# bifurcation/fourq

Hardware: AMD Instinct MI355X
Metric: FourQ scalar-mults/sec (batch, whole node) (higher is better)
Workload: dtype u64

## Files before the change

### fourq_amd/_lib.py

```python
import ctypes
import os
from ctypes import POINTER, c_char_p, c_int, c_size_t, c_uint8, c_uint64, c_void_p

HERE = os.path.dirname(os.path.abspath(__file__))
LIB_PATH = os.environ.get("FOURQ_AMD_LIB") or os.path.join(HERE, "libfourq_amd.so")

os.environ.setdefault("GPU_MAX_HW_QUEUES", "8")

OK, ERR_INVALID, ERR_NODEVICE, ERR_NOMEM, ERR_HIP = 0, -1, -2, -3, -4
DH_OK, DH_NOT_ON_CURVE, DH_NEUTRAL = 0, 1, 2
DECODE_OK, DECODE_RESERVED_BIT, DECODE_NOT_ON_CURVE, DECODE_REF_ATTRIBUTE_ERROR = 0, 1, 2, 3

MAX_BATCH = 0xFFFFFF00
ABI_VERSION = 600
COMB_POINTS = 1024 + 80
COMB_WORDS = COMB_POINTS * 12
BYTES_DECODE_BASE = 16
SIG_S_RANGE, SIG_MSG_CLAMPED, SIG_MAX_MSG = 32, 64, 1 << 20
H2C_RO, H2C_NU, H2C_MAX_DST = 0, 1, 255


class HostStats(ctypes.Structure):
    _fields_ = [("h2d_ms", ctypes.c_double), ("d2h_ms", ctypes.c_double), ("h2d_bytes", c_uint64), ("d2h_bytes", c_uint64),
                ("chunks", ctypes.c_uint32), ("pinned_in", c_int), ("pinned_out", c_int), ("kernels_ms", ctypes.c_double), ("kernels_span_ms", ctypes.c_double),
# ... 24 lines not shown
    "fourq_ctx_host_stats_sized": (c_int, [c_void_p, c_void_p, c_size_t]),
    "fourq_ctx_host_chunk_stamps": (c_int, [c_void_p, ctypes.c_uint32, POINTER(ctypes.c_double)]),
    "fourq_ctx_set_host_timing": (c_int, [c_void_p, c_int]),
    "fourq_diag_clock": (c_int, [c_void_p, ctypes.c_uint32, POINTER(ctypes.c_double), POINTER(ctypes.c_double), POINTER(ctypes.c_double), POINTER(c_int)]),
    "fourq_diag_clock_begin": (c_int, [c_void_p]),
    "fourq_diag_clock_stop": (c_int, [c_void_p]),
    "fourq_diag_clock_end": (c_int, [c_void_p, POINTER(ctypes.c_double), POINTER(ctypes.c_double), POINTER(ctypes.c_double), POINTER(ctypes.c_double)]),
    "fourq_dev_alloc": (c_int, [c_void_p, c_size_t, POINTER(c_void_p)]),
    "fourq_dev_free": (c_int, [c_void_p, c_void_p]),
    "fourq_dev_upload": (c_int, [c_void_p, c_void_p, c_void_p, c_size_t]),
    "fourq_dev_download": (c_int, [c_void_p, c_void_p, c_void_p, c_size_t]),
    "fourq_table_windowed": (c_int, [c_void_p, c_void_p, c_void_p]),
    "fourq_table_endo": (c_int, [c_void_p, c_void_p, c_void_p]),
    "fourq_mul_endo_batch": (c_int, [c_void_p, c_void_p, c_void_p, c_void_p, c_size_t]),
    "fourq_mul_windowed_batch": (c_int, [c_void_p, c_void_p, c_void_p, c_void_p, c_size_t]),
    "fourq_mul_endo_batch_dev": (c_int, [c_void_p, c_void_p, c_void_p, c_void_p, c_size_t]),
    "fourq_mul_windowed_batch_dev": (c_int, [c_void_p, c_void_p, c_void_p, c_void_p, c_size_t]),
    "fourq_mul_endo_affine_batch": (c_int, [c_void_p, c_void_p, c_void_p, c_void_p, c_size_t]),
    "fourq_mul_windowed_affine_batch": (c_int, [c_void_p, c_void_p, c_void_p, c_void_p, c_size_t]),
    "fourq_mul_endo_affine_batch_dev": (c_int, [c_void_p, c_void_p, c_void_p, c_void_p, c_size_t]),
    "fourq_mul_windowed_affine_batch_dev": (c_int, [c_void_p, c_void_p, c_void_p, c_void_p, c_size_t]),
    "fourq_mul_endo_bytes_batch": (c_int, [c_void_p, c_void_p, c_void_p, c_void_p, c_void_p, c_size_t]),
    "fourq_mul_windowed_bytes_batch": (c_int, [c_void_p, c_void_p, c_void_p, c_void_p, c_void_p, c_size_t]),
    "fourq_mul_endo_bytes_batch_dev": (c_int, [c_void_p, c_void_p, c_void_p, c_void_p, c_void_p, c_size_t]),
    "fourq_mul_windowed_bytes_batch_dev": (c_int, [c_void_p, c_void_p, c_void_p, c_void_p, c_void_p, c_size_t]),
    "fourq_mul_endo_fixed_batch": (c_int, [c_void_p, c_void_p, c_void_p, c_void_p, c_size_t]),
    "fourq_mul_windowed_fixed_batch": (c_int, [c_void_p, c_void_p, c_void_p, c_void_p, c_size_t]),
    "fourq_mul_endo_fixed_batch_dev": (c_int, [c_void_p, c_void_p, c_void_p, c_void_p, c_size_t]),
    "fourq_mul_windowed_fixed_batch_dev": (c_int, [c_void_p, c_void_p, c_void_p, c_void_p, c_size_t]),
    "fourq_mul_endo_mixed_batch": (c_int, [c_void_p, c_void_p, c_void_p, c_void_p, c_void_p, c_void_p, c_size_t]),
    "fourq_mul_endo_mixed_batch_dev": (c_int, [c_void_p, c_void_p, c_void_p, c_void_p, c_void_p, c_void_p, c_size_t]),
    "fourq_dh_endo_batch": (c_int, [c_void_p, c_void_p, c_void_p, c_void_p, c_void_p, c_void_p, c_size_t]),
    "fourq_dh_windowed_batch": (c_int, [c_void_p, c_void_p, c_void_p, c_void_p, c_void_p, c_void_p, c_size_t]),
    "fourq_dh_endo_batch_dev": (c_int, [c_void_p, c_void_p, c_void_p, c_void_p, c_void_p, c_void_p, c_size_t]),
    "fourq_dh_windowed_batch_dev": (c_int, [c_void_p, c_void_p, c_void_p, c_void_p, c_void_p, c_void_p, c_size_t]),
    "fourq_dh_endo_bytes_batch": (c_int, [c_void_p, c_void_p, c_void_p, c_void_p, c_void_p, c_void_p, c_size_t]),
    "fourq_dh_windowed_bytes_batch": (c_int, [c_void_p, c_void_p, c_void_p, c_void_p, c_void_p, c_void_p, c_size_t]),
    "fourq_dh_endo_bytes_batch_dev": (c_int, [c_void_p, c_void_p, c_void_p, c_void_p, c_void_p, c_void_p, c_size_t]),
    "fourq_dh_windowed_bytes_batch_dev": (c_int, [c_void_p, c_void_p, c_void_p, c_void_p, c_void_p, c_void_p, c_size_t]),
    "fourq_dh_exchange_batch": (c_int, [c_void_p, c_void_p, c_void_p, c_void_p, c_void_p, c_void_p, c_void_p, c_size_t]),
    "fourq_dh_exchange_batch_dev": (c_int, [c_void_p, c_void_p, c_void_p, c_void_p, c_void_p, c_void_p, c_void_p, c_size_t]),
    "fourq_dh_exchange_comb_batch": (c_int, [c_void_p, c_void_p, c_void_p, c_void_p, c_void_p, c_void_p, c_size_t]),
    "fourq_dh_exchange_comb_batch_dev": (c_int, [c_void_p, c_void_p, c_void_p, c_void_p, c_void_p, c_void_p, c_size_t]),
    "fourq_comb_table": (c_int, [c_void_p, c_void_p, c_void_p]),
    "fourq_comb_stage": (c_int, [c_void_p, c_void_p]),
    "fourq_comb_mul_batch": (c_int, [c_void_p, c_void_p, c_void_p, c_void_p, c_void_p, c_size_t]),
    "fourq_comb_mul_batch_dev": (c_int, [c_void_p, c_void_p, c_void_p, c_void_p, c_void_p, c_size_t]),
    "fourq_double_mul_affine_batch": (c_int, [c_void_p, c_void_p, c_void_p, c_void_p, c_void_p, c_void_p, c_size_t]),
    "fourq_double_mul_affine_batch_dev": (c_int, [c_void_p, c_void_p, c_void_p, c_void_p, c_void_p, c_void_p, c_size_t]),
    "fourq_double_mul_bytes_batch": (c_int, [c_void_p, c_void_p, c_void_p, c_void_p, c_void_p, c_void_p, c_void_p, c_size_t]),
    "fourq_double_mul_bytes_batch_dev": (c_int, [c_void_p, c_void_p, c_void_p, c_void_p, c_void_p, c_void_p, c_void_p, c_size_t]),
    "fourq_verify_bytes_batch": (c_int, [c_void_p, c_void_p, c_void_p, c_void_p, c_void_p, c_void_p, c_void_p, c_void_p, c_size_t]),
    "fourq_verify_bytes_batch_dev": (c_int, [c_void_p, c_void_p, c_void_p, c_void_p, c_void_p, c_void_p, c_void_p, c_void_p, c_size_t]),
    "fourq_sha512_batch": (c_int, [c_void_p, c_void_p, c_size_t, c_void_p, c_size_t, c_void_p, c_size_t]),
    "fourq_sha512_batch_dev": (c_int, [c_void_p, c_void_p, c_size_t, c_void_p, c_size_t, c_void_p, c_size_t]),
    "fourq_sig_keygen_batch": (c_int, [c_void_p, c_void_p, c_void_p, c_void_p, c_size_t]),
    "fourq_sig_keygen_batch_dev": (c_int, [c_void_p, c_void_p, c_void_p, c_void_p, c_size_t]),
    "fourq_sig_sign_batch": (c_int, [c_void_p, c_void_p, c_void_p, c_void_p, c_void_p, c_size_t, c_void_p, c_size_t, c_void_p, c_size_t]),
    "fourq_sig_sign_batch_dev": (c_int, [c_void_p, c_void_p, c_void_p, c_void_p, c_void_p, c_size_t, c_void_p, c_size_t, c_void_p, c_size_t]),
    "fourq_sig_verify_batch": (c_int, [c_void_p, c_void_p, c_void_p, c_void_p, c_size_t, c_void_p, c_size_t, c_void_p, c_void_p, c_void_p, c_size_t]),
    "fourq_sig_verify_batch_dev": (c_int, [c_void_p, c_void_p, c_void_p, c_void_p, c_size_t, c_void_p, c_size_t, c_void_p, c_void_p, c_void_p, c_size_t]),
    "fourq_hash_to_field_batch": (c_int, [c_void_p, c_void_p, c_size_t, c_int, c_void_p, c_size_t, c_void_p, c_size_t, c_void_p, c_size_t]),
    "fourq_hash_to_field_batch_dev": (c_int, [c_void_p, c_void_p, c_size_t, c_int, c_void_p, c_size_t, c_void_p, c_size_t, c_void_p, c_size_t]),
    "fourq_map_to_curve_batch": (c_int, [c_void_p, c_void_p, c_void_p, c_size_t]),
    "fourq_map_to_curve_batch_dev": (c_int, [c_void_p, c_void_p, c_void_p, c_size_t]),
    "fourq_hash_to_curve_batch": (c_int, [c_void_p, c_void_p, c_size_t, c_int, c_void_p, c_size_t, c_void_p, c_size_t, c_void_p, c_size_t]),
    "fourq_hash_to_curve_batch_dev": (c_int, [c_void_p, c_void_p, c_size_t, c_int, c_void_p, c_size_t, c_void_p, c_size_t, c_void_p, c_size_t]),
    "fourq_hash_to_curve_affine_batch": (c_int, [c_void_p, c_void_p, c_size_t, c_int, c_void_p, c_size_t, c_void_p, c_size_t, c_void_p, c_size_t]),
    "fourq_hash_to_curve_affine_batch_dev": (c_int, [c_void_p, c_void_p, c_size_t, c_int, c_void_p, c_size_t, c_void_p, c_size_t, c_void_p, c_size_t]),
    "fourq_encode_batch": (c_int, [c_void_p, c_void_p, c_void_p, c_size_t]),
    "fourq_decode_batch": (c_int, [c_void_p, c_void_p, c_void_p, c_void_p, c_size_t]),
    "fourq_encode_batch_dev": (c_int, [c_void_p, c_void_p, c_void_p, c_size_t]),
    "fourq_decode_batch_dev": (c_int, [c_void_p, c_void_p, c_void_p, c_void_p, c_size_t]),
    "fourq_prim_words": (c_int, [c_int, POINTER(c_size_t), POINTER(c_size_t)]),
    "fourq_prim_batch": (c_int, [c_void_p, c_int, c_void_p, c_void_p, c_size_t]),
}

PRIM = {
    "FP_ADD": 0, "FP_SUB": 1, "FP_MUL": 2, "FP_SQR": 3, "FP_NEG": 4, "FP_INV": 5, "FP_INVSQRT": 6, "FP_SELECT": 7,
    "FP2_ADD": 16, "FP2_SUB": 17, "FP2_MUL": 18, "FP2_SQR": 19, "FP2_NEG": 20, "FP2_CONJ": 21, "FP2_INV": 22, "FP2_SELECT": 23,
    "PT_DBL": 32, "PT_ADD": 33, "PT_ADD_CORE": 34, "PT_R1TOR2": 35, "PT_R1TOR3": 36, "PT_R2TOR4": 37,
    "PT_TAU": 38, "PT_TAU_DUAL": 39, "PT_UPSILON": 40, "PT_CHI": 41, "PT_PHI": 42, "PT_PSI": 43,
    "PT_ON_CURVE": 44, "PT_COFACTOR392": 45, "PT_R1TOAFFINE": 46, "PT_MAP_ELL2": 47,
    "SC_DECOMPOSE": 64, "SC_RECODE": 65, "SC_WINDOWED": 66, "SC_REDUCE512": 67, "SC_MULSUB": 68, "SC_MUL": 69,
}


class FourQError(RuntimeError):
    pass


_lib = None


def load():
    global _lib
    if _lib is not None:
        return _lib
    if os.environ.get("FOURQ_NO_TORCH") != "1":
        try:
            import torch
        except ImportError:
            pass
    if not os.path.exists(LIB_PATH):
        try:
            from .build import build_library
            build_library()
        except Exception as exc:
            raise FourQError("libfourq_amd.so is not built (%s) and building it failed: %s. "
                             "Run `python -m fourq_amd.build`; there is no CPU fallback." % (LIB_PATH, exc))
    lib = ctypes.CDLL(LIB_PATH)
    for name, (res, args) in PROTOTYPES.items():
        fn = getattr(lib, name)
        fn.restype = res
        fn.argtypes = args
    if lib.fourq_version() != ABI_VERSION:
        raise FourQError("%s is version %d, this package expects %d: rebuild it (`python -m fourq_amd.build --force`)"
                         % (LIB_PATH, lib.fourq_version(), ABI_VERSION))
    _warn_if_not_built_from_these_sources(lib)
    _lib = lib
    return lib


def build_matches_sources(lib=None):
    if os.environ.get("FOURQ_AMD_LIB"):
        return None
    try:
        from .build import source_id
        want = source_id()
    except OSError:
        return None
    return (lib or load()).fourq_build_id().decode() == want


def _warn_if_not_built_from_these_sources(lib):
    if build_matches_sources(lib) is False:
        import warnings
        warnings.warn("%s (build %s) was not compiled from the sources in %s: run `python -m fourq_amd.build` -- results and timings "
                      "below are those of the OLD code" % (LIB_PATH, lib.fourq_build_id().decode(), os.path.join(HERE, "csrc")), RuntimeWarning, stacklevel=3)


def check(rc, ctx=None):
    if rc == OK:
        return
    lib = load()
    msg = lib.fourq_strerror(rc).decode()
    if ctx is not None and rc == ERR_HIP:
        msg += ": " + lib.fourq_last_error(ctx).decode()
    raise FourQError("fourq_amd: %s (code %d)" % (msg, rc))
```

### fourq_amd/csrc/fourq_amd.hip

```cpp
#include <hip/hip_runtime.h>
#include <stdint.h>
#include <stdio.h>
#include <stdlib.h>
#include <string.h>
#include <algorithm>
#include <functional>
#include <mutex>
#include <new>
#include <thread>
#include <utility>
#include <vector>

#ifndef FQ_CHAIN
#define FQ_CHAIN 0
#endif
#include "kernels.hip.h"
#include "pipeline_plan.h"
#include "work_layout.h"
#include "sig.hip.h"
#include "h2c.hip.h"

using namespace fq;

namespace {
// ... 247 lines not shown
    store_fe2(w, p.X); store_fe2(w + 4, p.Y); store_fe2(w + 8, p.Z);
}
FQ_DEV R2s ld_r2s(const u64* w) { return as_signed(load_r2_packed(w)); }

__global__ __launch_bounds__(64) void prim_kernel(int op, const u64* in, u64* out, u32 n, u32 iw, u32 ow) {
    u32 i = blockIdx.x * blockDim.x + threadIdx.x;
    if (i >= n) return;
    const u64* x = in + (size_t)i * iw;
    u64* y = out + (size_t)i * ow;
    switch (op) {
    case FOURQ_FP_ADD: st_fe(y, fe_add(ld_fe(x), ld_fe(x + 2))); break;
    case FOURQ_FP_SUB: st_fe(y, fe_sub(ld_fe(x), ld_fe(x + 2))); break;
    case FOURQ_FP_MUL: st_fe(y, fe_mul(ld_fe(x), ld_fe(x + 2))); break;
    case FOURQ_FP_SQR: st_fe(y, fe_sqr(ld_fe(x))); break;
    case FOURQ_FP_NEG: st_fe(y, fe_neg(ld_fe(x))); break;
    case FOURQ_FP_INV: st_fe(y, fe_inv(fe_carry(ld_fe(x)))); break;
    case FOURQ_FP_INVSQRT: st_fe(y, fe_invsqrt(fe_carry(ld_fe(x)))); break;
    case FOURQ_FP_SELECT:
    case FOURQ_FP2_SELECT: {
        const u64 m_lo = 0 - x[0], m_hi = ~x[1] + (x[0] == 0 ? 1 : 0);
        const int parts = op == FOURQ_FP_SELECT ? 1 : 2;
        const u64* a = x + 2;
        const u64* b = x + 2 + 2 * parts;
        for (int k = 0; k < parts; k++) {
            y[2 * k] = b[2 * k] ^ (m_lo & (a[2 * k] ^ b[2 * k]));
            y[2 * k + 1] = b[2 * k + 1] ^ (m_hi & (a[2 * k + 1] ^ b[2 * k + 1]));
        }
        break;
    }
    case FOURQ_FP2_ADD: store_fe2(y, fe2_add(load_fe2(x), load_fe2(x + 4))); break;
    case FOURQ_FP2_SUB: store_fe2(y, fe2_sub(load_fe2(x), load_fe2(x + 4))); break;
    case FOURQ_FP2_MUL: store_fe2(y, fe2_mul(load_fe2(x), load_fe2(x + 4))); break;
    case FOURQ_FP2_SQR: store_fe2(y, fe2_sqr(load_fe2(x))); break;
    case FOURQ_FP2_NEG: store_fe2(y, fe2_neg(load_fe2(x))); break;
    case FOURQ_FP2_CONJ: store_fe2(y, fe2_conj(load_fe2(x))); break;
    case FOURQ_FP2_INV: store_fe2(y, fe2_inv(load_fe2(x))); break;
    case FOURQ_PT_DBL: store_r1(y, dbl(load_r1(x))); break;
    case FOURQ_PT_ADD: store_r1(y, add(load_r1(x), ld_r2s(x + 20))); break;
    case FOURQ_PT_ADD_CORE: {
        R2 p = load_r2_packed(x);
        R3 p3; p3.N = widen<2>(p.N); p3.D = widen<3>(p.D); p3.E = p.E; p3.F = p.F;
        store_r1(y, add_core(p3, ld_r2s(x + 16)));
        break;
    }
    case FOURQ_PT_R1TOR2: store_r2_packed(y, r1_to_r2(load_r1(x))); break;
    case FOURQ_PT_R1TOR3: {
        R3 r = r1_to_r3(load_r1(x));
        store_fe2(y, r.N); store_fe2(y + 4, r.D); store_fe2(y + 8, r.E); store_fe2(y + 12, r.F);
        break;
    }
    case FOURQ_PT_R2TOR4: st_proj(y, r2_to_r4(ld_r2s(x))); break;
    case FOURQ_PT_TAU: st_proj(y, tau(load_fe2(x), load_fe2(x + 4), load_fe2(x + 8))); break;
    case FOURQ_PT_TAU_DUAL:
        store_r1(y, tau_dual(widen<2>(load_fe2(x)), widen<2>(load_fe2(x + 4)), widen<2>(load_fe2(x + 8))));
        break;
    case FOURQ_PT_UPSILON:
    case FOURQ_PT_CHI: {
        Proj<1, 2, 1> p; p.X = load_fe2(x); p.Y = widen<2>(load_fe2(x + 4)); p.Z = load_fe2(x + 8);
        if (op == FOURQ_PT_UPSILON) st_proj(y, upsilon(p)); else st_proj(y, chi(p));
        break;
    }
    case FOURQ_PT_PHI: store_r1(y, phi(load_r1(x))); break;
    case FOURQ_PT_PSI: store_r1(y, psi(load_r1(x))); break;
    case FOURQ_PT_ON_CURVE: y[0] = point_on_curve(load_fe2(x), load_fe2(x + 4)) ? 1 : 0; break;
    case FOURQ_PT_COFACTOR392: store_r1(y, clear_cofactor_392(load_fe2(x), load_fe2(x + 4))); break;
    case FOURQ_PT_R1TOAFFINE: {
        Fe2<1> ax, ay;
        r1_to_affine(load_r1(x), ax, ay);
        store_fe2(y, ax); store_fe2(y + 4, ay);
        break;
    }
    case FOURQ_SC_DECOMPOSE: {
        u64 m[4] = { x[0], x[1], x[2], x[3] }, v[4];
        decompose(m, v);
        y[0] = v[0]; y[1] = v[1]; y[2] = v[2]; y[3] = v[3];
        break;
    }
    case FOURQ_SC_RECODE: {
        u64 v[4] = { x[0], x[1], x[2], x[3] };
        EndoDigits e = recode(v);
        y[0] = e.sign; y[1] = e.d[0]; y[2] = e.d[1]; y[3] = e.d[2]; y[4] = e.top;
        break;
    }
    case FOURQ_SC_WINDOWED: {
        u64 m[4] = { x[0], x[1], x[2], x[3] };
        WinScalar w = win_reduce(m);
        uint8_t* b = reinterpret_cast<uint8_t*>(y);
        for (int k = 0; k < 62; k++) b[k] = (uint8_t)win_code_from_window(win_window(w, k));
        b[62] = (uint8_t)win_top_code(w);
        b[63] = 0;
        break;
    }
    default: break;
    }
}

struct PrimShape { int op; size_t in_words, out_words; };
const PrimShape PRIMS[] = {
    { FOURQ_FP_ADD, 4, 2 }, { FOURQ_FP_SUB, 4, 2 }, { FOURQ_FP_MUL, 4, 2 }, { FOURQ_FP_SQR, 4, 2 }, { FOURQ_FP_NEG, 4, 2 }, { FOURQ_FP_INV, 4, 2 }, { FOURQ_FP_INVSQRT, 4, 2 },
    { FOURQ_FP_SELECT, 6, 2 }, { FOURQ_FP2_SELECT, 10, 4 },
    { FOURQ_FP2_ADD, 8, 4 }, { FOURQ_FP2_SUB, 8, 4 }, { FOURQ_FP2_MUL, 8, 4 }, { FOURQ_FP2_SQR, 8, 4 }, { FOURQ_FP2_NEG, 8, 4 },
    { FOURQ_FP2_CONJ, 8, 4 }, { FOURQ_FP2_INV, 8, 4 },
    { FOURQ_PT_DBL, 20, 20 }, { FOURQ_PT_ADD, 36, 20 }, { FOURQ_PT_ADD_CORE, 32, 20 }, { FOURQ_PT_R1TOR2, 20, 16 },
    { FOURQ_PT_R1TOR3, 20, 16 }, { FOURQ_PT_R2TOR4, 16, 12 }, { FOURQ_PT_TAU, 12, 12 }, { FOURQ_PT_TAU_DUAL, 12, 20 },
    { FOURQ_PT_UPSILON, 12, 12 }, { FOURQ_PT_CHI, 12, 12 }, { FOURQ_PT_PHI, 20, 20 }, { FOURQ_PT_PSI, 20, 20 },
    { FOURQ_PT_ON_CURVE, 8, 1 }, { FOURQ_PT_COFACTOR392, 8, 20 }, { FOURQ_PT_R1TOAFFINE, 20, 8 },
    { FOURQ_PT_MAP_ELL2, 4, 8 },
    { FOURQ_SC_DECOMPOSE, 4, 4 }, { FOURQ_SC_RECODE, 4, 5 }, { FOURQ_SC_WINDOWED, 4, 8 },
    { FOURQ_SC_REDUCE512, 8, 4 }, { FOURQ_SC_MULSUB, 12, 4 }, { FOURQ_SC_MUL, 8, 4 },
};
const PrimShape* find_prim(int op) {
    for (const PrimShape& p : PRIMS) if (p.op == op) return &p;
    return nullptr;
}

}

enum PipeRouteId { PR_MUL_VAR = 0, PR_MUL_FIX = 2, PR_DH_VAR = 4, PR_DH_FIX = 6, PR_MIXED = 8, PR_COMB = 9, PR_ENCODE = 10, PR_DECODE = 11, PR_DHB_VAR = 12,
                   PR_DHB_FIX = 14, PR_AFF = 16, PR_BYTES = 18, PR_EXCH = 20, PR_EXCH_COMB = 22, PR_DOUBLE_AFF = 23, PR_DOUBLE_BYTES = 24, PR_DOUBLE_VERIFY = 25,
                   PR_SHA512 = 26, PR_SIG_KEYGEN = 27, PR_SIG_SIGN = 28, PR_SIG_VERIFY = 29, PR_H2F = 30, PR_H2C_MAP = 31, PR_H2C = 32, PR_H2C_AFFINE = 34, PR_COUNT = 36 };
static_assert(PR_H2C_AFFINE + FOURQ_H2C_NU < PR_COUNT && FOURQ_H2C_RO == 0 && FOURQ_H2C_NU == 1, "the highest route id plus its mode offset must fit fourq_ctx::plan_kt");
constexpr int PIPE_SLOTS_MAX = 6;
struct fourq_ctx {
    int device = 0;
    hipStream_t own_stream = nullptr;
    hipStream_t stream = nullptr;
    int cus = 0;
    size_t lanes = 0;
    size_t lanes_w4 = 0;
    size_t split_min = 0;
    size_t split_chunk = 0;
    bool split_all = false;
    size_t split_endo_min = 0;
    u32* scratch = nullptr;
    u32* table_limbs = nullptr;
    u32* table_slots = nullptr;
    u64* table_packed = nullptr;
    u32* comb_limbs = nullptr;
    u64* comb_packed = nullptr;
    uint64_t table_shadow[FOURQ_TABLE_WORDS];
    uint64_t comb_shadow[FOURQ_COMB_WORDS];
    bool table_staged = false, comb_staged = false;
    bool comb_known = false;
    hipEvent_t shadow_read = nullptr;
    u32* part_counter = nullptr;
    u32* part_list = nullptr;
    u32* part_slot = nullptr;
    u32* part_fix = nullptr;
    bool ct = false;
    int mixed_queue = -1;
    size_t quad_max = 0;
    size_t pair_max = 0;
    uint4* proj = nullptr;
    size_t proj_capacity = 0;
    int norm_k = -1;
    void* stage = nullptr;
    size_t stage_bytes = 0;
    char* work = nullptr;
    size_t work_bytes = 0;
    hipStream_t copy_in = nullptr, copy_out = nullptr;
    hipEvent_t in_done[PIPE_SLOTS_MAX] = {}, kernels_done[PIPE_SLOTS_MAX] = {}, out_done[PIPE_SLOTS_MAX] = {};
    std::vector<hipEvent_t> ticks;
    int pipe_slots = 0;
    int pipe_gens = 0;
    bool pipe_host_poll = false;
    bool pipe_host_wait = false;
    bool host_timing = false;
    double plan_kt[PR_COUNT][2] = {};
    double plan_link_in = 0, plan_link_out = 0;
    hipEvent_t probe_ticks[6] = {};
    bool fused_io = true;
    int plan_measure = 1;
    std::vector<float> chunk_stamps;
    char* pipe_dev = nullptr;      size_t pipe_dev_bytes = 0;
    char* pipe_pin = nullptr;      size_t pipe_pin_bytes = 0;
    u64* diag_stamps = nullptr;
    hipEvent_t diag_mark = nullptr;
    u64* diag_bracket = nullptr;
    bool diag_open = false;
    bool diag_stopped = false;
    char* zero_copy = nullptr;
    fourq_host_stats host_stats = {};
    bool host_bounce = true;
    bool host_zero_copy = true;
    char err[256] = { 0 };
    mutable std::recursive_mutex mu;
};

namespace {

int fail(fourq_ctx* c, hipError_t e, const char* what) {
// ... 1617 lines not shown
```

### fourq_amd/csrc/ladder_asm_gfx950.inc

```
#define FQ_ASM_CLOBBERS "vcc", "v168", "v169", "v170", "v171", "v172", "v173", "v174", "v175", "v176", "v177", "v178", "v179", "v180", "v181", "v182", "v183", "v184", "v185", "v186", "v187", "v188", "v189", "v190", "v191", "v192", "v193", "v194", "v195", "v196", "v197", "v198", "v199", "v200", "v201", "v202", "v203", "v204", "v205", "v206", "v207", "v208", "v209", "v210", "v211", "v212", "v213", "v214", "v215", "v216", "v217", "v218", "v219", "v220", "v221", "v222", "v223", "v224", "v225", "v226", "v227", "v228", "v229", "v230", "v231", "v232", "v233", "v234", "v235", "v236", "v237", "v238", "v239", "v240", "v241", "v242", "v243", "v244", "v245", "v246", "v247", "v248", "v249", "v250", "v251", "v252", "v253", "v254", "v255"
#define FQ_ASM_SMALL_CLOBBERS "vcc", "v236", "v237", "v238", "v239", "v240", "v241", "v242", "v243", "v244", "v245", "v246", "v247", "v248", "v249", "v250", "v251", "v252", "v253", "v254", "v255"
#define FQ_ASM_DBL \
    ".p2align 3\n" \
    "v_mov_b32_e32 v255, 0\n" \
    "v_mov_b32_e32 v253, 0\n" \
    "v_add_u32_e32 v168, %0, %10\n" \
    "v_add_u32_e32 v169, %1, %11\n" \
    "v_add_u32_e32 v170, %2, %12\n" \
    "v_add_u32_e32 v171, %3, %13\n" \
    "v_add_u32_e32 v172, %4, %14\n" \
    "v_add_u32_e32 v173, %5, %15\n" \
    "v_add_u32_e32 v174, %6, %16\n" \
    "v_add_u32_e32 v175, %7, %17\n" \
    "v_add_u32_e32 v176, %8, %18\n" \
    "v_add_u32_e32 v177, %9, %19\n" \
    "v_add_u32_e32 v178, %0, %5\n" \
    "v_add_u32_e32 v179, %1, %6\n" \
    "v_add_u32_e32 v180, %2, %7\n" \
    "v_add_u32_e32 v181, %3, %8\n" \
    "v_add_u32_e32 v182, %4, %9\n" \
    "v_sub_u32_e32 v183, %0, %5\n" \
    "v_sub_u32_e32 v184, %1, %6\n" \
    "v_sub_u32_e32 v185, %2, %7\n" \
    "v_sub_u32_e32 v186, %3, %8\n" \
// ... 1832 lines not shown
    "v_mad_i64_i32 v[250:251], vcc, v208, v233, v[250:251]\n" \
    "v_mad_i64_i32 v[248:249], vcc, v203, v229, v[248:249]\n" \
    "v_and_b32_e64 %23, %40, v250\n" \
    "v_ashrrev_i64 v[250:251], 26, v[250:251]\n" \
    "v_and_b32_e64 %28, %40, v248\n" \
    "v_ashrrev_i64 v[248:249], 26, v[248:249]\n" \
    "v_mad_i64_i32 v[250:251], vcc, v187, v195, v[250:251]\n" \
    "v_mad_i64_i32 v[248:249], vcc, v187, v194, v[248:249]\n" \
    "v_mad_i64_i32 v[250:251], vcc, v204, v194, v[250:251]\n" \
    "v_mad_i64_i32 v[248:249], vcc, v197, v195, v[248:249]\n" \
    "v_mad_i64_i32 v[250:251], vcc, v179, v193, v[250:251]\n" \
    "v_mad_i64_i32 v[248:249], vcc, v179, v185, v[248:249]\n" \
    "v_mad_i64_i32 v[250:251], vcc, v205, v185, v[250:251]\n" \
    "v_mad_i64_i32 v[248:249], vcc, v186, v193, v[248:249]\n" \
    "v_mad_i64_i32 v[250:251], vcc, v183, v184, v[250:251]\n" \
    "v_mad_i64_i32 v[248:249], vcc, v183, v182, v[248:249]\n" \
    "v_mad_i64_i32 v[250:251], vcc, v206, v182, v[250:251]\n" \
    "v_mad_i64_i32 v[248:249], vcc, v189, v184, v[248:249]\n" \
    "v_mad_i64_i32 v[250:251], vcc, v188, v180, v[250:251]\n" \
    "v_mad_i64_i32 v[248:249], vcc, v188, v181, v[248:249]\n" \
    "v_mad_i64_i32 v[250:251], vcc, v207, v181, v[250:251]\n" \
    "v_mad_i64_i32 v[248:249], vcc, v198, v180, v[248:249]\n" \
    "v_mad_i64_i32 v[250:251], vcc, v196, v169, v[250:251]\n" \
    "v_mad_i64_i32 v[248:249], vcc, v196, v178, v[248:249]\n" \
    "v_mad_i64_i32 v[250:251], vcc, v208, v178, v[250:251]\n" \
    "v_mad_i64_i32 v[248:249], vcc, v203, v169, v[248:249]\n" \
    "v_and_b32_e64 %24, %40, v250\n" \
    "v_ashrrev_i64 v[250:251], 26, v[250:251]\n" \
    "v_and_b32_e64 %29, %40, v248\n" \
    "v_ashrrev_i64 v[248:249], 26, v[248:249]\n" \
    "v_lshl_add_u64 v[250:251], v[250:251], 3, v[254:255]\n" \
    "v_lshl_add_u64 v[248:249], v[248:249], 3, v[252:253]\n" \
    "v_and_b32_e64 %20, %40, v250\n" \
    "v_alignbit_b32 v168, v251, v250, 26\n" \
    "v_add_u32_e32 %21, %21, v168\n" \
    "v_and_b32_e32 %25, %40, v248\n" \
    "v_alignbit_b32 v168, v249, v248, 26\n" \
    "v_add_u32_e32 %26, %26, v168\n" \
    ""
#define FQ_ASM_ADD \
    ".p2align 3\n" \
    "v_mov_b32_e32 v255, 0\n" \
    "v_mov_b32_e32 v253, 0\n" \
    "v_add_u32_e32 v168, %0, %10\n" \
    "v_add_u32_e32 v169, %1, %11\n" \
    "v_add_u32_e32 v170, %2, %12\n" \
    "v_add_u32_e32 v171, %3, %13\n" \
    "v_add_u32_e32 v172, %4, %14\n" \
    "v_add_u32_e32 v173, %5, %15\n" \
    "v_add_u32_e32 v174, %6, %16\n" \
    "v_add_u32_e32 v175, %7, %17\n" \
    "v_add_u32_e32 v176, %8, %18\n" \
    "v_add_u32_e32 v177, %9, %19\n" \
    "v_sub_u32_e32 v178, %10, %0\n" \
    "v_sub_u32_e32 v179, %11, %1\n" \
    "v_sub_u32_e32 v180, %12, %2\n" \
    "v_sub_u32_e32 v181, %13, %3\n" \
    "v_sub_u32_e32 v182, %14, %4\n" \
    "v_sub_u32_e32 v183, %15, %5\n" \
    "v_sub_u32_e32 v184, %16, %6\n" \
    "v_sub_u32_e32 v185, %17, %7\n" \
    "v_sub_u32_e32 v186, %18, %8\n" \
    "v_sub_u32_e32 v187, %19, %9\n" \
    "v_bitop3_b32 v188, %100, %70, %60 bitop3:0xca\n" \
    "v_bitop3_b32 v189, %100, %71, %61 bitop3:0xca\n" \
    "v_bitop3_b32 v190, %100, %72, %62 bitop3:0xca\n" \
    "v_bitop3_b32 v191, %100, %73, %63 bitop3:0xca\n" \
    "v_bitop3_b32 v192, %100, %74, %64 bitop3:0xca\n" \
    "v_bitop3_b32 v193, %100, %60, %70 bitop3:0xca\n" \
    "v_bitop3_b32 v194, %100, %61, %71 bitop3:0xca\n" \
    "v_bitop3_b32 v195, %100, %62, %72 bitop3:0xca\n" \
    "v_bitop3_b32 v196, %100, %63, %73 bitop3:0xca\n" \
    "v_bitop3_b32 v197, %100, %64, %74 bitop3:0xca\n" \
    "v_bitop3_b32 v198, %100, %75, %65 bitop3:0xca\n" \
    "v_bitop3_b32 v199, %100, %76, %66 bitop3:0xca\n" \
    "v_bitop3_b32 v200, %100, %77, %67 bitop3:0xca\n" \
    "v_bitop3_b32 v201, %100, %78, %68 bitop3:0xca\n" \
    "v_bitop3_b32 v202, %100, %79, %69 bitop3:0xca\n" \
    "v_bitop3_b32 v203, %100, %65, %75 bitop3:0xca\n" \
    "v_bitop3_b32 v204, %100, %66, %76 bitop3:0xca\n" \
    "v_bitop3_b32 v205, %100, %67, %77 bitop3:0xca\n" \
    "v_bitop3_b32 v206, %100, %68, %78 bitop3:0xca\n" \
    "v_bitop3_b32 v207, %100, %69, %79 bitop3:0xca\n" \
    "v_xor_b32_e32 v208, %100, %90\n" \
    "v_xor_b32_e32 v209, %100, %91\n" \
    "v_xor_b32_e32 v210, %100, %92\n" \
    "v_xor_b32_e32 v211, %100, %93\n" \
    "v_xor_b32_e32 v212, %100, %94\n" \
    "v_sub_u32_e32 v208, v208, %100\n" \
    "v_sub_u32_e32 v209, v209, %100\n" \
    "v_sub_u32_e32 v210, v210, %100\n" \
    "v_sub_u32_e32 v211, v211, %100\n" \
    "v_sub_u32_e32 v212, v212, %100\n" \
    "v_xor_b32_e32 v213, %100, %95\n" \
    "v_xor_b32_e32 v214, %100, %96\n" \
    "v_xor_b32_e32 v215, %100, %97\n" \
    "v_xor_b32_e32 v216, %100, %98\n" \
    "v_xor_b32_e32 v217, %100, %99\n" \
    "v_sub_u32_e32 v213, v213, %100\n" \
    "v_sub_u32_e32 v214, v214, %100\n" \
    "v_sub_u32_e32 v215, v215, %100\n" \
    "v_sub_u32_e32 v216, v216, %100\n" \
    "v_sub_u32_e32 v217, v217, %100\n" \
    "v_sub_u32_e32 v218, 0, v183\n" \
    "v_sub_u32_e32 v219, 0, v184\n" \
    "v_sub_u32_e32 v220, 0, v185\n" \
    "v_sub_u32_e32 v221, 0, v186\n" \
    "v_sub_u32_e32 v222, 0, v187\n" \
    "v_lshlrev_b32_e32 v223, 3, v194\n" \
    "v_lshlrev_b32_e32 v224, 3, v195\n" \
    "v_lshlrev_b32_e32 v225, 3, v196\n" \
    "v_lshlrev_b32_e32 v226, 3, v197\n" \
    "v_lshlrev_b32_e32 v227, 3, v204\n" \
    "v_lshlrev_b32_e32 v228, 3, v205\n" \
    "v_lshlrev_b32_e32 v229, 3, v206\n" \
    "v_lshlrev_b32_e64 v230, 3, v207\n" \
    "v_mad_i64_i32 v[250:251], vcc, v178, v193, 0\n" \
    "v_mad_i64_i32 v[248:249], vcc, v178, v203, 0\n" \
    "v_mad_i64_i32 v[250:251], vcc, v218, v203, v[250:251]\n" \
    "v_mad_i64_i32 v[248:249], vcc, v183, v193, v[248:249]\n" \
    "v_mad_i64_i32 v[250:251], vcc, v179, v226, v[250:251]\n" \
    "v_mad_i64_i32 v[248:249], vcc, v179, v230, v[248:249]\n" \
    "v_mad_i64_i32 v[250:251], vcc, v219, v230, v[250:251]\n" \
    "v_mad_i64_i32 v[248:249], vcc, v184, v226, v[248:249]\n" \
    "v_mad_i64_i32 v[250:251], vcc, v180, v225, v[250:251]\n" \
    "v_mad_i64_i32 v[248:249], vcc, v180, v229, v[248:249]\n" \
    "v_mad_i64_i32 v[250:251], vcc, v220, v229, v[250:251]\n" \
    "v_mad_i64_i32 v[248:249], vcc, v185, v225, v[248:249]\n" \
    "v_mad_i64_i32 v[250:251], vcc, v181, v224, v[250:251]\n" \
    "v_mad_i64_i32 v[248:249], vcc, v181, v228, v[248:249]\n" \
    "v_mad_i64_i32 v[250:251], vcc, v221, v228, v[250:251]\n" \
    "v_mad_i64_i32 v[248:249], vcc, v186, v224, v[248:249]\n" \
    "v_mad_i64_i32 v[250:251], vcc, v182, v223, v[250:251]\n" \
    "v_mad_i64_i32 v[248:249], vcc, v182, v227, v[248:249]\n" \
    "v_mad_i64_i32 v[250:251], vcc, v222, v227, v[250:251]\n" \
    "v_mad_i64_i32 v[248:249], vcc, v187, v223, v[248:249]\n" \
    "v_and_b32_e64 v254, %101, v250\n" \
    "v_ashrrev_i64 v[250:251], 26, v[250:251]\n" \
    "v_and_b32_e64 v252, %101, v248\n" \
    "v_ashrrev_i64 v[248:249], 26, v[248:249]\n" \
    "v_mad_i64_i32 v[250:251], vcc, v178, v194, v[250:251]\n" \
    "v_mad_i64_i32 v[248:249], vcc, v178, v204, v[248:249]\n" \
    "v_mad_i64_i32 v[250:251], vcc, v218, v204, v[250:251]\n" \
    "v_mad_i64_i32 v[248:249], vcc, v183, v194, v[248:249]\n" \
    "v_mad_i64_i32 v[250:251], vcc, v179, v193, v[250:251]\n" \
    "v_mad_i64_i32 v[248:249], vcc, v179, v203, v[248:249]\n" \
    "v_mad_i64_i32 v[250:251], vcc, v219, v203, v[250:251]\n" \
    "v_mad_i64_i32 v[248:249], vcc, v184, v193, v[248:249]\n" \
    "v_mad_i64_i32 v[250:251], vcc, v180, v226, v[250:251]\n" \
    "v_mad_i64_i32 v[248:249], vcc, v180, v230, v[248:249]\n" \
    "v_mad_i64_i32 v[250:251], vcc, v220, v230, v[250:251]\n" \
    "v_mad_i64_i32 v[248:249], vcc, v185, v226, v[248:249]\n" \
    "v_mad_i64_i32 v[250:251], vcc, v181, v225, v[250:251]\n" \
    "v_mad_i64_i32 v[248:249], vcc, v181, v229, v[248:249]\n" \
    "v_mad_i64_i32 v[250:251], vcc, v221, v229, v[250:251]\n" \
    "v_mad_i64_i32 v[248:249], vcc, v186, v225, v[248:249]\n" \
    "v_mad_i64_i32 v[250:251], vcc, v182, v224, v[250:251]\n" \
    "v_mad_i64_i32 v[248:249], vcc, v182, v228, v[248:249]\n" \
    "v_mad_i64_i32 v[250:251], vcc, v222, v228, v[250:251]\n" \
    "v_mad_i64_i32 v[248:249], vcc, v187, v224, v[248:249]\n" \
    "v_and_b32_e64 v223, %101, v250\n" \
    "v_ashrrev_i64 v[250:251], 26, v[250:251]\n" \
    "v_and_b32_e64 v224, %101, v248\n" \
    "v_ashrrev_i64 v[248:249], 26, v[248:249]\n" \
    "v_mad_i64_i32 v[250:251], vcc, v178, v195, v[250:251]\n" \
    "v_mad_i64_i32 v[248:249], vcc, v178, v205, v[248:249]\n" \
    "v_mad_i64_i32 v[250:251], vcc, v218, v205, v[250:251]\n" \
    "v_mad_i64_i32 v[248:249], vcc, v183, v195, v[248:249]\n" \
    "v_mad_i64_i32 v[250:251], vcc, v179, v194, v[250:251]\n" \
    "v_mad_i64_i32 v[248:249], vcc, v179, v204, v[248:249]\n" \
    "v_mad_i64_i32 v[250:251], vcc, v219, v204, v[250:251]\n" \
    "v_mad_i64_i32 v[248:249], vcc, v184, v194, v[248:249]\n" \
    "v_mad_i64_i32 v[250:251], vcc, v180, v193, v[250:251]\n" \
    "v_mad_i64_i32 v[248:249], vcc, v180, v203, v[248:249]\n" \
    "v_mad_i64_i32 v[250:251], vcc, v220, v203, v[250:251]\n" \
    "v_mad_i64_i32 v[248:249], vcc, v185, v193, v[248:249]\n" \
    "v_mad_i64_i32 v[250:251], vcc, v181, v226, v[250:251]\n" \
    "v_mad_i64_i32 v[248:249], vcc, v181, v230, v[248:249]\n" \
    "v_mad_i64_i32 v[250:251], vcc, v221, v230, v[250:251]\n" \
    "v_mad_i64_i32 v[248:249], vcc, v186, v226, v[248:249]\n" \
    "v_mad_i64_i32 v[250:251], vcc, v182, v225, v[250:251]\n" \
    "v_mad_i64_i32 v[248:249], vcc, v182, v229, v[248:249]\n" \
    "v_mad_i64_i32 v[250:251], vcc, v222, v229, v[250:251]\n" \
    "v_mad_i64_i32 v[248:249], vcc, v187, v225, v[248:249]\n" \
    "v_and_b32_e64 v225, %101, v250\n" \
    "v_ashrrev_i64 v[250:251], 26, v[250:251]\n" \
    "v_and_b32_e64 v227, %101, v248\n" \
    "v_ashrrev_i64 v[248:249], 26, v[248:249]\n" \
    "v_mad_i64_i32 v[250:251], vcc, v178, v196, v[250:251]\n" \
    "v_mad_i64_i32 v[248:249], vcc, v178, v206, v[248:249]\n" \
    "v_mad_i64_i32 v[250:251], vcc, v218, v206, v[250:251]\n" \
    "v_mad_i64_i32 v[248:249], vcc, v183, v196, v[248:249]\n" \
    "v_mad_i64_i32 v[250:251], vcc, v179, v195, v[250:251]\n" \
    "v_mad_i64_i32 v[248:249], vcc, v179, v205, v[248:249]\n" \
    "v_mad_i64_i32 v[250:251], vcc, v219, v205, v[250:251]\n" \
    "v_mad_i64_i32 v[248:249], vcc, v184, v195, v[248:249]\n" \
    "v_mad_i64_i32 v[250:251], vcc, v180, v194, v[250:251]\n" \
    "v_mad_i64_i32 v[248:249], vcc, v180, v204, v[248:249]\n" \
    "v_mad_i64_i32 v[250:251], vcc, v220, v204, v[250:251]\n" \
    "v_mad_i64_i32 v[248:249], vcc, v185, v194, v[248:249]\n" \
    "v_mad_i64_i32 v[250:251], vcc, v181, v193, v[250:251]\n" \
    "v_mad_i64_i32 v[248:249], vcc, v181, v203, v[248:249]\n" \
    "v_mad_i64_i32 v[250:251], vcc, v221, v203, v[250:251]\n" \
    "v_mad_i64_i32 v[248:249], vcc, v186, v193, v[248:249]\n" \
    "v_mad_i64_i32 v[250:251], vcc, v182, v226, v[250:251]\n" \
    "v_mad_i64_i32 v[248:249], vcc, v182, v230, v[248:249]\n" \
    "v_mad_i64_i32 v[250:251], vcc, v222, v230, v[250:251]\n" \
    "v_mad_i64_i32 v[248:249], vcc, v187, v226, v[248:249]\n" \
    "v_and_b32_e64 v226, %101, v250\n" \
    "v_ashrrev_i64 v[250:251], 26, v[250:251]\n" \
    "v_and_b32_e64 v228, %101, v248\n" \
    "v_ashrrev_i64 v[248:249], 26, v[248:249]\n" \
    "v_mad_i64_i32 v[250:251], vcc, v178, v197, v[250:251]\n" \
    "v_mad_i64_i32 v[248:249], vcc, v178, v207, v[248:249]\n" \
    "v_mad_i64_i32 v[250:251], vcc, v218, v207, v[250:251]\n" \
    "v_mad_i64_i32 v[248:249], vcc, v183, v197, v[248:249]\n" \
    "v_mad_i64_i32 v[250:251], vcc, v179, v196, v[250:251]\n" \
    "v_mad_i64_i32 v[248:249], vcc, v179, v206, v[248:249]\n" \
    "v_mad_i64_i32 v[250:251], vcc, v219, v206, v[250:251]\n" \
    "v_mad_i64_i32 v[248:249], vcc, v184, v196, v[248:249]\n" \
    "v_mad_i64_i32 v[250:251], vcc, v180, v195, v[250:251]\n" \
    "v_mad_i64_i32 v[248:249], vcc, v180, v205, v[248:249]\n" \
    "v_mad_i64_i32 v[250:251], vcc, v220, v205, v[250:251]\n" \
    "v_mad_i64_i32 v[248:249], vcc, v185, v195, v[248:249]\n" \
    "v_mad_i64_i32 v[250:251], vcc, v181, v194, v[250:251]\n" \
    "v_mad_i64_i32 v[248:249], vcc, v181, v204, v[248:249]\n" \
    "v_mad_i64_i32 v[250:251], vcc, v221, v204, v[250:251]\n" \
    "v_mad_i64_i32 v[248:249], vcc, v186, v194, v[248:249]\n" \
    "v_mad_i64_i32 v[250:251], vcc, v182, v193, v[250:251]\n" \
    "v_mad_i64_i32 v[248:249], vcc, v182, v203, v[248:249]\n" \
    "v_mad_i64_i32 v[250:251], vcc, v222, v203, v[250:251]\n" \
    "v_mad_i64_i32 v[248:249], vcc, v187, v193, v[248:249]\n" \
    "v_and_b32_e64 v178, %101, v250\n" \
    "v_ashrrev_i64 v[250:251], 26, v[250:251]\n" \
    "v_and_b32_e64 v179, %101, v248\n" \
    "v_ashrrev_i64 v[248:249], 26, v[248:249]\n" \
    "v_lshl_add_u64 v[250:251], v[250:251], 3, v[254:255]\n" \
    "v_lshl_add_u64 v[248:249], v[248:249], 3, v[252:253]\n" \
    "v_and_b32_e64 v180, %101, v250\n" \
    "v_alignbit_b32 v181, v251, v250, 26\n" \
    "v_add_u32_e32 v223, v223, v181\n" \
    "v_and_b32_e32 v181, %101, v248\n" \
    "v_alignbit_b32 v182, v249, v248, 26\n" \
    "v_add_u32_e32 v224, v224, v182\n" \
    "v_sub_u32_e32 v182, 0, v173\n" \
    "v_sub_u32_e32 v183, 0, v174\n" \
    "v_sub_u32_e32 v184, 0, v175\n" \
    "v_sub_u32_e32 v185, 0, v176\n" \
    "v_sub_u32_e32 v186, 0, v177\n" \
    "v_lshlrev_b32_e32 v187, 3, v189\n" \
    "v_lshlrev_b32_e32 v193, 3, v190\n" \
    "v_lshlrev_b32_e32 v194, 3, v191\n" \
    "v_lshlrev_b32_e32 v195, 3, v192\n" \
    "v_lshlrev_b32_e32 v196, 3, v199\n" \
    "v_lshlrev_b32_e32 v197, 3, v200\n" \
    "v_lshlrev_b32_e32 v203, 3, v201\n" \
    "v_lshlrev_b32_e32 v204, 3, v202\n" \
    "v_mad_i64_i32 v[250:251], vcc, v168, v188, 0\n" \
    "v_mad_i64_i32 v[248:249], vcc, v168, v198, 0\n" \
    "v_mad_i64_i32 v[250:251], vcc, v182, v198, v[250:251]\n" \
    "v_mad_i64_i32 v[248:249], vcc, v173, v188, v[248:249]\n" \
    "v_mad_i64_i32 v[250:251], vcc, v169, v195, v[250:251]\n" \
    "v_mad_i64_i32 v[248:249], vcc, v169, v204, v[248:249]\n" \
    "v_mad_i64_i32 v[250:251], vcc, v183, v204, v[250:251]\n" \
    "v_mad_i64_i32 v[248:249], vcc, v174, v195, v[248:249]\n" \
    "v_mad_i64_i32 v[250:251], vcc, v170, v194, v[250:251]\n" \
    "v_mad_i64_i32 v[248:249], vcc, v170, v203, v[248:249]\n" \
    "v_mad_i64_i32 v[250:251], vcc, v184, v203, v[250:251]\n" \
    "v_mad_i64_i32 v[248:249], vcc, v175, v194, v[248:249]\n" \
    "v_mad_i64_i32 v[250:251], vcc, v171, v193, v[250:251]\n" \
    "v_mad_i64_i32 v[248:249], vcc, v171, v197, v[248:249]\n" \
    "v_mad_i64_i32 v[250:251], vcc, v185, v197, v[250:251]\n" \
    "v_mad_i64_i32 v[248:249], vcc, v176, v193, v[248:249]\n" \
    "v_mad_i64_i32 v[250:251], vcc, v172, v187, v[250:251]\n" \
    "v_mad_i64_i32 v[248:249], vcc, v172, v196, v[248:249]\n" \
    "v_mad_i64_i32 v[250:251], vcc, v186, v196, v[250:251]\n" \
    "v_mad_i64_i32 v[248:249], vcc, v177, v187, v[248:249]\n" \
    "v_and_b32_e64 v254, %101, v250\n" \
    "v_ashrrev_i64 v[250:251], 26, v[250:251]\n" \
    "v_and_b32_e64 v252, %101, v248\n" \
    "v_ashrrev_i64 v[248:249], 26, v[248:249]\n" \
    "v_mad_i64_i32 v[250:251], vcc, v168, v189, v[250:251]\n" \
    "v_mad_i64_i32 v[248:249], vcc, v168, v199, v[248:249]\n" \
    "v_mad_i64_i32 v[250:251], vcc, v182, v199, v[250:251]\n" \
    "v_mad_i64_i32 v[248:249], vcc, v173, v189, v[248:249]\n" \
    "v_mad_i64_i32 v[250:251], vcc, v169, v188, v[250:251]\n" \
    "v_mad_i64_i32 v[248:249], vcc, v169, v198, v[248:249]\n" \
    "v_mad_i64_i32 v[250:251], vcc, v183, v198, v[250:251]\n" \
    "v_mad_i64_i32 v[248:249], vcc, v174, v188, v[248:249]\n" \
    "v_mad_i64_i32 v[250:251], vcc, v170, v195, v[250:251]\n" \
    "v_mad_i64_i32 v[248:249], vcc, v170, v204, v[248:249]\n" \
    "v_mad_i64_i32 v[250:251], vcc, v184, v204, v[250:251]\n" \
    "v_mad_i64_i32 v[248:249], vcc, v175, v195, v[248:249]\n" \
    "v_mad_i64_i32 v[250:251], vcc, v171, v194, v[250:251]\n" \
    "v_mad_i64_i32 v[248:249], vcc, v171, v203, v[248:249]\n" \
    "v_mad_i64_i32 v[250:251], vcc, v185, v203, v[250:251]\n" \
    "v_mad_i64_i32 v[248:249], vcc, v176, v194, v[248:249]\n" \
    "v_mad_i64_i32 v[250:251], vcc, v172, v193, v[250:251]\n" \
// ... 4 lines not shown
    "v_ashrrev_i64 v[250:251], 26, v[250:251]\n" \
    "v_and_b32_e64 v193, %101, v248\n" \
    "v_ashrrev_i64 v[248:249], 26, v[248:249]\n" \
    "v_mad_i64_i32 v[250:251], vcc, v168, v190, v[250:251]\n" \
    "v_mad_i64_i32 v[248:249], vcc, v168, v200, v[248:249]\n" \
    "v_mad_i64_i32 v[250:251], vcc, v182, v200, v[250:251]\n" \
    "v_mad_i64_i32 v[248:249], vcc, v173, v190, v[248:249]\n" \
    "v_mad_i64_i32 v[250:251], vcc, v169, v189, v[250:251]\n" \
    "v_mad_i64_i32 v[248:249], vcc, v169, v199, v[248:249]\n" \
    "v_mad_i64_i32 v[250:251], vcc, v183, v199, v[250:251]\n" \
    "v_mad_i64_i32 v[248:249], vcc, v174, v189, v[248:249]\n" \
    "v_mad_i64_i32 v[250:251], vcc, v170, v188, v[250:251]\n" \
    "v_mad_i64_i32 v[248:249], vcc, v170, v198, v[248:249]\n" \
    "v_mad_i64_i32 v[250:251], vcc, v184, v198, v[250:251]\n" \
    "v_mad_i64_i32 v[248:249], vcc, v175, v188, v[248:249]\n" \
    "v_mad_i64_i32 v[250:251], vcc, v171, v195, v[250:251]\n" \
    "v_mad_i64_i32 v[248:249], vcc, v171, v204, v[248:249]\n" \
    "v_mad_i64_i32 v[250:251], vcc, v185, v204, v[250:251]\n" \
    "v_mad_i64_i32 v[248:249], vcc, v176, v195, v[248:249]\n" \
    "v_mad_i64_i32 v[250:251], vcc, v172, v194, v[250:251]\n" \
    "v_mad_i64_i32 v[248:249], vcc, v172, v203, v[248:249]\n" \
    "v_mad_i64_i32 v[250:251], vcc, v186, v203, v[250:251]\n" \
    "v_mad_i64_i32 v[248:249], vcc, v177, v194, v[248:249]\n" \
    "v_and_b32_e64 v194, %101, v250\n" \
    "v_ashrrev_i64 v[250:251], 26, v[250:251]\n" \
    "v_and_b32_e64 v196, %101, v248\n" \
    "v_ashrrev_i64 v[248:249], 26, v[248:249]\n" \
    "v_mad_i64_i32 v[250:251], vcc, v168, v191, v[250:251]\n" \
    "v_mad_i64_i32 v[248:249], vcc, v168, v201, v[248:249]\n" \
    "v_mad_i64_i32 v[250:251], vcc, v182, v201, v[250:251]\n" \
    "v_mad_i64_i32 v[248:249], vcc, v173, v191, v[248:249]\n" \
    "v_mad_i64_i32 v[250:251], vcc, v169, v190, v[250:251]\n" \
    "v_mad_i64_i32 v[248:249], vcc, v169, v200, v[248:249]\n" \
    "v_mad_i64_i32 v[250:251], vcc, v183, v200, v[250:251]\n" \
    "v_mad_i64_i32 v[248:249], vcc, v174, v190, v[248:249]\n" \
    "v_mad_i64_i32 v[250:251], vcc, v170, v189, v[250:251]\n" \
    "v_mad_i64_i32 v[248:249], vcc, v170, v199, v[248:249]\n" \
    "v_mad_i64_i32 v[250:251], vcc, v184, v199, v[250:251]\n" \
    "v_mad_i64_i32 v[248:249], vcc, v175, v189, v[248:249]\n" \
    "v_mad_i64_i32 v[250:251], vcc, v171, v188, v[250:251]\n" \
    "v_mad_i64_i32 v[248:249], vcc, v171, v198, v[248:249]\n" \
    "v_mad_i64_i32 v[250:251], vcc, v185, v198, v[250:251]\n" \
    "v_mad_i64_i32 v[248:249], vcc, v176, v188, v[248:249]\n" \
    "v_mad_i64_i32 v[250:251], vcc, v172, v195, v[250:251]\n" \
    "v_mad_i64_i32 v[248:249], vcc, v172, v204, v[248:249]\n" \
    "v_mad_i64_i32 v[250:251], vcc, v186, v204, v[250:251]\n" \
    "v_mad_i64_i32 v[248:249], vcc, v177, v195, v[248:249]\n" \
    "v_and_b32_e64 v195, %101, v250\n" \
    "v_ashrrev_i64 v[250:251], 26, v[250:251]\n" \
    "v_and_b32_e64 v197, %101, v248\n" \
    "v_ashrrev_i64 v[248:249], 26, v[248:249]\n" \
    "v_mad_i64_i32 v[250:251], vcc, v168, v192, v[250:251]\n" \
    "v_mad_i64_i32 v[248:249], vcc, v168, v202, v[248:249]\n" \
    "v_mad_i64_i32 v[250:251], vcc, v182, v202, v[250:251]\n" \
    "v_mad_i64_i32 v[248:249], vcc, v173, v192, v[248:249]\n" \
    "v_mad_i64_i32 v[250:251], vcc, v169, v191, v[250:251]\n" \
    "v_mad_i64_i32 v[248:249], vcc, v169, v201, v[248:249]\n" \
    "v_mad_i64_i32 v[250:251], vcc, v183, v201, v[250:251]\n" \
    "v_mad_i64_i32 v[248:249], vcc, v174, v191, v[248:249]\n" \
    "v_mad_i64_i32 v[250:251], vcc, v170, v190, v[250:251]\n" \
    "v_mad_i64_i32 v[248:249], vcc, v170, v200, v[248:249]\n" \
    "v_mad_i64_i32 v[250:251], vcc, v184, v200, v[250:251]\n" \
    "v_mad_i64_i32 v[248:249], vcc, v175, v190, v[248:249]\n" \
    "v_mad_i64_i32 v[250:251], vcc, v171, v189, v[250:251]\n" \
    "v_mad_i64_i32 v[248:249], vcc, v171, v199, v[248:249]\n" \
    "v_mad_i64_i32 v[250:251], vcc, v185, v199, v[250:251]\n" \
    "v_mad_i64_i32 v[248:249], vcc, v176, v189, v[248:249]\n" \
    "v_mad_i64_i32 v[250:251], vcc, v172, v188, v[250:251]\n" \
    "v_mad_i64_i32 v[248:249], vcc, v172, v198, v[248:249]\n" \
    "v_mad_i64_i32 v[250:251], vcc, v186, v198, v[250:251]\n" \
    "v_mad_i64_i32 v[248:249], vcc, v177, v188, v[248:249]\n" \
    "v_and_b32_e64 v168, %101, v250\n" \
    "v_ashrrev_i64 v[250:251], 26, v[250:251]\n" \
    "v_and_b32_e64 v169, %101, v248\n" \
    "v_ashrrev_i64 v[248:249], 26, v[248:249]\n" \
    "v_lshl_add_u64 v[250:251], v[250:251], 3, v[254:255]\n" \
    "v_lshl_add_u64 v[248:249], v[248:249], 3, v[252:253]\n" \
    "v_and_b32_e64 v170, %101, v250\n" \
    "v_alignbit_b32 v171, v251, v250, 26\n" \
    "v_add_u32_e32 v187, v187, v171\n" \
    "v_and_b32_e32 v171, %101, v248\n" \
    "v_alignbit_b32 v172, v249, v248, 26\n" \
    "v_add_u32_e32 v193, v193, v172\n" \
    "v_sub_u32_e32 v172, 0, v213\n" \
    "v_sub_u32_e32 v173, 0, v214\n" \
    "v_sub_u32_e32 v174, 0, v215\n" \
    "v_sub_u32_e32 v175, 0, v216\n" \
    "v_sub_u32_e32 v176, 0, v217\n" \
    "v_lshlrev_b32_e32 v177, 3, %51\n" \
    "v_lshlrev_b32_e32 v182, 3, %52\n" \
    "v_lshlrev_b32_e32 v183, 3, %53\n" \
    "v_lshlrev_b32_e32 v184, 3, %54\n" \
    "v_lshlrev_b32_e32 v185, 3, %56\n" \
    "v_lshlrev_b32_e32 v186, 3, %57\n" \
    "v_lshlrev_b32_e32 v188, 3, %58\n" \
    "v_lshlrev_b32_e32 v189, 3, %59\n" \
    "v_mad_i64_i32 v[250:251], vcc, v208, %50, 0\n" \
    "v_mad_i64_i32 v[248:249], vcc, v208, %55, 0\n" \
    "v_mad_i64_i32 v[250:251], vcc, v172, %55, v[250:251]\n" \
    "v_mad_i64_i32 v[248:249], vcc, v213, %50, v[248:249]\n" \
    "v_mad_i64_i32 v[250:251], vcc, v209, v184, v[250:251]\n" \
    "v_mad_i64_i32 v[248:249], vcc, v209, v189, v[248:249]\n" \
    "v_mad_i64_i32 v[250:251], vcc, v173, v189, v[250:251]\n" \
    "v_mad_i64_i32 v[248:249], vcc, v214, v184, v[248:249]\n" \
    "v_mad_i64_i32 v[250:251], vcc, v210, v183, v[250:251]\n" \
    "v_mad_i64_i32 v[248:249], vcc, v210, v188, v[248:249]\n" \
    "v_mad_i64_i32 v[250:251], vcc, v174, v188, v[250:251]\n" \
    "v_mad_i64_i32 v[248:249], vcc, v215, v183, v[248:249]\n" \
    "v_mad_i64_i32 v[250:251], vcc, v211, v182, v[250:251]\n" \
    "v_mad_i64_i32 v[248:249], vcc, v211, v186, v[248:249]\n" \
    "v_mad_i64_i32 v[250:251], vcc, v175, v186, v[250:251]\n" \
    "v_mad_i64_i32 v[248:249], vcc, v216, v182, v[248:249]\n" \
    "v_mad_i64_i32 v[250:251], vcc, v212, v177, v[250:251]\n" \
    "v_mad_i64_i32 v[248:249], vcc, v212, v185, v[248:249]\n" \
    "v_mad_i64_i32 v[250:251], vcc, v176, v185, v[250:251]\n" \
    "v_mad_i64_i32 v[248:249], vcc, v217, v177, v[248:249]\n" \
    "v_and_b32_e64 v254, %101, v250\n" \
    "v_ashrrev_i64 v[250:251], 26, v[250:251]\n" \
    "v_and_b32_e64 v252, %101, v248\n" \
    "v_ashrrev_i64 v[248:249], 26, v[248:249]\n" \
    "v_mad_i64_i32 v[250:251], vcc, v208, %51, v[250:251]\n" \
    "v_mad_i64_i32 v[248:249], vcc, v208, %56, v[248:249]\n" \
    "v_mad_i64_i32 v[250:251], vcc, v172, %56, v[250:251]\n" \
    "v_mad_i64_i32 v[248:249], vcc, v213, %51, v[248:249]\n" \
    "v_mad_i64_i32 v[250:251], vcc, v209, %50, v[250:251]\n" \
    "v_mad_i64_i32 v[248:249], vcc, v209, %55, v[248:249]\n" \
    "v_mad_i64_i32 v[250:251], vcc, v173, %55, v[250:251]\n" \
    "v_mad_i64_i32 v[248:249], vcc, v214, %50, v[248:249]\n" \
    "v_mad_i64_i32 v[250:251], vcc, v210, v184, v[250:251]\n" \
    "v_mad_i64_i32 v[248:249], vcc, v210, v189, v[248:249]\n" \
    "v_mad_i64_i32 v[250:251], vcc, v174, v189, v[250:251]\n" \
    "v_mad_i64_i32 v[248:249], vcc, v215, v184, v[248:249]\n" \
    "v_mad_i64_i32 v[250:251], vcc, v211, v183, v[250:251]\n" \
    "v_mad_i64_i32 v[248:249], vcc, v211, v188, v[248:249]\n" \
    "v_mad_i64_i32 v[250:251], vcc, v175, v188, v[250:251]\n" \
    "v_mad_i64_i32 v[248:249], vcc, v216, v183, v[248:249]\n" \
    "v_mad_i64_i32 v[250:251], vcc, v212, v182, v[250:251]\n" \
    "v_mad_i64_i32 v[248:249], vcc, v212, v186, v[248:249]\n" \
    "v_mad_i64_i32 v[250:251], vcc, v176, v186, v[250:251]\n" \
    "v_mad_i64_i32 v[248:249], vcc, v217, v182, v[248:249]\n" \
    "v_and_b32_e64 v177, %101, v250\n" \
    "v_ashrrev_i64 v[250:251], 26, v[250:251]\n" \
    "v_and_b32_e64 v182, %101, v248\n" \
    "v_ashrrev_i64 v[248:249], 26, v[248:249]\n" \
    "v_mad_i64_i32 v[250:251], vcc, v208, %52, v[250:251]\n" \
    "v_mad_i64_i32 v[248:249], vcc, v208, %57, v[248:249]\n" \
    "v_mad_i64_i32 v[250:251], vcc, v172, %57, v[250:251]\n" \
    "v_mad_i64_i32 v[248:249], vcc, v213, %52, v[248:249]\n" \
    "v_mad_i64_i32 v[250:251], vcc, v209, %51, v[250:251]\n" \
    "v_mad_i64_i32 v[248:249], vcc, v209, %56, v[248:249]\n" \
    "v_mad_i64_i32 v[250:251], vcc, v173, %56, v[250:251]\n" \
    "v_mad_i64_i32 v[248:249], vcc, v214, %51, v[248:249]\n" \
    "v_mad_i64_i32 v[250:251], vcc, v210, %50, v[250:251]\n" \
    "v_mad_i64_i32 v[248:249], vcc, v210, %55, v[248:249]\n" \
    "v_mad_i64_i32 v[250:251], vcc, v174, %55, v[250:251]\n" \
    "v_mad_i64_i32 v[248:249], vcc, v215, %50, v[248:249]\n" \
    "v_mad_i64_i32 v[250:251], vcc, v211, v184, v[250:251]\n" \
    "v_mad_i64_i32 v[248:249], vcc, v211, v189, v[248:249]\n" \
    "v_mad_i64_i32 v[250:251], vcc, v175, v189, v[250:251]\n" \
    "v_mad_i64_i32 v[248:249], vcc, v216, v184, v[248:249]\n" \
    "v_mad_i64_i32 v[250:251], vcc, v212, v183, v[250:251]\n" \
    "v_mad_i64_i32 v[248:249], vcc, v212, v188, v[248:249]\n" \
    "v_mad_i64_i32 v[250:251], vcc, v176, v188, v[250:251]\n" \
    "v_mad_i64_i32 v[248:249], vcc, v217, v183, v[248:249]\n" \
    "v_and_b32_e64 v183, %101, v250\n" \
    "v_ashrrev_i64 v[250:251], 26, v[250:251]\n" \
    "v_and_b32_e64 v185, %101, v248\n" \
    "v_ashrrev_i64 v[248:249], 26, v[248:249]\n" \
    "v_mad_i64_i32 v[250:251], vcc, v208, %53, v[250:251]\n" \
    "v_mad_i64_i32 v[248:249], vcc, v208, %58, v[248:249]\n" \
    "v_mad_i64_i32 v[250:251], vcc, v172, %58, v[250:251]\n" \
    "v_mad_i64_i32 v[248:249], vcc, v213, %53, v[248:249]\n" \
    "v_mad_i64_i32 v[250:251], vcc, v209, %52, v[250:251]\n" \
    "v_mad_i64_i32 v[248:249], vcc, v209, %57, v[248:249]\n" \
    "v_mad_i64_i32 v[250:251], vcc, v173, %57, v[250:251]\n" \
    "v_mad_i64_i32 v[248:249], vcc, v214, %52, v[248:249]\n" \
    "v_mad_i64_i32 v[250:251], vcc, v210, %51, v[250:251]\n" \
    "v_mad_i64_i32 v[248:249], vcc, v210, %56, v[248:249]\n" \
    "v_mad_i64_i32 v[250:251], vcc, v174, %56, v[250:251]\n" \
    "v_mad_i64_i32 v[248:249], vcc, v215, %51, v[248:249]\n" \
    "v_mad_i64_i32 v[250:251], vcc, v211, %50, v[250:251]\n" \
    "v_mad_i64_i32 v[248:249], vcc, v211, %55, v[248:249]\n" \
    "v_mad_i64_i32 v[250:251], vcc, v175, %55, v[250:251]\n" \
    "v_mad_i64_i32 v[248:249], vcc, v216, %50, v[248:249]\n" \
    "v_mad_i64_i32 v[250:251], vcc, v212, v184, v[250:251]\n" \
    "v_mad_i64_i32 v[248:249], vcc, v212, v189, v[248:249]\n" \
    "v_mad_i64_i32 v[250:251], vcc, v176, v189, v[250:251]\n" \
    "v_mad_i64_i32 v[248:249], vcc, v217, v184, v[248:249]\n" \
    "v_and_b32_e64 v184, %101, v250\n" \
    "v_ashrrev_i64 v[250:251], 26, v[250:251]\n" \
    "v_and_b32_e64 v186, %101, v248\n" \
    "v_ashrrev_i64 v[248:249], 26, v[248:249]\n" \
    "v_mad_i64_i32 v[250:251], vcc, v208, %54, v[250:251]\n" \
    "v_mad_i64_i32 v[248:249], vcc, v208, %59, v[248:249]\n" \
    "v_mad_i64_i32 v[250:251], vcc, v172, %59, v[250:251]\n" \
    "v_mad_i64_i32 v[248:249], vcc, v213, %54, v[248:249]\n" \
    "v_mad_i64_i32 v[250:251], vcc, v209, %53, v[250:251]\n" \
    "v_mad_i64_i32 v[248:249], vcc, v209, %58, v[248:249]\n" \
    "v_mad_i64_i32 v[250:251], vcc, v173, %58, v[250:251]\n" \
    "v_mad_i64_i32 v[248:249], vcc, v214, %53, v[248:249]\n" \
    "v_mad_i64_i32 v[250:251], vcc, v210, %52, v[250:251]\n" \
    "v_mad_i64_i32 v[248:249], vcc, v210, %57, v[248:249]\n" \
    "v_mad_i64_i32 v[250:251], vcc, v174, %57, v[250:251]\n" \
    "v_mad_i64_i32 v[248:249], vcc, v215, %52, v[248:249]\n" \
    "v_mad_i64_i32 v[250:251], vcc, v211, %51, v[250:251]\n" \
    "v_mad_i64_i32 v[248:249], vcc, v211, %56, v[248:249]\n" \
    "v_mad_i64_i32 v[250:251], vcc, v175, %56, v[250:251]\n" \
    "v_mad_i64_i32 v[248:249], vcc, v216, %51, v[248:249]\n" \
    "v_mad_i64_i32 v[250:251], vcc, v212, %50, v[250:251]\n" \
    "v_mad_i64_i32 v[248:249], vcc, v212, %55, v[248:249]\n" \
    "v_mad_i64_i32 v[250:251], vcc, v176, %55, v[250:251]\n" \
    "v_mad_i64_i32 v[248:249], vcc, v217, %50, v[248:249]\n" \
    "v_and_b32_e64 v172, %101, v250\n" \
    "v_ashrrev_i64 v[250:251], 26, v[250:251]\n" \
    "v_and_b32_e64 v173, %101, v248\n" \
    "v_ashrrev_i64 v[248:249], 26, v[248:249]\n" \
    "v_lshl_add_u64 v[250:251], v[250:251], 3, v[254:255]\n" \
    "v_lshl_add_u64 v[248:249], v[248:249], 3, v[252:253]\n" \
    "v_and_b32_e64 v174, %101, v250\n" \
    "v_alignbit_b32 v175, v251, v250, 26\n" \
    "v_add_u32_e32 v177, v177, v175\n" \
    "v_and_b32_e32 v175, %101, v248\n" \
    "v_alignbit_b32 v176, v249, v248, 26\n" \
    "v_add_u32_e32 v182, v182, v176\n" \
    "v_sub_u32_e32 v176, 0, %85\n" \
    "v_sub_u32_e32 v188, 0, %86\n" \
    "v_sub_u32_e32 v189, 0, %87\n" \
    "v_sub_u32_e32 v190, 0, %88\n" \
    "v_sub_u32_e32 v191, 0, %89\n" \
    "v_lshlrev_b32_e32 v192, 3, %21\n" \
    "v_lshlrev_b32_e32 v198, 3, %22\n" \
    "v_lshlrev_b32_e32 v199, 3, %23\n" \
    "v_lshlrev_b32_e32 v200, 3, %24\n" \
    "v_lshlrev_b32_e32 v201, 3, %26\n" \
    "v_lshlrev_b32_e32 v202, 3, %27\n" \
    "v_lshlrev_b32_e32 v203, 3, %28\n" \
    "v_lshlrev_b32_e32 v204, 3, %29\n" \
    "v_mad_i64_i32 v[250:251], vcc, %80, %20, 0\n" \
    "v_mad_i64_i32 v[248:249], vcc, %80, %25, 0\n" \
    "v_mad_i64_i32 v[250:251], vcc, v176, %25, v[250:251]\n" \
    "v_mad_i64_i32 v[248:249], vcc, %85, %20, v[248:249]\n" \
    "v_mad_i64_i32 v[250:251], vcc, %81, v200, v[250:251]\n" \
    "v_mad_i64_i32 v[248:249], vcc, %81, v204, v[248:249]\n" \
    "v_mad_i64_i32 v[250:251], vcc, v188, v204, v[250:251]\n" \
    "v_mad_i64_i32 v[248:249], vcc, %86, v200, v[248:249]\n" \
    "v_mad_i64_i32 v[250:251], vcc, %82, v199, v[250:251]\n" \
    "v_mad_i64_i32 v[248:249], vcc, %82, v203, v[248:249]\n" \
    "v_mad_i64_i32 v[250:251], vcc, v189, v203, v[250:251]\n" \
    "v_mad_i64_i32 v[248:249], vcc, %87, v199, v[248:249]\n" \
    "v_mad_i64_i32 v[250:251], vcc, %83, v198, v[250:251]\n" \
    "v_mad_i64_i32 v[248:249], vcc, %83, v202, v[248:249]\n" \
    "v_mad_i64_i32 v[250:251], vcc, v190, v202, v[250:251]\n" \
    "v_mad_i64_i32 v[248:249], vcc, %88, v198, v[248:249]\n" \
    "v_mad_i64_i32 v[250:251], vcc, %84, v192, v[250:251]\n" \
    "v_mad_i64_i32 v[248:249], vcc, %84, v201, v[248:249]\n" \
    "v_mad_i64_i32 v[250:251], vcc, v191, v201, v[250:251]\n" \
    "v_mad_i64_i32 v[248:249], vcc, %89, v192, v[248:249]\n" \
    "v_and_b32_e64 v254, %101, v250\n" \
    "v_ashrrev_i64 v[250:251], 26, v[250:251]\n" \
    "v_and_b32_e64 v252, %101, v248\n" \
    "v_ashrrev_i64 v[248:249], 26, v[248:249]\n" \
    "v_mad_i64_i32 v[250:251], vcc, %80, %21, v[250:251]\n" \
    "v_mad_i64_i32 v[248:249], vcc, %80, %26, v[248:249]\n" \
    "v_mad_i64_i32 v[250:251], vcc, v176, %26, v[250:251]\n" \
    "v_mad_i64_i32 v[248:249], vcc, %85, %21, v[248:249]\n" \
    "v_mad_i64_i32 v[250:251], vcc, %81, %20, v[250:251]\n" \
    "v_mad_i64_i32 v[248:249], vcc, %81, %25, v[248:249]\n" \
    "v_mad_i64_i32 v[250:251], vcc, v188, %25, v[250:251]\n" \
    "v_mad_i64_i32 v[248:249], vcc, %86, %20, v[248:249]\n" \
    "v_mad_i64_i32 v[250:251], vcc, %82, v200, v[250:251]\n" \
    "v_mad_i64_i32 v[248:249], vcc, %82, v204, v[248:249]\n" \
    "v_mad_i64_i32 v[250:251], vcc, v189, v204, v[250:251]\n" \
    "v_mad_i64_i32 v[248:249], vcc, %87, v200, v[248:249]\n" \
    "v_mad_i64_i32 v[250:251], vcc, %83, v199, v[250:251]\n" \
    "v_mad_i64_i32 v[248:249], vcc, %83, v203, v[248:249]\n" \
    "v_mad_i64_i32 v[250:251], vcc, v190, v203, v[250:251]\n" \
    "v_mad_i64_i32 v[248:249], vcc, %88, v199, v[248:249]\n" \
    "v_mad_i64_i32 v[250:251], vcc, %84, v198, v[250:251]\n" \
    "v_mad_i64_i32 v[248:249], vcc, %84, v202, v[248:249]\n" \
    "v_mad_i64_i32 v[250:251], vcc, v191, v202, v[250:251]\n" \
    "v_mad_i64_i32 v[248:249], vcc, %89, v198, v[248:249]\n" \
    "v_and_b32_e64 v192, %101, v250\n" \
    "v_ashrrev_i64 v[250:251], 26, v[250:251]\n" \
    "v_and_b32_e64 v198, %101, v248\n" \
    "v_ashrrev_i64 v[248:249], 26, v[248:249]\n" \
    "v_mad_i64_i32 v[250:251], vcc, %80, %22, v[250:251]\n" \
    "v_mad_i64_i32 v[248:249], vcc, %80, %27, v[248:249]\n" \
    "v_mad_i64_i32 v[250:251], vcc, v176, %27, v[250:251]\n" \
    "v_mad_i64_i32 v[248:249], vcc, %85, %22, v[248:249]\n" \
    "v_mad_i64_i32 v[250:251], vcc, %81, %21, v[250:251]\n" \
    "v_mad_i64_i32 v[248:249], vcc, %81, %26, v[248:249]\n" \
    "v_mad_i64_i32 v[250:251], vcc, v188, %26, v[250:251]\n" \
    "v_mad_i64_i32 v[248:249], vcc, %86, %21, v[248:249]\n" \
    "v_mad_i64_i32 v[250:251], vcc, %82, %20, v[250:251]\n" \
    "v_mad_i64_i32 v[248:249], vcc, %82, %25, v[248:249]\n" \
// ... 1488 lines not shown
    "v_mad_i64_i32 v[248:249], vcc, v188, v178, v[248:249]\n" \
    "v_mad_i64_i32 v[250:251], vcc, v207, v178, v[250:251]\n" \
    "v_mad_i64_i32 v[248:249], vcc, v198, v169, v[248:249]\n" \
    "v_mad_i64_i32 v[250:251], vcc, v196, v229, v[250:251]\n" \
    "v_mad_i64_i32 v[248:249], vcc, v196, v233, v[248:249]\n" \
    "v_mad_i64_i32 v[250:251], vcc, v208, v233, v[250:251]\n" \
    "v_mad_i64_i32 v[248:249], vcc, v203, v229, v[248:249]\n" \
    "v_and_b32_e64 %23, %91, v250\n" \
    "v_ashrrev_i64 v[250:251], 26, v[250:251]\n" \
    "v_and_b32_e64 %28, %91, v248\n" \
    "v_ashrrev_i64 v[248:249], 26, v[248:249]\n" \
    "v_mad_i64_i32 v[250:251], vcc, v187, v195, v[250:251]\n" \
    "v_mad_i64_i32 v[248:249], vcc, v187, v194, v[248:249]\n" \
    "v_mad_i64_i32 v[250:251], vcc, v204, v194, v[250:251]\n" \
    "v_mad_i64_i32 v[248:249], vcc, v197, v195, v[248:249]\n" \
    "v_mad_i64_i32 v[250:251], vcc, v179, v193, v[250:251]\n" \
    "v_mad_i64_i32 v[248:249], vcc, v179, v185, v[248:249]\n" \
    "v_mad_i64_i32 v[250:251], vcc, v205, v185, v[250:251]\n" \
    "v_mad_i64_i32 v[248:249], vcc, v186, v193, v[248:249]\n" \
    "v_mad_i64_i32 v[250:251], vcc, v183, v184, v[250:251]\n" \
    "v_mad_i64_i32 v[248:249], vcc, v183, v182, v[248:249]\n" \
    "v_mad_i64_i32 v[250:251], vcc, v206, v182, v[250:251]\n" \
    "v_mad_i64_i32 v[248:249], vcc, v189, v184, v[248:249]\n" \
    "v_mad_i64_i32 v[250:251], vcc, v188, v180, v[250:251]\n" \
    "v_mad_i64_i32 v[248:249], vcc, v188, v181, v[248:249]\n" \
    "v_mad_i64_i32 v[250:251], vcc, v207, v181, v[250:251]\n" \
    "v_mad_i64_i32 v[248:249], vcc, v198, v180, v[248:249]\n" \
    "v_mad_i64_i32 v[250:251], vcc, v196, v169, v[250:251]\n" \
    "v_mad_i64_i32 v[248:249], vcc, v196, v178, v[248:249]\n" \
    "v_mad_i64_i32 v[250:251], vcc, v208, v178, v[250:251]\n" \
    "v_mad_i64_i32 v[248:249], vcc, v203, v169, v[248:249]\n" \
    "v_and_b32_e64 %24, %91, v250\n" \
    "v_ashrrev_i64 v[250:251], 26, v[250:251]\n" \
    "v_and_b32_e64 %29, %91, v248\n" \
    "v_ashrrev_i64 v[248:249], 26, v[248:249]\n" \
    "v_lshl_add_u64 v[250:251], v[250:251], 3, v[254:255]\n" \
    "v_lshl_add_u64 v[248:249], v[248:249], 3, v[252:253]\n" \
    "v_and_b32_e64 %20, %91, v250\n" \
    "v_alignbit_b32 v168, v251, v250, 26\n" \
    "v_add_u32_e32 %21, %21, v168\n" \
    "v_and_b32_e32 %25, %91, v248\n" \
    "v_alignbit_b32 v168, v249, v248, 26\n" \
    "v_add_u32_e32 %26, %26, v168\n" \
    "v_add_u32_e32 v168, %0, %10\n" \
    "v_add_u32_e32 v169, %1, %11\n" \
    "v_add_u32_e32 v170, %2, %12\n" \
    "v_add_u32_e32 v171, %3, %13\n" \
    "v_add_u32_e32 v172, %4, %14\n" \
    "v_add_u32_e32 v173, %5, %15\n" \
    "v_add_u32_e32 v174, %6, %16\n" \
    "v_add_u32_e32 v175, %7, %17\n" \
    "v_add_u32_e32 v176, %8, %18\n" \
    "v_add_u32_e32 v177, %9, %19\n" \
    "v_sub_u32_e32 v178, %10, %0\n" \
    "v_sub_u32_e32 v179, %11, %1\n" \
    "v_sub_u32_e32 v180, %12, %2\n" \
    "v_sub_u32_e32 v181, %13, %3\n" \
    "v_sub_u32_e32 v182, %14, %4\n" \
    "v_sub_u32_e32 v183, %15, %5\n" \
    "v_sub_u32_e32 v184, %16, %6\n" \
    "v_sub_u32_e32 v185, %17, %7\n" \
    "v_sub_u32_e32 v186, %18, %8\n" \
    "v_sub_u32_e64 v187, %19, %9\n" \
    "v_bitop3_b32 v188, %90, %60, %50 bitop3:0xca\n" \
    "v_bitop3_b32 v189, %90, %61, %51 bitop3:0xca\n" \
    "v_bitop3_b32 v190, %90, %62, %52 bitop3:0xca\n" \
    "v_bitop3_b32 v191, %90, %63, %53 bitop3:0xca\n" \
    "v_bitop3_b32 v192, %90, %64, %54 bitop3:0xca\n" \
    "v_bitop3_b32 v193, %90, %50, %60 bitop3:0xca\n" \
    "v_bitop3_b32 v194, %90, %51, %61 bitop3:0xca\n" \
    "v_bitop3_b32 v195, %90, %52, %62 bitop3:0xca\n" \
    "v_bitop3_b32 v196, %90, %53, %63 bitop3:0xca\n" \
    "v_bitop3_b32 v197, %90, %54, %64 bitop3:0xca\n" \
    "v_bitop3_b32 v198, %90, %65, %55 bitop3:0xca\n" \
    "v_bitop3_b32 v199, %90, %66, %56 bitop3:0xca\n" \
    "v_bitop3_b32 v200, %90, %67, %57 bitop3:0xca\n" \
    "v_bitop3_b32 v201, %90, %68, %58 bitop3:0xca\n" \
    "v_bitop3_b32 v202, %90, %69, %59 bitop3:0xca\n" \
    "v_bitop3_b32 v203, %90, %55, %65 bitop3:0xca\n" \
    "v_bitop3_b32 v204, %90, %56, %66 bitop3:0xca\n" \
    "v_bitop3_b32 v205, %90, %57, %67 bitop3:0xca\n" \
    "v_bitop3_b32 v206, %90, %58, %68 bitop3:0xca\n" \
    "v_bitop3_b32 v207, %90, %59, %69 bitop3:0xca\n" \
    "v_xor_b32_e32 v208, %90, %80\n" \
    "v_xor_b32_e32 v209, %90, %81\n" \
    "v_xor_b32_e32 v210, %90, %82\n" \
    "v_xor_b32_e32 v211, %90, %83\n" \
    "v_xor_b32_e32 v212, %90, %84\n" \
    "v_sub_u32_e32 v208, v208, %90\n" \
    "v_sub_u32_e32 v209, v209, %90\n" \
    "v_sub_u32_e32 v210, v210, %90\n" \
    "v_sub_u32_e32 v211, v211, %90\n" \
    "v_sub_u32_e32 v212, v212, %90\n" \
    "v_xor_b32_e32 v213, %90, %85\n" \
    "v_xor_b32_e32 v214, %90, %86\n" \
    "v_xor_b32_e32 v215, %90, %87\n" \
    "v_xor_b32_e32 v216, %90, %88\n" \
    "v_xor_b32_e32 v217, %90, %89\n" \
    "v_sub_u32_e32 v213, v213, %90\n" \
    "v_sub_u32_e32 v214, v214, %90\n" \
    "v_sub_u32_e32 v215, v215, %90\n" \
    "v_sub_u32_e32 v216, v216, %90\n" \
    "v_sub_u32_e32 v217, v217, %90\n" \
    "v_sub_u32_e32 v218, 0, v183\n" \
    "v_sub_u32_e32 v219, 0, v184\n" \
    "v_sub_u32_e32 v220, 0, v185\n" \
    "v_sub_u32_e32 v221, 0, v186\n" \
    "v_sub_u32_e32 v222, 0, v187\n" \
    "v_lshlrev_b32_e32 v223, 3, v194\n" \
    "v_lshlrev_b32_e32 v224, 3, v195\n" \
    "v_lshlrev_b32_e32 v225, 3, v196\n" \
    "v_lshlrev_b32_e32 v226, 3, v197\n" \
    "v_lshlrev_b32_e32 v227, 3, v204\n" \
    "v_lshlrev_b32_e32 v228, 3, v205\n" \
    "v_lshlrev_b32_e32 v229, 3, v206\n" \
    "v_lshlrev_b32_e64 v230, 3, v207\n" \
    "v_mad_i64_i32 v[250:251], vcc, v178, v193, 0\n" \
    "v_mad_i64_i32 v[248:249], vcc, v178, v203, 0\n" \
    "v_mad_i64_i32 v[250:251], vcc, v218, v203, v[250:251]\n" \
    "v_mad_i64_i32 v[248:249], vcc, v183, v193, v[248:249]\n" \
    "v_mad_i64_i32 v[250:251], vcc, v179, v226, v[250:251]\n" \
    "v_mad_i64_i32 v[248:249], vcc, v179, v230, v[248:249]\n" \
    "v_mad_i64_i32 v[250:251], vcc, v219, v230, v[250:251]\n" \
    "v_mad_i64_i32 v[248:249], vcc, v184, v226, v[248:249]\n" \
    "v_mad_i64_i32 v[250:251], vcc, v180, v225, v[250:251]\n" \
    "v_mad_i64_i32 v[248:249], vcc, v180, v229, v[248:249]\n" \
    "v_mad_i64_i32 v[250:251], vcc, v220, v229, v[250:251]\n" \
    "v_mad_i64_i32 v[248:249], vcc, v185, v225, v[248:249]\n" \
    "v_mad_i64_i32 v[250:251], vcc, v181, v224, v[250:251]\n" \
    "v_mad_i64_i32 v[248:249], vcc, v181, v228, v[248:249]\n" \
    "v_mad_i64_i32 v[250:251], vcc, v221, v228, v[250:251]\n" \
    "v_mad_i64_i32 v[248:249], vcc, v186, v224, v[248:249]\n" \
    "v_mad_i64_i32 v[250:251], vcc, v182, v223, v[250:251]\n" \
    "v_mad_i64_i32 v[248:249], vcc, v182, v227, v[248:249]\n" \
    "v_mad_i64_i32 v[250:251], vcc, v222, v227, v[250:251]\n" \
    "v_mad_i64_i32 v[248:249], vcc, v187, v223, v[248:249]\n" \
    "v_and_b32_e64 v254, %91, v250\n" \
    "v_ashrrev_i64 v[250:251], 26, v[250:251]\n" \
    "v_and_b32_e64 v252, %91, v248\n" \
    "v_ashrrev_i64 v[248:249], 26, v[248:249]\n" \
    "v_mad_i64_i32 v[250:251], vcc, v178, v194, v[250:251]\n" \
    "v_mad_i64_i32 v[248:249], vcc, v178, v204, v[248:249]\n" \
    "v_mad_i64_i32 v[250:251], vcc, v218, v204, v[250:251]\n" \
    "v_mad_i64_i32 v[248:249], vcc, v183, v194, v[248:249]\n" \
    "v_mad_i64_i32 v[250:251], vcc, v179, v193, v[250:251]\n" \
    "v_mad_i64_i32 v[248:249], vcc, v179, v203, v[248:249]\n" \
    "v_mad_i64_i32 v[250:251], vcc, v219, v203, v[250:251]\n" \
    "v_mad_i64_i32 v[248:249], vcc, v184, v193, v[248:249]\n" \
    "v_mad_i64_i32 v[250:251], vcc, v180, v226, v[250:251]\n" \
    "v_mad_i64_i32 v[248:249], vcc, v180, v230, v[248:249]\n" \
    "v_mad_i64_i32 v[250:251], vcc, v220, v230, v[250:251]\n" \
    "v_mad_i64_i32 v[248:249], vcc, v185, v226, v[248:249]\n" \
    "v_mad_i64_i32 v[250:251], vcc, v181, v225, v[250:251]\n" \
    "v_mad_i64_i32 v[248:249], vcc, v181, v229, v[248:249]\n" \
    "v_mad_i64_i32 v[250:251], vcc, v221, v229, v[250:251]\n" \
    "v_mad_i64_i32 v[248:249], vcc, v186, v225, v[248:249]\n" \
    "v_mad_i64_i32 v[250:251], vcc, v182, v224, v[250:251]\n" \
    "v_mad_i64_i32 v[248:249], vcc, v182, v228, v[248:249]\n" \
    "v_mad_i64_i32 v[250:251], vcc, v222, v228, v[250:251]\n" \
    "v_mad_i64_i32 v[248:249], vcc, v187, v224, v[248:249]\n" \
    "v_and_b32_e64 v223, %91, v250\n" \
    "v_ashrrev_i64 v[250:251], 26, v[250:251]\n" \
    "v_and_b32_e64 v224, %91, v248\n" \
    "v_ashrrev_i64 v[248:249], 26, v[248:249]\n" \
    "v_mad_i64_i32 v[250:251], vcc, v178, v195, v[250:251]\n" \
    "v_mad_i64_i32 v[248:249], vcc, v178, v205, v[248:249]\n" \
    "v_mad_i64_i32 v[250:251], vcc, v218, v205, v[250:251]\n" \
    "v_mad_i64_i32 v[248:249], vcc, v183, v195, v[248:249]\n" \
    "v_mad_i64_i32 v[250:251], vcc, v179, v194, v[250:251]\n" \
    "v_mad_i64_i32 v[248:249], vcc, v179, v204, v[248:249]\n" \
    "v_mad_i64_i32 v[250:251], vcc, v219, v204, v[250:251]\n" \
    "v_mad_i64_i32 v[248:249], vcc, v184, v194, v[248:249]\n" \
    "v_mad_i64_i32 v[250:251], vcc, v180, v193, v[250:251]\n" \
    "v_mad_i64_i32 v[248:249], vcc, v180, v203, v[248:249]\n" \
    "v_mad_i64_i32 v[250:251], vcc, v220, v203, v[250:251]\n" \
    "v_mad_i64_i32 v[248:249], vcc, v185, v193, v[248:249]\n" \
    "v_mad_i64_i32 v[250:251], vcc, v181, v226, v[250:251]\n" \
    "v_mad_i64_i32 v[248:249], vcc, v181, v230, v[248:249]\n" \
    "v_mad_i64_i32 v[250:251], vcc, v221, v230, v[250:251]\n" \
    "v_mad_i64_i32 v[248:249], vcc, v186, v226, v[248:249]\n" \
    "v_mad_i64_i32 v[250:251], vcc, v182, v225, v[250:251]\n" \
    "v_mad_i64_i32 v[248:249], vcc, v182, v229, v[248:249]\n" \
    "v_mad_i64_i32 v[250:251], vcc, v222, v229, v[250:251]\n" \
    "v_mad_i64_i32 v[248:249], vcc, v187, v225, v[248:249]\n" \
    "v_and_b32_e64 v225, %91, v250\n" \
    "v_ashrrev_i64 v[250:251], 26, v[250:251]\n" \
    "v_and_b32_e64 v227, %91, v248\n" \
    "v_ashrrev_i64 v[248:249], 26, v[248:249]\n" \
    "v_mad_i64_i32 v[250:251], vcc, v178, v196, v[250:251]\n" \
    "v_mad_i64_i32 v[248:249], vcc, v178, v206, v[248:249]\n" \
    "v_mad_i64_i32 v[250:251], vcc, v218, v206, v[250:251]\n" \
    "v_mad_i64_i32 v[248:249], vcc, v183, v196, v[248:249]\n" \
    "v_mad_i64_i32 v[250:251], vcc, v179, v195, v[250:251]\n" \
    "v_mad_i64_i32 v[248:249], vcc, v179, v205, v[248:249]\n" \
    "v_mad_i64_i32 v[250:251], vcc, v219, v205, v[250:251]\n" \
    "v_mad_i64_i32 v[248:249], vcc, v184, v195, v[248:249]\n" \
    "v_mad_i64_i32 v[250:251], vcc, v180, v194, v[250:251]\n" \
    "v_mad_i64_i32 v[248:249], vcc, v180, v204, v[248:249]\n" \
    "v_mad_i64_i32 v[250:251], vcc, v220, v204, v[250:251]\n" \
    "v_mad_i64_i32 v[248:249], vcc, v185, v194, v[248:249]\n" \
    "v_mad_i64_i32 v[250:251], vcc, v181, v193, v[250:251]\n" \
    "v_mad_i64_i32 v[248:249], vcc, v181, v203, v[248:249]\n" \
    "v_mad_i64_i32 v[250:251], vcc, v221, v203, v[250:251]\n" \
    "v_mad_i64_i32 v[248:249], vcc, v186, v193, v[248:249]\n" \
    "v_mad_i64_i32 v[250:251], vcc, v182, v226, v[250:251]\n" \
    "v_mad_i64_i32 v[248:249], vcc, v182, v230, v[248:249]\n" \
    "v_mad_i64_i32 v[250:251], vcc, v222, v230, v[250:251]\n" \
    "v_mad_i64_i32 v[248:249], vcc, v187, v226, v[248:249]\n" \
    "v_and_b32_e64 v226, %91, v250\n" \
    "v_ashrrev_i64 v[250:251], 26, v[250:251]\n" \
    "v_and_b32_e64 v228, %91, v248\n" \
    "v_ashrrev_i64 v[248:249], 26, v[248:249]\n" \
    "v_mad_i64_i32 v[250:251], vcc, v178, v197, v[250:251]\n" \
    "v_mad_i64_i32 v[248:249], vcc, v178, v207, v[248:249]\n" \
    "v_mad_i64_i32 v[250:251], vcc, v218, v207, v[250:251]\n" \
    "v_mad_i64_i32 v[248:249], vcc, v183, v197, v[248:249]\n" \
    "v_mad_i64_i32 v[250:251], vcc, v179, v196, v[250:251]\n" \
    "v_mad_i64_i32 v[248:249], vcc, v179, v206, v[248:249]\n" \
    "v_mad_i64_i32 v[250:251], vcc, v219, v206, v[250:251]\n" \
    "v_mad_i64_i32 v[248:249], vcc, v184, v196, v[248:249]\n" \
    "v_mad_i64_i32 v[250:251], vcc, v180, v195, v[250:251]\n" \
    "v_mad_i64_i32 v[248:249], vcc, v180, v205, v[248:249]\n" \
    "v_mad_i64_i32 v[250:251], vcc, v220, v205, v[250:251]\n" \
    "v_mad_i64_i32 v[248:249], vcc, v185, v195, v[248:249]\n" \
    "v_mad_i64_i32 v[250:251], vcc, v181, v194, v[250:251]\n" \
    "v_mad_i64_i32 v[248:249], vcc, v181, v204, v[248:249]\n" \
    "v_mad_i64_i32 v[250:251], vcc, v221, v204, v[250:251]\n" \
    "v_mad_i64_i32 v[248:249], vcc, v186, v194, v[248:249]\n" \
    "v_mad_i64_i32 v[250:251], vcc, v182, v193, v[250:251]\n" \
    "v_mad_i64_i32 v[248:249], vcc, v182, v203, v[248:249]\n" \
    "v_mad_i64_i32 v[250:251], vcc, v222, v203, v[250:251]\n" \
    "v_mad_i64_i32 v[248:249], vcc, v187, v193, v[248:249]\n" \
    "v_and_b32_e64 v178, %91, v250\n" \
    "v_ashrrev_i64 v[250:251], 26, v[250:251]\n" \
    "v_and_b32_e64 v179, %91, v248\n" \
    "v_ashrrev_i64 v[248:249], 26, v[248:249]\n" \
    "v_lshl_add_u64 v[250:251], v[250:251], 3, v[254:255]\n" \
    "v_lshl_add_u64 v[248:249], v[248:249], 3, v[252:253]\n" \
    "v_and_b32_e64 v180, %91, v250\n" \
    "v_alignbit_b32 v181, v251, v250, 26\n" \
    "v_add_u32_e32 v223, v223, v181\n" \
    "v_and_b32_e32 v181, %91, v248\n" \
    "v_alignbit_b32 v182, v249, v248, 26\n" \
    "v_add_u32_e32 v224, v224, v182\n" \
    "v_sub_u32_e32 v182, 0, v173\n" \
    "v_sub_u32_e32 v183, 0, v174\n" \
    "v_sub_u32_e32 v184, 0, v175\n" \
    "v_sub_u32_e32 v185, 0, v176\n" \
    "v_sub_u32_e32 v186, 0, v177\n" \
    "v_lshlrev_b32_e32 v187, 3, v189\n" \
    "v_lshlrev_b32_e32 v193, 3, v190\n" \
    "v_lshlrev_b32_e32 v194, 3, v191\n" \
    "v_lshlrev_b32_e32 v195, 3, v192\n" \
    "v_lshlrev_b32_e32 v196, 3, v199\n" \
    "v_lshlrev_b32_e32 v197, 3, v200\n" \
    "v_lshlrev_b32_e32 v203, 3, v201\n" \
    "v_lshlrev_b32_e32 v204, 3, v202\n" \
    "v_mad_i64_i32 v[250:251], vcc, v168, v188, 0\n" \
    "v_mad_i64_i32 v[248:249], vcc, v168, v198, 0\n" \
    "v_mad_i64_i32 v[250:251], vcc, v182, v198, v[250:251]\n" \
    "v_mad_i64_i32 v[248:249], vcc, v173, v188, v[248:249]\n" \
    "v_mad_i64_i32 v[250:251], vcc, v169, v195, v[250:251]\n" \
    "v_mad_i64_i32 v[248:249], vcc, v169, v204, v[248:249]\n" \
    "v_mad_i64_i32 v[250:251], vcc, v183, v204, v[250:251]\n" \
    "v_mad_i64_i32 v[248:249], vcc, v174, v195, v[248:249]\n" \
    "v_mad_i64_i32 v[250:251], vcc, v170, v194, v[250:251]\n" \
    "v_mad_i64_i32 v[248:249], vcc, v170, v203, v[248:249]\n" \
    "v_mad_i64_i32 v[250:251], vcc, v184, v203, v[250:251]\n" \
    "v_mad_i64_i32 v[248:249], vcc, v175, v194, v[248:249]\n" \
    "v_mad_i64_i32 v[250:251], vcc, v171, v193, v[250:251]\n" \
    "v_mad_i64_i32 v[248:249], vcc, v171, v197, v[248:249]\n" \
    "v_mad_i64_i32 v[250:251], vcc, v185, v197, v[250:251]\n" \
    "v_mad_i64_i32 v[248:249], vcc, v176, v193, v[248:249]\n" \
    "v_mad_i64_i32 v[250:251], vcc, v172, v187, v[250:251]\n" \
    "v_mad_i64_i32 v[248:249], vcc, v172, v196, v[248:249]\n" \
    "v_mad_i64_i32 v[250:251], vcc, v186, v196, v[250:251]\n" \
    "v_mad_i64_i32 v[248:249], vcc, v177, v187, v[248:249]\n" \
    "v_and_b32_e64 v254, %91, v250\n" \
    "v_ashrrev_i64 v[250:251], 26, v[250:251]\n" \
    "v_and_b32_e64 v252, %91, v248\n" \
    "v_ashrrev_i64 v[248:249], 26, v[248:249]\n" \
    "v_mad_i64_i32 v[250:251], vcc, v168, v189, v[250:251]\n" \
    "v_mad_i64_i32 v[248:249], vcc, v168, v199, v[248:249]\n" \
    "v_mad_i64_i32 v[250:251], vcc, v182, v199, v[250:251]\n" \
    "v_mad_i64_i32 v[248:249], vcc, v173, v189, v[248:249]\n" \
    "v_mad_i64_i32 v[250:251], vcc, v169, v188, v[250:251]\n" \
    "v_mad_i64_i32 v[248:249], vcc, v169, v198, v[248:249]\n" \
    "v_mad_i64_i32 v[250:251], vcc, v183, v198, v[250:251]\n" \
    "v_mad_i64_i32 v[248:249], vcc, v174, v188, v[248:249]\n" \
    "v_mad_i64_i32 v[250:251], vcc, v170, v195, v[250:251]\n" \
    "v_mad_i64_i32 v[248:249], vcc, v170, v204, v[248:249]\n" \
    "v_mad_i64_i32 v[250:251], vcc, v184, v204, v[250:251]\n" \
    "v_mad_i64_i32 v[248:249], vcc, v175, v195, v[248:249]\n" \
    "v_mad_i64_i32 v[250:251], vcc, v171, v194, v[250:251]\n" \
    "v_mad_i64_i32 v[248:249], vcc, v171, v203, v[248:249]\n" \
    "v_mad_i64_i32 v[250:251], vcc, v185, v203, v[250:251]\n" \
    "v_mad_i64_i32 v[248:249], vcc, v176, v194, v[248:249]\n" \
    "v_mad_i64_i32 v[250:251], vcc, v172, v193, v[250:251]\n" \
// ... 4 lines not shown
    "v_ashrrev_i64 v[250:251], 26, v[250:251]\n" \
    "v_and_b32_e64 v193, %91, v248\n" \
    "v_ashrrev_i64 v[248:249], 26, v[248:249]\n" \
    "v_mad_i64_i32 v[250:251], vcc, v168, v190, v[250:251]\n" \
    "v_mad_i64_i32 v[248:249], vcc, v168, v200, v[248:249]\n" \
    "v_mad_i64_i32 v[250:251], vcc, v182, v200, v[250:251]\n" \
    "v_mad_i64_i32 v[248:249], vcc, v173, v190, v[248:249]\n" \
    "v_mad_i64_i32 v[250:251], vcc, v169, v189, v[250:251]\n" \
    "v_mad_i64_i32 v[248:249], vcc, v169, v199, v[248:249]\n" \
    "v_mad_i64_i32 v[250:251], vcc, v183, v199, v[250:251]\n" \
    "v_mad_i64_i32 v[248:249], vcc, v174, v189, v[248:249]\n" \
    "v_mad_i64_i32 v[250:251], vcc, v170, v188, v[250:251]\n" \
    "v_mad_i64_i32 v[248:249], vcc, v170, v198, v[248:249]\n" \
    "v_mad_i64_i32 v[250:251], vcc, v184, v198, v[250:251]\n" \
    "v_mad_i64_i32 v[248:249], vcc, v175, v188, v[248:249]\n" \
    "v_mad_i64_i32 v[250:251], vcc, v171, v195, v[250:251]\n" \
    "v_mad_i64_i32 v[248:249], vcc, v171, v204, v[248:249]\n" \
    "v_mad_i64_i32 v[250:251], vcc, v185, v204, v[250:251]\n" \
    "v_mad_i64_i32 v[248:249], vcc, v176, v195, v[248:249]\n" \
    "v_mad_i64_i32 v[250:251], vcc, v172, v194, v[250:251]\n" \
    "v_mad_i64_i32 v[248:249], vcc, v172, v203, v[248:249]\n" \
    "v_mad_i64_i32 v[250:251], vcc, v186, v203, v[250:251]\n" \
    "v_mad_i64_i32 v[248:249], vcc, v177, v194, v[248:249]\n" \
    "v_and_b32_e64 v194, %91, v250\n" \
    "v_ashrrev_i64 v[250:251], 26, v[250:251]\n" \
    "v_and_b32_e64 v196, %91, v248\n" \
    "v_ashrrev_i64 v[248:249], 26, v[248:249]\n" \
    "v_mad_i64_i32 v[250:251], vcc, v168, v191, v[250:251]\n" \
    "v_mad_i64_i32 v[248:249], vcc, v168, v201, v[248:249]\n" \
    "v_mad_i64_i32 v[250:251], vcc, v182, v201, v[250:251]\n" \
    "v_mad_i64_i32 v[248:249], vcc, v173, v191, v[248:249]\n" \
    "v_mad_i64_i32 v[250:251], vcc, v169, v190, v[250:251]\n" \
    "v_mad_i64_i32 v[248:249], vcc, v169, v200, v[248:249]\n" \
    "v_mad_i64_i32 v[250:251], vcc, v183, v200, v[250:251]\n" \
    "v_mad_i64_i32 v[248:249], vcc, v174, v190, v[248:249]\n" \
    "v_mad_i64_i32 v[250:251], vcc, v170, v189, v[250:251]\n" \
    "v_mad_i64_i32 v[248:249], vcc, v170, v199, v[248:249]\n" \
    "v_mad_i64_i32 v[250:251], vcc, v184, v199, v[250:251]\n" \
    "v_mad_i64_i32 v[248:249], vcc, v175, v189, v[248:249]\n" \
    "v_mad_i64_i32 v[250:251], vcc, v171, v188, v[250:251]\n" \
    "v_mad_i64_i32 v[248:249], vcc, v171, v198, v[248:249]\n" \
    "v_mad_i64_i32 v[250:251], vcc, v185, v198, v[250:251]\n" \
    "v_mad_i64_i32 v[248:249], vcc, v176, v188, v[248:249]\n" \
    "v_mad_i64_i32 v[250:251], vcc, v172, v195, v[250:251]\n" \
    "v_mad_i64_i32 v[248:249], vcc, v172, v204, v[248:249]\n" \
    "v_mad_i64_i32 v[250:251], vcc, v186, v204, v[250:251]\n" \
    "v_mad_i64_i32 v[248:249], vcc, v177, v195, v[248:249]\n" \
    "v_and_b32_e64 v195, %91, v250\n" \
    "v_ashrrev_i64 v[250:251], 26, v[250:251]\n" \
    "v_and_b32_e64 v197, %91, v248\n" \
    "v_ashrrev_i64 v[248:249], 26, v[248:249]\n" \
    "v_mad_i64_i32 v[250:251], vcc, v168, v192, v[250:251]\n" \
    "v_mad_i64_i32 v[248:249], vcc, v168, v202, v[248:249]\n" \
    "v_mad_i64_i32 v[250:251], vcc, v182, v202, v[250:251]\n" \
    "v_mad_i64_i32 v[248:249], vcc, v173, v192, v[248:249]\n" \
    "v_mad_i64_i32 v[250:251], vcc, v169, v191, v[250:251]\n" \
    "v_mad_i64_i32 v[248:249], vcc, v169, v201, v[248:249]\n" \
    "v_mad_i64_i32 v[250:251], vcc, v183, v201, v[250:251]\n" \
    "v_mad_i64_i32 v[248:249], vcc, v174, v191, v[248:249]\n" \
    "v_mad_i64_i32 v[250:251], vcc, v170, v190, v[250:251]\n" \
    "v_mad_i64_i32 v[248:249], vcc, v170, v200, v[248:249]\n" \
    "v_mad_i64_i32 v[250:251], vcc, v184, v200, v[250:251]\n" \
    "v_mad_i64_i32 v[248:249], vcc, v175, v190, v[248:249]\n" \
    "v_mad_i64_i32 v[250:251], vcc, v171, v189, v[250:251]\n" \
    "v_mad_i64_i32 v[248:249], vcc, v171, v199, v[248:249]\n" \
    "v_mad_i64_i32 v[250:251], vcc, v185, v199, v[250:251]\n" \
    "v_mad_i64_i32 v[248:249], vcc, v176, v189, v[248:249]\n" \
    "v_mad_i64_i32 v[250:251], vcc, v172, v188, v[250:251]\n" \
    "v_mad_i64_i32 v[248:249], vcc, v172, v198, v[248:249]\n" \
    "v_mad_i64_i32 v[250:251], vcc, v186, v198, v[250:251]\n" \
    "v_mad_i64_i32 v[248:249], vcc, v177, v188, v[248:249]\n" \
    "v_and_b32_e64 v168, %91, v250\n" \
    "v_ashrrev_i64 v[250:251], 26, v[250:251]\n" \
    "v_and_b32_e64 v169, %91, v248\n" \
    "v_ashrrev_i64 v[248:249], 26, v[248:249]\n" \
    "v_lshl_add_u64 v[250:251], v[250:251], 3, v[254:255]\n" \
    "v_lshl_add_u64 v[248:249], v[248:249], 3, v[252:253]\n" \
    "v_and_b32_e64 v170, %91, v250\n" \
    "v_alignbit_b32 v171, v251, v250, 26\n" \
    "v_add_u32_e32 v187, v187, v171\n" \
    "v_and_b32_e32 v171, %91, v248\n" \
    "v_alignbit_b32 v172, v249, v248, 26\n" \
    "v_add_u32_e32 v193, v193, v172\n" \
    "v_sub_u32_e32 v172, 0, v213\n" \
    "v_sub_u32_e32 v173, 0, v214\n" \
    "v_sub_u32_e32 v174, 0, v215\n" \
    "v_sub_u32_e32 v175, 0, v216\n" \
    "v_sub_u32_e32 v176, 0, v217\n" \
    "v_lshlrev_b32_e32 v177, 3, v234\n" \
    "v_lshlrev_b32_e32 v182, 3, v236\n" \
    "v_lshlrev_b32_e32 v183, 3, v238\n" \
    "v_lshlrev_b32_e32 v184, 3, v240\n" \
    "v_lshlrev_b32_e32 v185, 3, v235\n" \
    "v_lshlrev_b32_e32 v186, 3, v237\n" \
    "v_lshlrev_b32_e32 v188, 3, v239\n" \
    "v_lshlrev_b32_e32 v189, 3, v241\n" \
    "v_mad_i64_i32 v[250:251], vcc, v208, v242, 0\n" \
    "v_mad_i64_i32 v[248:249], vcc, v208, v243, 0\n" \
    "v_mad_i64_i32 v[250:251], vcc, v172, v243, v[250:251]\n" \
    "v_mad_i64_i32 v[248:249], vcc, v213, v242, v[248:249]\n" \
    "v_mad_i64_i32 v[250:251], vcc, v209, v184, v[250:251]\n" \
    "v_mad_i64_i32 v[248:249], vcc, v209, v189, v[248:249]\n" \
    "v_mad_i64_i32 v[250:251], vcc, v173, v189, v[250:251]\n" \
    "v_mad_i64_i32 v[248:249], vcc, v214, v184, v[248:249]\n" \
    "v_mad_i64_i32 v[250:251], vcc, v210, v183, v[250:251]\n" \
    "v_mad_i64_i32 v[248:249], vcc, v210, v188, v[248:249]\n" \
    "v_mad_i64_i32 v[250:251], vcc, v174, v188, v[250:251]\n" \
    "v_mad_i64_i32 v[248:249], vcc, v215, v183, v[248:249]\n" \
    "v_mad_i64_i32 v[250:251], vcc, v211, v182, v[250:251]\n" \
    "v_mad_i64_i32 v[248:249], vcc, v211, v186, v[248:249]\n" \
    "v_mad_i64_i32 v[250:251], vcc, v175, v186, v[250:251]\n" \
    "v_mad_i64_i32 v[248:249], vcc, v216, v182, v[248:249]\n" \
    "v_mad_i64_i32 v[250:251], vcc, v212, v177, v[250:251]\n" \
    "v_mad_i64_i32 v[248:249], vcc, v212, v185, v[248:249]\n" \
    "v_mad_i64_i32 v[250:251], vcc, v176, v185, v[250:251]\n" \
    "v_mad_i64_i32 v[248:249], vcc, v217, v177, v[248:249]\n" \
    "v_and_b32_e64 v254, %91, v250\n" \
    "v_ashrrev_i64 v[250:251], 26, v[250:251]\n" \
    "v_and_b32_e64 v252, %91, v248\n" \
    "v_ashrrev_i64 v[248:249], 26, v[248:249]\n" \
    "v_mad_i64_i32 v[250:251], vcc, v208, v234, v[250:251]\n" \
    "v_mad_i64_i32 v[248:249], vcc, v208, v235, v[248:249]\n" \
    "v_mad_i64_i32 v[250:251], vcc, v172, v235, v[250:251]\n" \
    "v_mad_i64_i32 v[248:249], vcc, v213, v234, v[248:249]\n" \
    "v_mad_i64_i32 v[250:251], vcc, v209, v242, v[250:251]\n" \
    "v_mad_i64_i32 v[248:249], vcc, v209, v243, v[248:249]\n" \
    "v_mad_i64_i32 v[250:251], vcc, v173, v243, v[250:251]\n" \
    "v_mad_i64_i32 v[248:249], vcc, v214, v242, v[248:249]\n" \
    "v_mad_i64_i32 v[250:251], vcc, v210, v184, v[250:251]\n" \
    "v_mad_i64_i32 v[248:249], vcc, v210, v189, v[248:249]\n" \
    "v_mad_i64_i32 v[250:251], vcc, v174, v189, v[250:251]\n" \
    "v_mad_i64_i32 v[248:249], vcc, v215, v184, v[248:249]\n" \
    "v_mad_i64_i32 v[250:251], vcc, v211, v183, v[250:251]\n" \
    "v_mad_i64_i32 v[248:249], vcc, v211, v188, v[248:249]\n" \
    "v_mad_i64_i32 v[250:251], vcc, v175, v188, v[250:251]\n" \
    "v_mad_i64_i32 v[248:249], vcc, v216, v183, v[248:249]\n" \
    "v_mad_i64_i32 v[250:251], vcc, v212, v182, v[250:251]\n" \
    "v_mad_i64_i32 v[248:249], vcc, v212, v186, v[248:249]\n" \
    "v_mad_i64_i32 v[250:251], vcc, v176, v186, v[250:251]\n" \
    "v_mad_i64_i32 v[248:249], vcc, v217, v182, v[248:249]\n" \
    "v_and_b32_e64 v177, %91, v250\n" \
    "v_ashrrev_i64 v[250:251], 26, v[250:251]\n" \
    "v_and_b32_e64 v182, %91, v248\n" \
    "v_ashrrev_i64 v[248:249], 26, v[248:249]\n" \
    "v_mad_i64_i32 v[250:251], vcc, v208, v236, v[250:251]\n" \
    "v_mad_i64_i32 v[248:249], vcc, v208, v237, v[248:249]\n" \
    "v_mad_i64_i32 v[250:251], vcc, v172, v237, v[250:251]\n" \
    "v_mad_i64_i32 v[248:249], vcc, v213, v236, v[248:249]\n" \
    "v_mad_i64_i32 v[250:251], vcc, v209, v234, v[250:251]\n" \
    "v_mad_i64_i32 v[248:249], vcc, v209, v235, v[248:249]\n" \
    "v_mad_i64_i32 v[250:251], vcc, v173, v235, v[250:251]\n" \
    "v_mad_i64_i32 v[248:249], vcc, v214, v234, v[248:249]\n" \
    "v_mad_i64_i32 v[250:251], vcc, v210, v242, v[250:251]\n" \
    "v_mad_i64_i32 v[248:249], vcc, v210, v243, v[248:249]\n" \
    "v_mad_i64_i32 v[250:251], vcc, v174, v243, v[250:251]\n" \
    "v_mad_i64_i32 v[248:249], vcc, v215, v242, v[248:249]\n" \
    "v_mad_i64_i32 v[250:251], vcc, v211, v184, v[250:251]\n" \
    "v_mad_i64_i32 v[248:249], vcc, v211, v189, v[248:249]\n" \
    "v_mad_i64_i32 v[250:251], vcc, v175, v189, v[250:251]\n" \
    "v_mad_i64_i32 v[248:249], vcc, v216, v184, v[248:249]\n" \
    "v_mad_i64_i32 v[250:251], vcc, v212, v183, v[250:251]\n" \
    "v_mad_i64_i32 v[248:249], vcc, v212, v188, v[248:249]\n" \
    "v_mad_i64_i32 v[250:251], vcc, v176, v188, v[250:251]\n" \
    "v_mad_i64_i32 v[248:249], vcc, v217, v183, v[248:249]\n" \
    "v_and_b32_e64 v183, %91, v250\n" \
    "v_ashrrev_i64 v[250:251], 26, v[250:251]\n" \
    "v_and_b32_e64 v185, %91, v248\n" \
    "v_ashrrev_i64 v[248:249], 26, v[248:249]\n" \
    "v_mad_i64_i32 v[250:251], vcc, v208, v238, v[250:251]\n" \
    "v_mad_i64_i32 v[248:249], vcc, v208, v239, v[248:249]\n" \
    "v_mad_i64_i32 v[250:251], vcc, v172, v239, v[250:251]\n" \
    "v_mad_i64_i32 v[248:249], vcc, v213, v238, v[248:249]\n" \
    "v_mad_i64_i32 v[250:251], vcc, v209, v236, v[250:251]\n" \
    "v_mad_i64_i32 v[248:249], vcc, v209, v237, v[248:249]\n" \
    "v_mad_i64_i32 v[250:251], vcc, v173, v237, v[250:251]\n" \
    "v_mad_i64_i32 v[248:249], vcc, v214, v236, v[248:249]\n" \
    "v_mad_i64_i32 v[250:251], vcc, v210, v234, v[250:251]\n" \
    "v_mad_i64_i32 v[248:249], vcc, v210, v235, v[248:249]\n" \
    "v_mad_i64_i32 v[250:251], vcc, v174, v235, v[250:251]\n" \
    "v_mad_i64_i32 v[248:249], vcc, v215, v234, v[248:249]\n" \
    "v_mad_i64_i32 v[250:251], vcc, v211, v242, v[250:251]\n" \
    "v_mad_i64_i32 v[248:249], vcc, v211, v243, v[248:249]\n" \
    "v_mad_i64_i32 v[250:251], vcc, v175, v243, v[250:251]\n" \
    "v_mad_i64_i32 v[248:249], vcc, v216, v242, v[248:249]\n" \
    "v_mad_i64_i32 v[250:251], vcc, v212, v184, v[250:251]\n" \
    "v_mad_i64_i32 v[248:249], vcc, v212, v189, v[248:249]\n" \
    "v_mad_i64_i32 v[250:251], vcc, v176, v189, v[250:251]\n" \
    "v_mad_i64_i32 v[248:249], vcc, v217, v184, v[248:249]\n" \
    "v_and_b32_e64 v184, %91, v250\n" \
    "v_ashrrev_i64 v[250:251], 26, v[250:251]\n" \
    "v_and_b32_e64 v186, %91, v248\n" \
    "v_ashrrev_i64 v[248:249], 26, v[248:249]\n" \
    "v_mad_i64_i32 v[250:251], vcc, v208, v240, v[250:251]\n" \
    "v_mad_i64_i32 v[248:249], vcc, v208, v241, v[248:249]\n" \
    "v_mad_i64_i32 v[250:251], vcc, v172, v241, v[250:251]\n" \
    "v_mad_i64_i32 v[248:249], vcc, v213, v240, v[248:249]\n" \
    "v_mad_i64_i32 v[250:251], vcc, v209, v238, v[250:251]\n" \
    "v_mad_i64_i32 v[248:249], vcc, v209, v239, v[248:249]\n" \
    "v_mad_i64_i32 v[250:251], vcc, v173, v239, v[250:251]\n" \
    "v_mad_i64_i32 v[248:249], vcc, v214, v238, v[248:249]\n" \
    "v_mad_i64_i32 v[250:251], vcc, v210, v236, v[250:251]\n" \
    "v_mad_i64_i32 v[248:249], vcc, v210, v237, v[248:249]\n" \
    "v_mad_i64_i32 v[250:251], vcc, v174, v237, v[250:251]\n" \
    "v_mad_i64_i32 v[248:249], vcc, v215, v236, v[248:249]\n" \
    "v_mad_i64_i32 v[250:251], vcc, v211, v234, v[250:251]\n" \
    "v_mad_i64_i32 v[248:249], vcc, v211, v235, v[248:249]\n" \
    "v_mad_i64_i32 v[250:251], vcc, v175, v235, v[250:251]\n" \
    "v_mad_i64_i32 v[248:249], vcc, v216, v234, v[248:249]\n" \
    "v_mad_i64_i32 v[250:251], vcc, v212, v242, v[250:251]\n" \
    "v_mad_i64_i32 v[248:249], vcc, v212, v243, v[248:249]\n" \
    "v_mad_i64_i32 v[250:251], vcc, v176, v243, v[250:251]\n" \
    "v_mad_i64_i32 v[248:249], vcc, v217, v242, v[248:249]\n" \
    "v_and_b32_e64 v172, %91, v250\n" \
    "v_ashrrev_i64 v[250:251], 26, v[250:251]\n" \
    "v_and_b32_e64 v173, %91, v248\n" \
    "v_ashrrev_i64 v[248:249], 26, v[248:249]\n" \
    "v_lshl_add_u64 v[250:251], v[250:251], 3, v[254:255]\n" \
    "v_lshl_add_u64 v[248:249], v[248:249], 3, v[252:253]\n" \
    "v_and_b32_e64 v174, %91, v250\n" \
    "v_alignbit_b32 v175, v251, v250, 26\n" \
    "v_add_u32_e32 v177, v177, v175\n" \
    "v_and_b32_e32 v175, %91, v248\n" \
    "v_alignbit_b32 v176, v249, v248, 26\n" \
    "v_add_u32_e32 v182, v182, v176\n" \
    "v_sub_u32_e32 v176, 0, %75\n" \
    "v_sub_u32_e32 v188, 0, %76\n" \
    "v_sub_u32_e32 v189, 0, %77\n" \
    "v_sub_u32_e32 v190, 0, %78\n" \
    "v_sub_u32_e32 v191, 0, %79\n" \
    "v_lshlrev_b32_e32 v192, 3, %21\n" \
    "v_lshlrev_b32_e32 v198, 3, %22\n" \
    "v_lshlrev_b32_e32 v199, 3, %23\n" \
    "v_lshlrev_b32_e32 v200, 3, %24\n" \
    "v_lshlrev_b32_e32 v201, 3, %26\n" \
    "v_lshlrev_b32_e32 v202, 3, %27\n" \
    "v_lshlrev_b32_e32 v203, 3, %28\n" \
    "v_lshlrev_b32_e32 v204, 3, %29\n" \
    "v_mad_i64_i32 v[250:251], vcc, %70, %20, 0\n" \
    "v_mad_i64_i32 v[248:249], vcc, %70, %25, 0\n" \
    "v_mad_i64_i32 v[250:251], vcc, v176, %25, v[250:251]\n" \
    "v_mad_i64_i32 v[248:249], vcc, %75, %20, v[248:249]\n" \
    "v_mad_i64_i32 v[250:251], vcc, %71, v200, v[250:251]\n" \
    "v_mad_i64_i32 v[248:249], vcc, %71, v204, v[248:249]\n" \
    "v_mad_i64_i32 v[250:251], vcc, v188, v204, v[250:251]\n" \
    "v_mad_i64_i32 v[248:249], vcc, %76, v200, v[248:249]\n" \
    "v_mad_i64_i32 v[250:251], vcc, %72, v199, v[250:251]\n" \
    "v_mad_i64_i32 v[248:249], vcc, %72, v203, v[248:249]\n" \
    "v_mad_i64_i32 v[250:251], vcc, v189, v203, v[250:251]\n" \
    "v_mad_i64_i32 v[248:249], vcc, %77, v199, v[248:249]\n" \
    "v_mad_i64_i32 v[250:251], vcc, %73, v198, v[250:251]\n" \
    "v_mad_i64_i32 v[248:249], vcc, %73, v202, v[248:249]\n" \
    "v_mad_i64_i32 v[250:251], vcc, v190, v202, v[250:251]\n" \
    "v_mad_i64_i32 v[248:249], vcc, %78, v198, v[248:249]\n" \
    "v_mad_i64_i32 v[250:251], vcc, %74, v192, v[250:251]\n" \
    "v_mad_i64_i32 v[248:249], vcc, %74, v201, v[248:249]\n" \
    "v_mad_i64_i32 v[250:251], vcc, v191, v201, v[250:251]\n" \
    "v_mad_i64_i32 v[248:249], vcc, %79, v192, v[248:249]\n" \
    "v_and_b32_e64 v254, %91, v250\n" \
    "v_ashrrev_i64 v[250:251], 26, v[250:251]\n" \
    "v_and_b32_e64 v252, %91, v248\n" \
    "v_ashrrev_i64 v[248:249], 26, v[248:249]\n" \
    "v_mad_i64_i32 v[250:251], vcc, %70, %21, v[250:251]\n" \
    "v_mad_i64_i32 v[248:249], vcc, %70, %26, v[248:249]\n" \
    "v_mad_i64_i32 v[250:251], vcc, v176, %26, v[250:251]\n" \
    "v_mad_i64_i32 v[248:249], vcc, %75, %21, v[248:249]\n" \
    "v_mad_i64_i32 v[250:251], vcc, %71, %20, v[250:251]\n" \
    "v_mad_i64_i32 v[248:249], vcc, %71, %25, v[248:249]\n" \
    "v_mad_i64_i32 v[250:251], vcc, v188, %25, v[250:251]\n" \
    "v_mad_i64_i32 v[248:249], vcc, %76, %20, v[248:249]\n" \
    "v_mad_i64_i32 v[250:251], vcc, %72, v200, v[250:251]\n" \
    "v_mad_i64_i32 v[248:249], vcc, %72, v204, v[248:249]\n" \
    "v_mad_i64_i32 v[250:251], vcc, v189, v204, v[250:251]\n" \
    "v_mad_i64_i32 v[248:249], vcc, %77, v200, v[248:249]\n" \
    "v_mad_i64_i32 v[250:251], vcc, %73, v199, v[250:251]\n" \
    "v_mad_i64_i32 v[248:249], vcc, %73, v203, v[248:249]\n" \
    "v_mad_i64_i32 v[250:251], vcc, v190, v203, v[250:251]\n" \
    "v_mad_i64_i32 v[248:249], vcc, %78, v199, v[248:249]\n" \
    "v_mad_i64_i32 v[250:251], vcc, %74, v198, v[250:251]\n" \
    "v_mad_i64_i32 v[248:249], vcc, %74, v202, v[248:249]\n" \
    "v_mad_i64_i32 v[250:251], vcc, v191, v202, v[250:251]\n" \
    "v_mad_i64_i32 v[248:249], vcc, %79, v198, v[248:249]\n" \
    "v_and_b32_e64 v192, %91, v250\n" \
    "v_ashrrev_i64 v[250:251], 26, v[250:251]\n" \
    "v_and_b32_e64 v198, %91, v248\n" \
    "v_ashrrev_i64 v[248:249], 26, v[248:249]\n" \
    "v_mad_i64_i32 v[250:251], vcc, %70, %22, v[250:251]\n" \
    "v_mad_i64_i32 v[248:249], vcc, %70, %27, v[248:249]\n" \
    "v_mad_i64_i32 v[250:251], vcc, v176, %27, v[250:251]\n" \
    "v_mad_i64_i32 v[248:249], vcc, %75, %22, v[248:249]\n" \
    "v_mad_i64_i32 v[250:251], vcc, %71, %21, v[250:251]\n" \
    "v_mad_i64_i32 v[248:249], vcc, %71, %26, v[248:249]\n" \
    "v_mad_i64_i32 v[250:251], vcc, v188, %26, v[250:251]\n" \
    "v_mad_i64_i32 v[248:249], vcc, %76, %21, v[248:249]\n" \
    "v_mad_i64_i32 v[250:251], vcc, %72, %20, v[250:251]\n" \
    "v_mad_i64_i32 v[248:249], vcc, %72, %25, v[248:249]\n" \
// ... 9572 lines not shown
```

### fourq_amd/csrc/recode.hip.h

```cpp
#pragma once
#include "fp127.hip.h"

namespace fq {

typedef unsigned __int128 u128;

FQ_DEV u64 mul_shift256(const u64 a[4], const u64 m[4]) {
    u64 w0, w1, w2, w3, w4;
    u128 t;
    t = (u128)a[0] * m[0];                       w0 = (u64)t;
    t = (u128)a[0] * m[1] + (u64)(t >> 64);      w1 = (u64)t;
    t = (u128)a[0] * m[2] + (u64)(t >> 64);      w2 = (u64)t;
    t = (u128)a[0] * m[3] + (u64)(t >> 64);      w3 = (u64)t; w4 = (u64)(t >> 64);
    t = (u128)a[1] * m[0] + w1;                  w1 = (u64)t;
    t = (u128)a[1] * m[1] + w2 + (u64)(t >> 64); w2 = (u64)t;
    t = (u128)a[1] * m[2] + w3 + (u64)(t >> 64); w3 = (u64)t;
    w4 += a[1] * m[3] + (u64)(t >> 64);
    t = (u128)a[2] * m[0] + w2;                  w2 = (u64)t;
    t = (u128)a[2] * m[1] + w3 + (u64)(t >> 64); w3 = (u64)t;
    w4 += a[2] * m[2] + (u64)(t >> 64);
    t = (u128)a[3] * m[0] + w3;                  w3 = (u64)t;
    w4 += a[3] * m[1] + (u64)(t >> 64);
    (void)w0; (void)w1; (void)w2; (void)w3;
    return w4;
}

FQ_DEV void decompose(const u64 m[4], u64 v[4]) {
    u64 t[4];
#pragma unroll
    for (int i = 0; i < 4; i++) {
        u64 ell[4] = { ELL[i][0], ELL[i][1], ELL[i][2], ELL[i][3] };
        t[i] = mul_shift256(ell, m);
    }
    u64 ac[4], acp[4];
#pragma unroll
    for (int i = 0; i < 4; i++) {
        u64 a = (i == 0) ? m[0] : 0;
#pragma unroll
        for (int j = 0; j < 4; j++) a -= t[j] * BASIS[j][i];
        ac[i] = a + OFFSET_C[i];
        acp[i] = a + OFFSET_CP[i];
    }
    u64 mask = (u64)0 - (ac[0] & 1);
#pragma unroll
    for (int i = 0; i < 4; i++) v[i] = acp[i] ^ (mask & (ac[i] ^ acp[i]));
}

struct EndoDigits {
    u64 sign;
    u64 d[3];
    u32 top;
};
FQ_DEV EndoDigits recode(const u64 vin[4]) {
    EndoDigits r;
    r.sign = vin[0] >> 1;
    u64 v1 = vin[1], v2 = vin[2], v3 = vin[3];
    u64 p1 = 0, p2 = 0, p3 = 0;
    u64 s = r.sign;
#pragma unroll 1
    for (int i = 0; i < 64; i++) {
        u64 nb1 = ~(s >> i) & 1;
        u64 b;
        b = v1 & 1; p1 |= b << i; v1 = (v1 >> 1) + (nb1 & b);
        b = v2 & 1; p2 |= b << i; v2 = (v2 >> 1) + (nb1 & b);
        b = v3 & 1; p3 |= b << i; v3 = (v3 >> 1) + (nb1 & b);
    }
    r.d[0] = p1; r.d[1] = p2; r.d[2] = p3;
    r.top = (u32)(v1 + 2 * v2 + 4 * v3);
    return r;
}
struct EndoNibbles {
    u32 w[8];
    u32 top;
};
FQ_DEV EndoNibbles recode_nibbles(const u64 vin[4]) {
    EndoNibbles r;
    u64 s = vin[0] >> 1;
    u64 v1 = vin[1], v2 = vin[2], v3 = vin[3];
#pragma unroll
    for (int t = 0; t < 8; t++) r.w[t] = 0;
#pragma unroll 1
    for (int k = 0; k < 8; k++) {
        u32 w = 0;
#pragma unroll
        for (int j = 0; j < 8; j++) {
            const u32 nb1 = ~(u32)s & 1;
            s >>= 1;
            const u32 b1 = (u32)v1 & 1, b2 = (u32)v2 & 1, b3 = (u32)v3 & 1;
            v1 = (v1 >> 1) + (nb1 & b1);
            v2 = (v2 >> 1) + (nb1 & b2);
            v3 = (v3 >> 1) + (nb1 & b3);
            w = (w >> 4) | ((b1 | (b2 << 1) | (b3 << 2) | (nb1 << 3)) << 28);
        }
#pragma unroll
        for (int t = 0; t < 7; t++) r.w[t] = r.w[t + 1];
        r.w[7] = w;
    }
    r.top = (u32)(v1 + 2 * v2 + 4 * v3);
    return r;
}
FQ_DEV u32 endo_digit(const EndoDigits& e, int i) {
    return (u32)((e.d[0] >> i) & 1) | ((u32)((e.d[1] >> i) & 1) << 1) | ((u32)((e.d[2] >> i) & 1) << 2);
}
FQ_DEV u32 endo_neg_mask(const EndoDigits& e, int i) {
    return (u32)((e.sign >> i) & 1) - 1u;
}

struct WinScalar {
    u64 r[4];
};
FQ_DEV bool ge256(const u64 a[4], const u64 b[4]) {
    bool ge = true;
#pragma unroll
    for (int i = 0; i < 4; i++) ge = (a[i] == b[i]) ? ge : (a[i] > b[i]);
    return ge;
}
FQ_DEV WinScalar win_reduce(const u64 m[4]) {
    u64 r[4] = { m[0], m[1], m[2], m[3] };
#pragma unroll 1
    for (int k = 10; k >= 0; k--) {
        u64 s[4];
        s[0] = ORDER_N[0] << k;
#pragma unroll
        for (int i = 1; i < 4; i++) s[i] = (ORDER_N[i] << k) | (k ? (ORDER_N[i - 1] >> (64 - k)) : 0);
        u64 keep = ge256(r, s) ? ~(u64)0 : 0;
        u64 borrow = 0;
#pragma unroll
        for (int i = 0; i < 4; i++) {
            u64 si = s[i] & keep;
            u64 d1 = r[i] - si;
            u64 b1 = r[i] < si;
            u64 d2 = d1 - borrow;
            u64 b2 = d1 < borrow;
            r[i] = d2; borrow = b1 | b2;
        }
    }
    u64 addn = (r[0] & 1) ? 0 : ~(u64)0;
    u64 carry = 0;
#pragma unroll
    for (int i = 0; i < 4; i++) {
        u64 ni = ORDER_N[i] & addn;
        u64 s1 = r[i] + ni;
        u64 c1 = s1 < ni;
        u64 s2 = s1 + carry;
        u64 c2 = s2 < carry;
        r[i] = s2; carry = c1 | c2;
    }
    WinScalar w; w.r[0] = r[0]; w.r[1] = r[1]; w.r[2] = r[2]; w.r[3] = r[3];
    return w;
}
FQ_DEV u32 win_code_from_window(u32 w5) {
    u32 w = (w5 & 31) | 1;
    u32 pos = w >> 4;
    u32 ind = ((pos ? w : ~w) & 15) >> 1;
    return (pos << 3) | ind;
}
FQ_DEV u32 win_window(const WinScalar& w, int i) {
    int bit = 4 * i, word = bit >> 6, off = bit & 63;
    u64 lo = (word == 0) ? w.r[0] : (word == 1) ? w.r[1] : (word == 2) ? w.r[2] : w.r[3];
    u64 hi = (word == 0) ? w.r[1] : (word == 1) ? w.r[2] : (word == 2) ? w.r[3] : 0;
    u64 v = lo >> off;
    if (off > 59) v |= hi << (64 - off);
    return (u32)v & 31;
}
FQ_DEV u32 win_top_code(const WinScalar& w) {
    u32 d = (u32)(w.r[3] >> 60) | 1;
    return (1u << 3) | (((d - 1) >> 1) & 7);
}

template <int W_, int V_, int E_> struct CombShape {
    static constexpr int W = W_, V = V_, E = E_, D = V_ * E_, BLOCK_POINTS = 1 << (W_ - 1), POINTS = V_ << (W_ - 1);
    static_assert(W_ * V_ * E_ >= 250 && V_ * E_ <= 64, "comb shape");
};
typedef CombShape<9, 4, 7> CombFast;
typedef CombShape<5, 5, 10> CombScan;
constexpr int COMB_POINTS_ALL = CombFast::POINTS + CombScan::POINTS;
template <typename S> struct CombDigits {
    typedef typename std::conditional<(S::D <= 32), u32, u64>::type plane_t;
    plane_t plane[S::W];
    u32 negate;
};
template <typename S> FQ_DEV CombDigits<S> comb_recode(const u64 m[4]) {
    constexpr int COMB_W = S::W, COMB_D = S::D;
    WinScalar red = win_reduce(m);
    u64 k[4] = { red.r[0], red.r[1], red.r[2], red.r[3] };
    u64 n[4] = { ORDER_N[0], ORDER_N[1], ORDER_N[2], ORDER_N[3] };
    const bool was_even = ge256(k, n);
    u64 twoN[4], alt[4];
    twoN[0] = n[0] << 1; twoN[1] = (n[1] << 1) | (n[0] >> 63); twoN[2] = (n[2] << 1) | (n[1] >> 63); twoN[3] = (n[3] << 1) | (n[2] >> 63);
    u64 borrow = 0;
#pragma unroll
    for (int i = 0; i < 4; i++) {
        u64 d1 = twoN[i] - k[i], b1 = twoN[i] < k[i];
        u64 d2 = d1 - borrow, b2 = d1 < borrow;
        alt[i] = d2; borrow = b1 | b2;
    }
    CombDigits<S> c;
    c.negate = was_even ? ~0u : 0u;
#pragma unroll
    for (int i = 0; i < 4; i++) k[i] = was_even ? alt[i] : k[i];
    const u64 mask_d = (1ull << COMB_D) - 1;
    const u64 sign = ((k[0] >> 1) & (mask_d >> 1)) | (1ull << (COMB_D - 1));
    typedef typename CombDigits<S>::plane_t plane_t;
    c.plane[0] = (plane_t)sign;
    u64 c0 = (k[0] >> COMB_D) | (k[1] << (64 - COMB_D)), c1 = (k[1] >> COMB_D) | (k[2] << (64 - COMB_D));
    u64 c2 = (k[2] >> COMB_D) | (k[3] << (64 - COMB_D)), c3 = k[3] >> COMB_D;
    const plane_t neg = (plane_t)(~sign & mask_d);
#pragma unroll
    for (int r = 1; r < COMB_W; r++) {
        const plane_t low = (plane_t)(c0 & mask_d);
        plane_t T = low;
#pragma unroll 4
        for (int i = 0; i < COMB_D; i++) T = (plane_t)((low + (plane_t)((T & neg) << 1)) & (plane_t)mask_d);
        c.plane[r] = T;
        const u64 up = (u64)(T & neg) << 1, down = (u64)T;
        u64 s0 = c0 + up, cy = s0 < up;
        u64 s1 = c1 + cy; cy = s1 < cy;
        u64 s2 = c2 + cy; cy = s2 < cy;
        u64 s3 = c3 + cy;
        u64 t0 = s0 - down, bw = s0 < down;
        u64 t1 = s1 - bw; bw = s1 < bw;
        u64 t2 = s2 - bw; bw = s2 < bw;
        u64 t3 = s3 - bw;
        c0 = (t0 >> COMB_D) | (t1 << (64 - COMB_D)); c1 = (t1 >> COMB_D) | (t2 << (64 - COMB_D));
        c2 = (t2 >> COMB_D) | (t3 << (64 - COMB_D)); c3 = t3 >> COMB_D;
    }
    return c;
}
template <typename S> FQ_DEV u32 comb_index(const CombDigits<S>& c, int col) {
    u32 idx = 0;
#pragma unroll
    for (int r = 1; r < S::W; r++) idx |= (u32)((c.plane[r] >> col) & 1) << (r - 1);
    return idx;
}
template <typename S> FQ_DEV u32 comb_neg_mask(const CombDigits<S>& c, int col) { return (u32)((c.plane[0] >> col) & 1) - 1u; }
template <typename S> FQ_DEV void comb_point_scalar(u32 t, u64 m[4]) {
    const u32 j = t >> (S::W - 1), u = t & ((1u << (S::W - 1)) - 1);
    m[0] = m[1] = m[2] = m[3] = 0;
    auto set_bit = [&](int bit) { m[bit >> 6] |= 1ull << (bit & 63); };
    set_bit(S::E * j);
    for (int r = 0; r < S::W - 1; r++) if ((u >> r) & 1) set_bit(S::E * j + (r + 1) * S::D);
}

}
```

### include/fourq_amd.h

```cpp
#ifndef FOURQ_AMD_H
#define FOURQ_AMD_H

#include <stddef.h>
#include <stdint.h>

#ifdef __cplusplus
extern "C" {
#endif

#define FOURQ_OK 0
#define FOURQ_ERR_INVALID (-1)
#define FOURQ_ERR_NODEVICE (-2)
#define FOURQ_ERR_NOMEM (-3)
#define FOURQ_ERR_HIP (-4)

#define FOURQ_DH_OK 0
#define FOURQ_DH_NOT_ON_CURVE 1
#define FOURQ_DH_NEUTRAL 2

#define FOURQ_MAX_BATCH 0xffffff00u
#define FOURQ_BYTES_DECODE_BASE 16

#define FOURQ_SCALAR_WORDS 4
#define FOURQ_AFFINE_WORDS 8
// ... 112 lines not shown
int fourq_comb_mul_batch(fourq_ctx *ctx, const uint64_t *scalars, const uint64_t *comb, uint64_t *out_affine, uint8_t *status, size_t n);
int fourq_comb_mul_batch_dev(fourq_ctx *ctx, const uint64_t *scalars, const uint64_t *comb, uint64_t *out_affine, uint8_t *status, size_t n);
int fourq_dh_exchange_comb_batch(fourq_ctx *ctx, const uint64_t *a_scalars, const uint64_t *b_scalars, const uint64_t *comb,
                                 uint64_t *out_affine, uint8_t *status, size_t n);
int fourq_dh_exchange_comb_batch_dev(fourq_ctx *ctx, const uint64_t *a_scalars, const uint64_t *b_scalars, const uint64_t *comb,
                                     uint64_t *out_affine, uint8_t *status, size_t n);

int fourq_double_mul_affine_batch(fourq_ctx *ctx, const uint64_t *k_scalars, const uint64_t *comb, const uint64_t *l_scalars,
                                  const uint64_t *points_affine, uint64_t *out_affine, size_t n);
int fourq_double_mul_affine_batch_dev(fourq_ctx *ctx, const uint64_t *k_scalars, const uint64_t *comb, const uint64_t *l_scalars,
                                      const uint64_t *points_affine, uint64_t *out_affine, size_t n);
int fourq_double_mul_bytes_batch(fourq_ctx *ctx, const uint64_t *k_scalars, const uint64_t *comb, const uint64_t *l_scalars,
                                 const uint8_t *points32, uint8_t *out32, uint8_t *status, size_t n);
int fourq_double_mul_bytes_batch_dev(fourq_ctx *ctx, const uint64_t *k_scalars, const uint64_t *comb, const uint64_t *l_scalars,
                                     const uint8_t *points32, uint8_t *out32, uint8_t *status, size_t n);
int fourq_verify_bytes_batch(fourq_ctx *ctx, const uint64_t *k_scalars, const uint64_t *comb, const uint64_t *l_scalars,
                             const uint8_t *points32, const uint8_t *expect32, uint8_t *ok, uint8_t *status, size_t n);
int fourq_verify_bytes_batch_dev(fourq_ctx *ctx, const uint64_t *k_scalars, const uint64_t *comb, const uint64_t *l_scalars,
                                 const uint8_t *points32, const uint8_t *expect32, uint8_t *ok, uint8_t *status, size_t n);

#define FOURQ_SIG_S_RANGE 32
#define FOURQ_SIG_MSG_CLAMPED 64
#define FOURQ_SIG_MAX_MSG (1u << 20)
int fourq_sha512_batch(fourq_ctx *ctx, const uint8_t *msgs, size_t stride, const uint32_t *lens, size_t msg_len, uint8_t *out64, size_t n);
int fourq_sha512_batch_dev(fourq_ctx *ctx, const uint8_t *msgs, size_t stride, const uint32_t *lens, size_t msg_len, uint8_t *out64, size_t n);
int fourq_sig_keygen_batch(fourq_ctx *ctx, const uint8_t *sk32, const uint64_t *comb, uint8_t *pk32, size_t n);
int fourq_sig_keygen_batch_dev(fourq_ctx *ctx, const uint8_t *sk32, const uint64_t *comb, uint8_t *pk32, size_t n);
int fourq_sig_sign_batch(fourq_ctx *ctx, const uint8_t *sk32, const uint8_t *pk32, const uint64_t *comb,
                         const uint8_t *msgs, size_t stride, const uint32_t *lens, size_t msg_len, uint8_t *sig64, size_t n);
int fourq_sig_sign_batch_dev(fourq_ctx *ctx, const uint8_t *sk32, const uint8_t *pk32, const uint64_t *comb,
                             const uint8_t *msgs, size_t stride, const uint32_t *lens, size_t msg_len, uint8_t *sig64, size_t n);
int fourq_sig_verify_batch(fourq_ctx *ctx, const uint8_t *pk32, const uint64_t *comb,
                           const uint8_t *msgs, size_t stride, const uint32_t *lens, size_t msg_len,
                           const uint8_t *sig64, uint8_t *ok, uint8_t *status, size_t n);
int fourq_sig_verify_batch_dev(fourq_ctx *ctx, const uint8_t *pk32, const uint64_t *comb,
                               const uint8_t *msgs, size_t stride, const uint32_t *lens, size_t msg_len,
                               const uint8_t *sig64, uint8_t *ok, uint8_t *status, size_t n);

#define FOURQ_H2C_RO 0
#define FOURQ_H2C_NU 1
#define FOURQ_H2C_MAX_DST 255
int fourq_hash_to_field_batch(fourq_ctx *ctx, const uint8_t *dst, size_t dst_len, int mode,
                              const uint8_t *msgs, size_t stride, const uint32_t *lens, size_t msg_len, uint64_t *out_u, size_t n);
int fourq_hash_to_field_batch_dev(fourq_ctx *ctx, const uint8_t *dst, size_t dst_len, int mode,
                                  const uint8_t *msgs, size_t stride, const uint32_t *lens, size_t msg_len, uint64_t *out_u, size_t n);
int fourq_map_to_curve_batch(fourq_ctx *ctx, const uint64_t *u, uint64_t *out_affine, size_t n);
int fourq_map_to_curve_batch_dev(fourq_ctx *ctx, const uint64_t *u, uint64_t *out_affine, size_t n);
int fourq_hash_to_curve_batch(fourq_ctx *ctx, const uint8_t *dst, size_t dst_len, int mode,
                              const uint8_t *msgs, size_t stride, const uint32_t *lens, size_t msg_len, uint8_t *out32, size_t n);
int fourq_hash_to_curve_batch_dev(fourq_ctx *ctx, const uint8_t *dst, size_t dst_len, int mode,
                                  const uint8_t *msgs, size_t stride, const uint32_t *lens, size_t msg_len, uint8_t *out32, size_t n);
int fourq_hash_to_curve_affine_batch(fourq_ctx *ctx, const uint8_t *dst, size_t dst_len, int mode,
                                     const uint8_t *msgs, size_t stride, const uint32_t *lens, size_t msg_len, uint64_t *out_affine, size_t n);
int fourq_hash_to_curve_affine_batch_dev(fourq_ctx *ctx, const uint8_t *dst, size_t dst_len, int mode,
                                         const uint8_t *msgs, size_t stride, const uint32_t *lens, size_t msg_len, uint64_t *out_affine, size_t n);

enum fourq_prim {
    FOURQ_FP_ADD = 0, FOURQ_FP_SUB = 1, FOURQ_FP_MUL = 2, FOURQ_FP_SQR = 3, FOURQ_FP_NEG = 4, FOURQ_FP_INV = 5,
    FOURQ_FP_INVSQRT = 6,
    FOURQ_FP_SELECT = 7, FOURQ_FP2_SELECT = 23,
    FOURQ_FP2_ADD = 16, FOURQ_FP2_SUB = 17, FOURQ_FP2_MUL = 18, FOURQ_FP2_SQR = 19, FOURQ_FP2_NEG = 20,
    FOURQ_FP2_CONJ = 21, FOURQ_FP2_INV = 22,
    FOURQ_PT_DBL = 32,
    FOURQ_PT_ADD = 33,
    FOURQ_PT_ADD_CORE = 34,
    FOURQ_PT_R1TOR2 = 35,
    FOURQ_PT_R1TOR3 = 36,
    FOURQ_PT_R2TOR4 = 37,
    FOURQ_PT_TAU = 38,
    FOURQ_PT_TAU_DUAL = 39,
    FOURQ_PT_UPSILON = 40,
    FOURQ_PT_CHI = 41,
    FOURQ_PT_PHI = 42,
    FOURQ_PT_PSI = 43,
    FOURQ_PT_ON_CURVE = 44,
    FOURQ_PT_COFACTOR392 = 45,
    FOURQ_PT_R1TOAFFINE = 46,
    FOURQ_PT_MAP_ELL2 = 47,
    FOURQ_SC_DECOMPOSE = 64,
    FOURQ_SC_RECODE = 65,
    FOURQ_SC_WINDOWED = 66,
    FOURQ_SC_REDUCE512 = 67,
    FOURQ_SC_MULSUB = 68,
    FOURQ_SC_MUL = 69
};
int fourq_prim_words(int op, size_t *in_words, size_t *out_words);
int fourq_prim_batch(fourq_ctx *ctx, int op, const uint64_t *in, uint64_t *out, size_t n);

#ifdef __cplusplus
}
#endif
#endif
```

Baseline: 220.7 million.

## Replace serial endomorphism recoding with closed-form carry planes and bit-transpose

The scalar recoding for the 4-dimensional GLV decomposition no longer walks 64 bits one at a time. It computes each digit plane in closed form as (v+n)^n, with the carry-out giving the top bits. The nibble-interleaved layout is then built with a butterfly bit-exchange transpose instead of a per-bit loop. Separately, the gfx950 ladder asm replaces the conditional-negation xor/sub pairs with v_xad_u32, which shortens the instruction stream and reassigns registers. A test primitive for the nibble recode is also added, and the header is made host-compilable.

```diff
diff --git a/fourq_amd/_lib.py b/fourq_amd/_lib.py
--- a/fourq_amd/_lib.py
+++ b/fourq_amd/_lib.py
@@ -130,7 +130,7 @@
     "PT_DBL": 32, "PT_ADD": 33, "PT_ADD_CORE": 34, "PT_R1TOR2": 35, "PT_R1TOR3": 36, "PT_R2TOR4": 37,
     "PT_TAU": 38, "PT_TAU_DUAL": 39, "PT_UPSILON": 40, "PT_CHI": 41, "PT_PHI": 42, "PT_PSI": 43,
     "PT_ON_CURVE": 44, "PT_COFACTOR392": 45, "PT_R1TOAFFINE": 46, "PT_MAP_ELL2": 47,
-    "SC_DECOMPOSE": 64, "SC_RECODE": 65, "SC_WINDOWED": 66, "SC_REDUCE512": 67, "SC_MULSUB": 68, "SC_MUL": 69,
+    "SC_DECOMPOSE": 64, "SC_RECODE": 65, "SC_WINDOWED": 66, "SC_REDUCE512": 67, "SC_MULSUB": 68, "SC_MUL": 69, "SC_RECODE_NIBBLES": 70,
 }
 
 
diff --git a/fourq_amd/csrc/fourq_amd.hip b/fourq_amd/csrc/fourq_amd.hip
--- a/fourq_amd/csrc/fourq_amd.hip
+++ b/fourq_amd/csrc/fourq_amd.hip
@@ -353,6 +353,13 @@
         y[0] = e.sign; y[1] = e.d[0]; y[2] = e.d[1]; y[3] = e.d[2]; y[4] = e.top;
         break;
     }
+    case FOURQ_SC_RECODE_NIBBLES: {
+        u64 v[4] = { x[0], x[1], x[2], x[3] };
+        EndoNibbles e = recode_nibbles(v);
+        for (int k = 0; k < 8; k++) y[k] = e.w[k];
+        y[8] = e.top;
+        break;
+    }
     case FOURQ_SC_WINDOWED: {
         u64 m[4] = { x[0], x[1], x[2], x[3] };
         WinScalar w = win_reduce(m);
@@ -377,7 +384,7 @@
     { FOURQ_PT_UPSILON, 12, 12 }, { FOURQ_PT_CHI, 12, 12 }, { FOURQ_PT_PHI, 20, 20 }, { FOURQ_PT_PSI, 20, 20 },
     { FOURQ_PT_ON_CURVE, 8, 1 }, { FOURQ_PT_COFACTOR392, 8, 20 }, { FOURQ_PT_R1TOAFFINE, 20, 8 },
     { FOURQ_PT_MAP_ELL2, 4, 8 },
-    { FOURQ_SC_DECOMPOSE, 4, 4 }, { FOURQ_SC_RECODE, 4, 5 }, { FOURQ_SC_WINDOWED, 4, 8 },
+    { FOURQ_SC_DECOMPOSE, 4, 4 }, { FOURQ_SC_RECODE, 4, 5 }, { FOURQ_SC_RECODE_NIBBLES, 4, 9 }, { FOURQ_SC_WINDOWED, 4, 8 },
     { FOURQ_SC_REDUCE512, 8, 4 }, { FOURQ_SC_MULSUB, 12, 4 }, { FOURQ_SC_MUL, 8, 4 },
 };
 const PrimShape* find_prim(int op) {
diff --git a/fourq_amd/csrc/ladder_asm_gfx950.inc b/fourq_amd/csrc/ladder_asm_gfx950.inc
--- a/fourq_amd/csrc/ladder_asm_gfx950.inc
+++ b/fourq_amd/csrc/ladder_asm_gfx950.inc
@@ -1938,27 +1938,18 @@
     "v_bitop3_b32 v205, %100, %67, %77 bitop3:0xca\n" \
     "v_bitop3_b32 v206, %100, %68, %78 bitop3:0xca\n" \
     "v_bitop3_b32 v207, %100, %69, %79 bitop3:0xca\n" \
-    "v_xor_b32_e32 v208, %100, %90\n" \
-    "v_xor_b32_e32 v209, %100, %91\n" \
-    "v_xor_b32_e32 v210, %100, %92\n" \
-    "v_xor_b32_e32 v211, %100, %93\n" \
-    "v_xor_b32_e32 v212, %100, %94\n" \
-    "v_sub_u32_e32 v208, v208, %100\n" \
-    "v_sub_u32_e32 v209, v209, %100\n" \
-    "v_sub_u32_e32 v210, v210, %100\n" \
-    "v_sub_u32_e32 v211, v211, %100\n" \
-    "v_sub_u32_e32 v212, v212, %100\n" \
-    "v_xor_b32_e32 v213, %100, %95\n" \
-    "v_xor_b32_e32 v214, %100, %96\n" \
-    "v_xor_b32_e32 v215, %100, %97\n" \
-    "v_xor_b32_e32 v216, %100, %98\n" \
-    "v_xor_b32_e32 v217, %100, %99\n" \
-    "v_sub_u32_e32 v213, v213, %100\n" \
-    "v_sub_u32_e32 v214, v214, %100\n" \
-    "v_sub_u32_e32 v215, v215, %100\n" \
-    "v_sub_u32_e32 v216, v216, %100\n" \
-    "v_sub_u32_e32 v217, v217, %100\n" \
-    "v_sub_u32_e32 v218, 0, v183\n" \
+    "v_sub_u32_e64 v208, 0, %100\n" \
+    "v_xad_u32 v209, %90, %100, v208\n" \
+    "v_xad_u32 v210, %91, %100, v208\n" \
+    "v_xad_u32 v211, %92, %100, v208\n" \
+    "v_xad_u32 v212, %93, %100, v208\n" \
+    "v_xad_u32 v213, %94, %100, v208\n" \
+    "v_xad_u32 v214, %95, %100, v208\n" \
+    "v_xad_u32 v215, %96, %100, v208\n" \
+    "v_xad_u32 v216, %97, %100, v208\n" \
+    "v_xad_u32 v217, %98, %100, v208\n" \
+    "v_xad_u32 v218, %99, %100, v208\n" \
+    "v_sub_u32_e32 v208, 0, v183\n" \
     "v_sub_u32_e32 v219, 0, v184\n" \
     "v_sub_u32_e32 v220, 0, v185\n" \
     "v_sub_u32_e32 v221, 0, v186\n" \
@@ -1973,7 +1964,7 @@
     "v_lshlrev_b32_e64 v230, 3, v207\n" \
     "v_mad_i64_i32 v[250:251], vcc, v178, v193, 0\n" \
     "v_mad_i64_i32 v[248:249], vcc, v178, v203, 0\n" \
-    "v_mad_i64_i32 v[250:251], vcc, v218, v203, v[250:251]\n" \
+    "v_mad_i64_i32 v[250:251], vcc, v208, v203, v[250:251]\n" \
     "v_mad_i64_i32 v[248:249], vcc, v183, v193, v[248:249]\n" \
     "v_mad_i64_i32 v[250:251], vcc, v179, v226, v[250:251]\n" \
     "v_mad_i64_i32 v[248:249], vcc, v179, v230, v[248:249]\n" \
@@ -1997,7 +1988,7 @@
     "v_ashrrev_i64 v[248:249], 26, v[248:249]\n" \
     "v_mad_i64_i32 v[250:251], vcc, v178, v194, v[250:251]\n" \
     "v_mad_i64_i32 v[248:249], vcc, v178, v204, v[248:249]\n" \
-    "v_mad_i64_i32 v[250:251], vcc, v218, v204, v[250:251]\n" \
+    "v_mad_i64_i32 v[250:251], vcc, v208, v204, v[250:251]\n" \
     "v_mad_i64_i32 v[248:249], vcc, v183, v194, v[248:249]\n" \
     "v_mad_i64_i32 v[250:251], vcc, v179, v193, v[250:251]\n" \
     "v_mad_i64_i32 v[248:249], vcc, v179, v203, v[248:249]\n" \
@@ -2021,7 +2012,7 @@
     "v_ashrrev_i64 v[248:249], 26, v[248:249]\n" \
     "v_mad_i64_i32 v[250:251], vcc, v178, v195, v[250:251]\n" \
     "v_mad_i64_i32 v[248:249], vcc, v178, v205, v[248:249]\n" \
-    "v_mad_i64_i32 v[250:251], vcc, v218, v205, v[250:251]\n" \
+    "v_mad_i64_i32 v[250:251], vcc, v208, v205, v[250:251]\n" \
     "v_mad_i64_i32 v[248:249], vcc, v183, v195, v[248:249]\n" \
     "v_mad_i64_i32 v[250:251], vcc, v179, v194, v[250:251]\n" \
     "v_mad_i64_i32 v[248:249], vcc, v179, v204, v[248:249]\n" \
@@ -2045,7 +2036,7 @@
     "v_ashrrev_i64 v[248:249], 26, v[248:249]\n" \
     "v_mad_i64_i32 v[250:251], vcc, v178, v196, v[250:251]\n" \
     "v_mad_i64_i32 v[248:249], vcc, v178, v206, v[248:249]\n" \
-    "v_mad_i64_i32 v[250:251], vcc, v218, v206, v[250:251]\n" \
+    "v_mad_i64_i32 v[250:251], vcc, v208, v206, v[250:251]\n" \
     "v_mad_i64_i32 v[248:249], vcc, v183, v196, v[248:249]\n" \
     "v_mad_i64_i32 v[250:251], vcc, v179, v195, v[250:251]\n" \
     "v_mad_i64_i32 v[248:249], vcc, v179, v205, v[248:249]\n" \
@@ -2069,7 +2060,7 @@
     "v_ashrrev_i64 v[248:249], 26, v[248:249]\n" \
     "v_mad_i64_i32 v[250:251], vcc, v178, v197, v[250:251]\n" \
     "v_mad_i64_i32 v[248:249], vcc, v178, v207, v[248:249]\n" \
-    "v_mad_i64_i32 v[250:251], vcc, v218, v207, v[250:251]\n" \
+    "v_mad_i64_i32 v[250:251], vcc, v208, v207, v[250:251]\n" \
     "v_mad_i64_i32 v[248:249], vcc, v183, v197, v[248:249]\n" \
     "v_mad_i64_i32 v[250:251], vcc, v179, v196, v[250:251]\n" \
     "v_mad_i64_i32 v[248:249], vcc, v179, v206, v[248:249]\n" \
@@ -2240,11 +2231,11 @@
     "v_and_b32_e32 v171, %101, v248\n" \
     "v_alignbit_b32 v172, v249, v248, 26\n" \
     "v_add_u32_e32 v193, v193, v172\n" \
-    "v_sub_u32_e32 v172, 0, v213\n" \
-    "v_sub_u32_e32 v173, 0, v214\n" \
-    "v_sub_u32_e32 v174, 0, v215\n" \
-    "v_sub_u32_e32 v175, 0, v216\n" \
-    "v_sub_u32_e32 v176, 0, v217\n" \
+    "v_sub_u32_e32 v172, 0, v214\n" \
+    "v_sub_u32_e32 v173, 0, v215\n" \
+    "v_sub_u32_e32 v174, 0, v216\n" \
+    "v_sub_u32_e32 v175, 0, v217\n" \
+    "v_sub_u32_e32 v176, 0, v218\n" \
     "v_lshlrev_b32_e32 v177, 3, %51\n" \
     "v_lshlrev_b32_e32 v182, 3, %52\n" \
     "v_lshlrev_b32_e32 v183, 3, %53\n" \
@@ -2253,122 +2244,122 @@
     "v_lshlrev_b32_e32 v186, 3, %57\n" \
     "v_lshlrev_b32_e32 v188, 3, %58\n" \
     "v_lshlrev_b32_e32 v189, 3, %59\n" \
-    "v_mad_i64_i32 v[250:251], vcc, v208, %50, 0\n" \
-    "v_mad_i64_i32 v[248:249], vcc, v208, %55, 0\n" \
+    "v_mad_i64_i32 v[250:251], vcc, v209, %50, 0\n" \
+    "v_mad_i64_i32 v[248:249], vcc, v209, %55, 0\n" \
     "v_mad_i64_i32 v[250:251], vcc, v172, %55, v[250:251]\n" \
-    "v_mad_i64_i32 v[248:249], vcc, v213, %50, v[248:249]\n" \
-    "v_mad_i64_i32 v[250:251], vcc, v209, v184, v[250:251]\n" \
-    "v_mad_i64_i32 v[248:249], vcc, v209, v189, v[248:249]\n" \
-    "v_mad_i64_i32 v[250:251], vcc, v173, v189, v[250:251]\n" \
-    "v_mad_i64_i32 v[248:249], vcc, v214, v184, v[248:249]\n" \
-    "v_mad_i64_i32 v[250:251], vcc, v210, v183, v[250:251]\n" \
-    "v_mad_i64_i32 v[248:249], vcc, v210, v188, v[248:249]\n" \
-    "v_mad_i64_i32 v[250:251], vcc, v174, v188, v[250:251]\n" \
-    "v_mad_i64_i32 v[248:249], vcc, v215, v183, v[248:249]\n" \
-    "v_mad_i64_i32 v[250:251], vcc, v211, v182, v[250:251]\n" \
-    "v_mad_i64_i32 v[248:249], vcc, v211, v186, v[248:249]\n" \
-    "v_mad_i64_i32 v[250:251], vcc, v175, v186, v[250:251]\n" \
-    "v_mad_i64_i32 v[248:249], vcc, v216, v182, v[248:249]\n" \
-    "v_mad_i64_i32 v[250:251], vcc, v212, v177, v[250:251]\n" \
-    "v_mad_i64_i32 v[248:249], vcc, v212, v185, v[248:249]\n" \
-    "v_mad_i64_i32 v[250:251], vcc, v176, v185, v[250:251]\n" \
-    "v_mad_i64_i32 v[248:249], vcc, v217, v177, v[248:249]\n" \
-    "v_and_b32_e64 v254, %101, v250\n" \
-    "v_ashrrev_i64 v[250:251], 26, v[250:251]\n" \
-    "v_and_b32_e64 v252, %101, v248\n" \
-    "v_ashrrev_i64 v[248:249], 26, v[248:249]\n" \
-    "v_mad_i64_i32 v[250:251], vcc, v208, %51, v[250:251]\n" \
-    "v_mad_i64_i32 v[248:249], vcc, v208, %56, v[248:249]\n" \
-    "v_mad_i64_i32 v[250:251], vcc, v172, %56, v[250:251]\n" \
-    "v_mad_i64_i32 v[248:249], vcc, v213, %51, v[248:249]\n" \
-    "v_mad_i64_i32 v[250:251], vcc, v209, %50, v[250:251]\n" \
-    "v_mad_i64_i32 v[248:249], vcc, v209, %55, v[248:249]\n" \
-    "v_mad_i64_i32 v[250:251], vcc, v173, %55, v[250:251]\n" \
     "v_mad_i64_i32 v[248:249], vcc, v214, %50, v[248:249]\n" \
     "v_mad_i64_i32 v[250:251], vcc, v210, v184, v[250:251]\n" \
     "v_mad_i64_i32 v[248:249], vcc, v210, v189, v[248:249]\n" \
-    "v_mad_i64_i32 v[250:251], vcc, v174, v189, v[250:251]\n" \
+    "v_mad_i64_i32 v[250:251], vcc, v173, v189, v[250:251]\n" \
     "v_mad_i64_i32 v[248:249], vcc, v215, v184, v[248:249]\n" \
     "v_mad_i64_i32 v[250:251], vcc, v211, v183, v[250:251]\n" \
     "v_mad_i64_i32 v[248:249], vcc, v211, v188, v[248:249]\n" \
-    "v_mad_i64_i32 v[250:251], vcc, v175, v188, v[250:251]\n" \
+    "v_mad_i64_i32 v[250:251], vcc, v174, v188, v[250:251]\n" \
     "v_mad_i64_i32 v[248:249], vcc, v216, v183, v[248:249]\n" \
     "v_mad_i64_i32 v[250:251], vcc, v212, v182, v[250:251]\n" \
     "v_mad_i64_i32 v[248:249], vcc, v212, v186, v[248:249]\n" \
-    "v_mad_i64_i32 v[250:251], vcc, v176, v186, v[250:251]\n" \
+    "v_mad_i64_i32 v[250:251], vcc, v175, v186, v[250:251]\n" \
     "v_mad_i64_i32 v[248:249], vcc, v217, v182, v[248:249]\n" \
-    "v_and_b32_e64 v177, %101, v250\n" \
-    "v_ashrrev_i64 v[250:251], 26, v[250:251]\n" \
-    "v_and_b32_e64 v182, %101, v248\n" \
-    "v_ashrrev_i64 v[248:249], 26, v[248:249]\n" \
-    "v_mad_i64_i32 v[250:251], vcc, v208, %52, v[250:251]\n" \
-    "v_mad_i64_i32 v[248:249], vcc, v208, %57, v[248:249]\n" \
-    "v_mad_i64_i32 v[250:251], vcc, v172, %57, v[250:251]\n" \
-    "v_mad_i64_i32 v[248:249], vcc, v213, %52, v[248:249]\n" \
+    "v_mad_i64_i32 v[250:251], vcc, v213, v177, v[250:251]\n" \
+    "v_mad_i64_i32 v[248:249], vcc, v213, v185, v[248:249]\n" \
+    "v_mad_i64_i32 v[250:251], vcc, v176, v185, v[250:251]\n" \
+    "v_mad_i64_i32 v[248:249], vcc, v218, v177, v[248:249]\n" \
+    "v_and_b32_e64 v254, %101, v250\n" \
+    "v_ashrrev_i64 v[250:251], 26, v[250:251]\n" \
+    "v_and_b32_e64 v252, %101, v248\n" \
+    "v_ashrrev_i64 v[248:249], 26, v[248:249]\n" \
     "v_mad_i64_i32 v[250:251], vcc, v209, %51, v[250:251]\n" \
     "v_mad_i64_i32 v[248:249], vcc, v209, %56, v[248:249]\n" \
-    "v_mad_i64_i32 v[250:251], vcc, v173, %56, v[250:251]\n" \
+    "v_mad_i64_i32 v[250:251], vcc, v172, %56, v[250:251]\n" \
     "v_mad_i64_i32 v[248:249], vcc, v214, %51, v[248:249]\n" \
     "v_mad_i64_i32 v[250:251], vcc, v210, %50, v[250:251]\n" \
     "v_mad_i64_i32 v[248:249], vcc, v210, %55, v[248:249]\n" \
-    "v_mad_i64_i32 v[250:251], vcc, v174, %55, v[250:251]\n" \
+    "v_mad_i64_i32 v[250:251], vcc, v173, %55, v[250:251]\n" \
     "v_mad_i64_i32 v[248:249], vcc, v215, %50, v[248:249]\n" \
     "v_mad_i64_i32 v[250:251], vcc, v211, v184, v[250:251]\n" \
     "v_mad_i64_i32 v[248:249], vcc, v211, v189, v[248:249]\n" \
-    "v_mad_i64_i32 v[250:251], vcc, v175, v189, v[250:251]\n" \
+    "v_mad_i64_i32 v[250:251], vcc, v174, v189, v[250:251]\n" \
     "v_mad_i64_i32 v[248:249], vcc, v216, v184, v[248:249]\n" \
     "v_mad_i64_i32 v[250:251], vcc, v212, v183, v[250:251]\n" \
     "v_mad_i64_i32 v[248:249], vcc, v212, v188, v[248:249]\n" \
-    "v_mad_i64_i32 v[250:251], vcc, v176, v188, v[250:251]\n" \
+    "v_mad_i64_i32 v[250:251], vcc, v175, v188, v[250:251]\n" \
     "v_mad_i64_i32 v[248:249], vcc, v217, v183, v[248:249]\n" \
-    "v_and_b32_e64 v183, %101, v250\n" \
-    "v_ashrrev_i64 v[250:251], 26, v[250:251]\n" \
-    "v_and_b32_e64 v185, %101, v248\n" \
-    "v_ashrrev_i64 v[248:249], 26, v[248:249]\n" \
-    "v_mad_i64_i32 v[250:251], vcc, v208, %53, v[250:251]\n" \
-    "v_mad_i64_i32 v[248:249], vcc, v208, %58, v[248:249]\n" \
-    "v_mad_i64_i32 v[250:251], vcc, v172, %58, v[250:251]\n" \
-    "v_mad_i64_i32 v[248:249], vcc, v213, %53, v[248:249]\n" \
+    "v_mad_i64_i32 v[250:251], vcc, v213, v182, v[250:251]\n" \
+    "v_mad_i64_i32 v[248:249], vcc, v213, v186, v[248:249]\n" \
+    "v_mad_i64_i32 v[250:251], vcc, v176, v186, v[250:251]\n" \
+    "v_mad_i64_i32 v[248:249], vcc, v218, v182, v[248:249]\n" \
+    "v_and_b32_e64 v177, %101, v250\n" \
+    "v_ashrrev_i64 v[250:251], 26, v[250:251]\n" \
+    "v_and_b32_e64 v182, %101, v248\n" \
+    "v_ashrrev_i64 v[248:249], 26, v[248:249]\n" \
     "v_mad_i64_i32 v[250:251], vcc, v209, %52, v[250:251]\n" \
     "v_mad_i64_i32 v[248:249], vcc, v209, %57, v[248:249]\n" \
-    "v_mad_i64_i32 v[250:251], vcc, v173, %57, v[250:251]\n" \
+    "v_mad_i64_i32 v[250:251], vcc, v172, %57, v[250:251]\n" \
     "v_mad_i64_i32 v[248:249], vcc, v214, %52, v[248:249]\n" \
     "v_mad_i64_i32 v[250:251], vcc, v210, %51, v[250:251]\n" \
     "v_mad_i64_i32 v[248:249], vcc, v210, %56, v[248:249]\n" \
-    "v_mad_i64_i32 v[250:251], vcc, v174, %56, v[250:251]\n" \
+    "v_mad_i64_i32 v[250:251], vcc, v173, %56, v[250:251]\n" \
     "v_mad_i64_i32 v[248:249], vcc, v215, %51, v[248:249]\n" \
     "v_mad_i64_i32 v[250:251], vcc, v211, %50, v[250:251]\n" \
     "v_mad_i64_i32 v[248:249], vcc, v211, %55, v[248:249]\n" \
-    "v_mad_i64_i32 v[250:251], vcc, v175, %55, v[250:251]\n" \
+    "v_mad_i64_i32 v[250:251], vcc, v174, %55, v[250:251]\n" \
     "v_mad_i64_i32 v[248:249], vcc, v216, %50, v[248:249]\n" \
     "v_mad_i64_i32 v[250:251], vcc, v212, v184, v[250:251]\n" \
     "v_mad_i64_i32 v[248:249], vcc, v212, v189, v[248:249]\n" \
-    "v_mad_i64_i32 v[250:251], vcc, v176, v189, v[250:251]\n" \
+    "v_mad_i64_i32 v[250:251], vcc, v175, v189, v[250:251]\n" \
     "v_mad_i64_i32 v[248:249], vcc, v217, v184, v[248:249]\n" \
-    "v_and_b32_e64 v184, %101, v250\n" \
-    "v_ashrrev_i64 v[250:251], 26, v[250:251]\n" \
-    "v_and_b32_e64 v186, %101, v248\n" \
-    "v_ashrrev_i64 v[248:249], 26, v[248:249]\n" \
-    "v_mad_i64_i32 v[250:251], vcc, v208, %54, v[250:251]\n" \
-    "v_mad_i64_i32 v[248:249], vcc, v208, %59, v[248:249]\n" \
-    "v_mad_i64_i32 v[250:251], vcc, v172, %59, v[250:251]\n" \
-    "v_mad_i64_i32 v[248:249], vcc, v213, %54, v[248:249]\n" \
+    "v_mad_i64_i32 v[250:251], vcc, v213, v183, v[250:251]\n" \
+    "v_mad_i64_i32 v[248:249], vcc, v213, v188, v[248:249]\n" \
+    "v_mad_i64_i32 v[250:251], vcc, v176, v188, v[250:251]\n" \
+    "v_mad_i64_i32 v[248:249], vcc, v218, v183, v[248:249]\n" \
+    "v_and_b32_e64 v183, %101, v250\n" \
+    "v_ashrrev_i64 v[250:251], 26, v[250:251]\n" \
+    "v_and_b32_e64 v185, %101, v248\n" \
+    "v_ashrrev_i64 v[248:249], 26, v[248:249]\n" \
     "v_mad_i64_i32 v[250:251], vcc, v209, %53, v[250:251]\n" \
     "v_mad_i64_i32 v[248:249], vcc, v209, %58, v[248:249]\n" \
-    "v_mad_i64_i32 v[250:251], vcc, v173, %58, v[250:251]\n" \
+    "v_mad_i64_i32 v[250:251], vcc, v172, %58, v[250:251]\n" \
     "v_mad_i64_i32 v[248:249], vcc, v214, %53, v[248:249]\n" \
     "v_mad_i64_i32 v[250:251], vcc, v210, %52, v[250:251]\n" \
     "v_mad_i64_i32 v[248:249], vcc, v210, %57, v[248:249]\n" \
-    "v_mad_i64_i32 v[250:251], vcc, v174, %57, v[250:251]\n" \
+    "v_mad_i64_i32 v[250:251], vcc, v173, %57, v[250:251]\n" \
     "v_mad_i64_i32 v[248:249], vcc, v215, %52, v[248:249]\n" \
     "v_mad_i64_i32 v[250:251], vcc, v211, %51, v[250:251]\n" \
     "v_mad_i64_i32 v[248:249], vcc, v211, %56, v[248:249]\n" \
-    "v_mad_i64_i32 v[250:251], vcc, v175, %56, v[250:251]\n" \
+    "v_mad_i64_i32 v[250:251], vcc, v174, %56, v[250:251]\n" \
     "v_mad_i64_i32 v[248:249], vcc, v216, %51, v[248:249]\n" \
     "v_mad_i64_i32 v[250:251], vcc, v212, %50, v[250:251]\n" \
     "v_mad_i64_i32 v[248:249], vcc, v212, %55, v[248:249]\n" \
+    "v_mad_i64_i32 v[250:251], vcc, v175, %55, v[250:251]\n" \
+    "v_mad_i64_i32 v[248:249], vcc, v217, %50, v[248:249]\n" \
+    "v_mad_i64_i32 v[250:251], vcc, v213, v184, v[250:251]\n" \
+    "v_mad_i64_i32 v[248:249], vcc, v213, v189, v[248:249]\n" \
+    "v_mad_i64_i32 v[250:251], vcc, v176, v189, v[250:251]\n" \
+    "v_mad_i64_i32 v[248:249], vcc, v218, v184, v[248:249]\n" \
+    "v_and_b32_e64 v184, %101, v250\n" \
+    "v_ashrrev_i64 v[250:251], 26, v[250:251]\n" \
+    "v_and_b32_e64 v186, %101, v248\n" \
+    "v_ashrrev_i64 v[248:249], 26, v[248:249]\n" \
+    "v_mad_i64_i32 v[250:251], vcc, v209, %54, v[250:251]\n" \
+    "v_mad_i64_i32 v[248:249], vcc, v209, %59, v[248:249]\n" \
+    "v_mad_i64_i32 v[250:251], vcc, v172, %59, v[250:251]\n" \
+    "v_mad_i64_i32 v[248:249], vcc, v214, %54, v[248:249]\n" \
+    "v_mad_i64_i32 v[250:251], vcc, v210, %53, v[250:251]\n" \
+    "v_mad_i64_i32 v[248:249], vcc, v210, %58, v[248:249]\n" \
+    "v_mad_i64_i32 v[250:251], vcc, v173, %58, v[250:251]\n" \
+    "v_mad_i64_i32 v[248:249], vcc, v215, %53, v[248:249]\n" \
+    "v_mad_i64_i32 v[250:251], vcc, v211, %52, v[250:251]\n" \
+    "v_mad_i64_i32 v[248:249], vcc, v211, %57, v[248:249]\n" \
+    "v_mad_i64_i32 v[250:251], vcc, v174, %57, v[250:251]\n" \
+    "v_mad_i64_i32 v[248:249], vcc, v216, %52, v[248:249]\n" \
+    "v_mad_i64_i32 v[250:251], vcc, v212, %51, v[250:251]\n" \
+    "v_mad_i64_i32 v[248:249], vcc, v212, %56, v[248:249]\n" \
+    "v_mad_i64_i32 v[250:251], vcc, v175, %56, v[250:251]\n" \
+    "v_mad_i64_i32 v[248:249], vcc, v217, %51, v[248:249]\n" \
+    "v_mad_i64_i32 v[250:251], vcc, v213, %50, v[250:251]\n" \
+    "v_mad_i64_i32 v[248:249], vcc, v213, %55, v[248:249]\n" \
     "v_mad_i64_i32 v[250:251], vcc, v176, %55, v[250:251]\n" \
-    "v_mad_i64_i32 v[248:249], vcc, v217, %50, v[248:249]\n" \
+    "v_mad_i64_i32 v[248:249], vcc, v218, %50, v[248:249]\n" \
     "v_and_b32_e64 v172, %101, v250\n" \
     "v_ashrrev_i64 v[250:251], 26, v[250:251]\n" \
     "v_and_b32_e64 v173, %101, v248\n" \
@@ -4023,27 +4014,18 @@
     "v_bitop3_b32 v205, %90, %57, %67 bitop3:0xca\n" \
     "v_bitop3_b32 v206, %90, %58, %68 bitop3:0xca\n" \
     "v_bitop3_b32 v207, %90, %59, %69 bitop3:0xca\n" \
-    "v_xor_b32_e32 v208, %90, %80\n" \
-    "v_xor_b32_e32 v209, %90, %81\n" \
-    "v_xor_b32_e32 v210, %90, %82\n" \
-    "v_xor_b32_e32 v211, %90, %83\n" \
-    "v_xor_b32_e32 v212, %90, %84\n" \
-    "v_sub_u32_e32 v208, v208, %90\n" \
-    "v_sub_u32_e32 v209, v209, %90\n" \
-    "v_sub_u32_e32 v210, v210, %90\n" \
-    "v_sub_u32_e32 v211, v211, %90\n" \
-    "v_sub_u32_e32 v212, v212, %90\n" \
-    "v_xor_b32_e32 v213, %90, %85\n" \
-    "v_xor_b32_e32 v214, %90, %86\n" \
-    "v_xor_b32_e32 v215, %90, %87\n" \
-    "v_xor_b32_e32 v216, %90, %88\n" \
-    "v_xor_b32_e32 v217, %90, %89\n" \
-    "v_sub_u32_e32 v213, v213, %90\n" \
-    "v_sub_u32_e32 v214, v214, %90\n" \
-    "v_sub_u32_e32 v215, v215, %90\n" \
-    "v_sub_u32_e32 v216, v216, %90\n" \
-    "v_sub_u32_e32 v217, v217, %90\n" \
-    "v_sub_u32_e32 v218, 0, v183\n" \
+    "v_sub_u32_e64 v208, 0, %90\n" \
+    "v_xad_u32 v209, %80, %90, v208\n" \
+    "v_xad_u32 v210, %81, %90, v208\n" \
+    "v_xad_u32 v211, %82, %90, v208\n" \
+    "v_xad_u32 v212, %83, %90, v208\n" \
+    "v_xad_u32 v213, %84, %90, v208\n" \
+    "v_xad_u32 v214, %85, %90, v208\n" \
+    "v_xad_u32 v215, %86, %90, v208\n" \
+    "v_xad_u32 v216, %87, %90, v208\n" \
+    "v_xad_u32 v217, %88, %90, v208\n" \
+    "v_xad_u32 v218, %89, %90, v208\n" \
+    "v_sub_u32_e32 v208, 0, v183\n" \
     "v_sub_u32_e32 v219, 0, v184\n" \
     "v_sub_u32_e32 v220, 0, v185\n" \
     "v_sub_u32_e32 v221, 0, v186\n" \
@@ -4058,7 +4040,7 @@
     "v_lshlrev_b32_e64 v230, 3, v207\n" \
     "v_mad_i64_i32 v[250:251], vcc, v178, v193, 0\n" \
     "v_mad_i64_i32 v[248:249], vcc, v178, v203, 0\n" \
-    "v_mad_i64_i32 v[250:251], vcc, v218, v203, v[250:251]\n" \
+    "v_mad_i64_i32 v[250:251], vcc, v208, v203, v[250:251]\n" \
     "v_mad_i64_i32 v[248:249], vcc, v183, v193, v[248:249]\n" \
     "v_mad_i64_i32 v[250:251], vcc, v179, v226, v[250:251]\n" \
     "v_mad_i64_i32 v[248:249], vcc, v179, v230, v[248:249]\n" \
@@ -4082,7 +4064,7 @@
     "v_ashrrev_i64 v[248:249], 26, v[248:249]\n" \
     "v_mad_i64_i32 v[250:251], vcc, v178, v194, v[250:251]\n" \
     "v_mad_i64_i32 v[248:249], vcc, v178, v204, v[248:249]\n" \
-    "v_mad_i64_i32 v[250:251], vcc, v218, v204, v[250:251]\n" \
+    "v_mad_i64_i32 v[250:251], vcc, v208, v204, v[250:251]\n" \
     "v_mad_i64_i32 v[248:249], vcc, v183, v194, v[248:249]\n" \
     "v_mad_i64_i32 v[250:251], vcc, v179, v193, v[250:251]\n" \
     "v_mad_i64_i32 v[248:249], vcc, v179, v203, v[248:249]\n" \
@@ -4106,7 +4088,7 @@
     "v_ashrrev_i64 v[248:249], 26, v[248:249]\n" \
     "v_mad_i64_i32 v[250:251], vcc, v178, v195, v[250:251]\n" \
     "v_mad_i64_i32 v[248:249], vcc, v178, v205, v[248:249]\n" \
-    "v_mad_i64_i32 v[250:251], vcc, v218, v205, v[250:251]\n" \
+    "v_mad_i64_i32 v[250:251], vcc, v208, v205, v[250:251]\n" \
     "v_mad_i64_i32 v[248:249], vcc, v183, v195, v[248:249]\n" \
     "v_mad_i64_i32 v[250:251], vcc, v179, v194, v[250:251]\n" \
     "v_mad_i64_i32 v[248:249], vcc, v179, v204, v[248:249]\n" \
@@ -4130,7 +4112,7 @@
     "v_ashrrev_i64 v[248:249], 26, v[248:249]\n" \
     "v_mad_i64_i32 v[250:251], vcc, v178, v196, v[250:251]\n" \
     "v_mad_i64_i32 v[248:249], vcc, v178, v206, v[248:249]\n" \
-    "v_mad_i64_i32 v[250:251], vcc, v218, v206, v[250:251]\n" \
+    "v_mad_i64_i32 v[250:251], vcc, v208, v206, v[250:251]\n" \
     "v_mad_i64_i32 v[248:249], vcc, v183, v196, v[248:249]\n" \
     "v_mad_i64_i32 v[250:251], vcc, v179, v195, v[250:251]\n" \
     "v_mad_i64_i32 v[248:249], vcc, v179, v205, v[248:249]\n" \
@@ -4154,7 +4136,7 @@
     "v_ashrrev_i64 v[248:249], 26, v[248:249]\n" \
     "v_mad_i64_i32 v[250:251], vcc, v178, v197, v[250:251]\n" \
     "v_mad_i64_i32 v[248:249], vcc, v178, v207, v[248:249]\n" \
-    "v_mad_i64_i32 v[250:251], vcc, v218, v207, v[250:251]\n" \
+    "v_mad_i64_i32 v[250:251], vcc, v208, v207, v[250:251]\n" \
     "v_mad_i64_i32 v[248:249], vcc, v183, v197, v[248:249]\n" \
     "v_mad_i64_i32 v[250:251], vcc, v179, v196, v[250:251]\n" \
     "v_mad_i64_i32 v[248:249], vcc, v179, v206, v[248:249]\n" \
@@ -4325,11 +4307,11 @@
     "v_and_b32_e32 v171, %91, v248\n" \
     "v_alignbit_b32 v172, v249, v248, 26\n" \
     "v_add_u32_e32 v193, v193, v172\n" \
-    "v_sub_u32_e32 v172, 0, v213\n" \
-    "v_sub_u32_e32 v173, 0, v214\n" \
-    "v_sub_u32_e32 v174, 0, v215\n" \
-    "v_sub_u32_e32 v175, 0, v216\n" \
-    "v_sub_u32_e32 v176, 0, v217\n" \
+    "v_sub_u32_e32 v172, 0, v214\n" \
+    "v_sub_u32_e32 v173, 0, v215\n" \
+    "v_sub_u32_e32 v174, 0, v216\n" \
+    "v_sub_u32_e32 v175, 0, v217\n" \
+    "v_sub_u32_e32 v176, 0, v218\n" \
     "v_lshlrev_b32_e32 v177, 3, v234\n" \
     "v_lshlrev_b32_e32 v182, 3, v236\n" \
     "v_lshlrev_b32_e32 v183, 3, v238\n" \
@@ -4338,122 +4320,122 @@
     "v_lshlrev_b32_e32 v186, 3, v237\n" \
     "v_lshlrev_b32_e32 v188, 3, v239\n" \
     "v_lshlrev_b32_e32 v189, 3, v241\n" \
-    "v_mad_i64_i32 v[250:251], vcc, v208, v242, 0\n" \
-    "v_mad_i64_i32 v[248:249], vcc, v208, v243, 0\n" \
+    "v_mad_i64_i32 v[250:251], vcc, v209, v242, 0\n" \
+    "v_mad_i64_i32 v[248:249], vcc, v209, v243, 0\n" \
     "v_mad_i64_i32 v[250:251], vcc, v172, v243, v[250:251]\n" \
-    "v_mad_i64_i32 v[248:249], vcc, v213, v242, v[248:249]\n" \
-    "v_mad_i64_i32 v[250:251], vcc, v209, v184, v[250:251]\n" \
-    "v_mad_i64_i32 v[248:249], vcc, v209, v189, v[248:249]\n" \
-    "v_mad_i64_i32 v[250:251], vcc, v173, v189, v[250:251]\n" \
-    "v_mad_i64_i32 v[248:249], vcc, v214, v184, v[248:249]\n" \
-    "v_mad_i64_i32 v[250:251], vcc, v210, v183, v[250:251]\n" \
-    "v_mad_i64_i32 v[248:249], vcc, v210, v188, v[248:249]\n" \
-    "v_mad_i64_i32 v[250:251], vcc, v174, v188, v[250:251]\n" \
-    "v_mad_i64_i32 v[248:249], vcc, v215, v183, v[248:249]\n" \
-    "v_mad_i64_i32 v[250:251], vcc, v211, v182, v[250:251]\n" \
-    "v_mad_i64_i32 v[248:249], vcc, v211, v186, v[248:249]\n" \
-    "v_mad_i64_i32 v[250:251], vcc, v175, v186, v[250:251]\n" \
-    "v_mad_i64_i32 v[248:249], vcc, v216, v182, v[248:249]\n" \
-    "v_mad_i64_i32 v[250:251], vcc, v212, v177, v[250:251]\n" \
-    "v_mad_i64_i32 v[248:249], vcc, v212, v185, v[248:249]\n" \
-    "v_mad_i64_i32 v[250:251], vcc, v176, v185, v[250:251]\n" \
-    "v_mad_i64_i32 v[248:249], vcc, v217, v177, v[248:249]\n" \
-    "v_and_b32_e64 v254, %91, v250\n" \
-    "v_ashrrev_i64 v[250:251], 26, v[250:251]\n" \
-    "v_and_b32_e64 v252, %91, v248\n" \
-    "v_ashrrev_i64 v[248:249], 26, v[248:249]\n" \
-    "v_mad_i64_i32 v[250:251], vcc, v208, v234, v[250:251]\n" \
-    "v_mad_i64_i32 v[248:249], vcc, v208, v235, v[248:249]\n" \
-    "v_mad_i64_i32 v[250:251], vcc, v172, v235, v[250:251]\n" \
-    "v_mad_i64_i32 v[248:249], vcc, v213, v234, v[248:249]\n" \
-    "v_mad_i64_i32 v[250:251], vcc, v209, v242, v[250:251]\n" \
-    "v_mad_i64_i32 v[248:249], vcc, v209, v243, v[248:249]\n" \
-    "v_mad_i64_i32 v[250:251], vcc, v173, v243, v[250:251]\n" \
     "v_mad_i64_i32 v[248:249], vcc, v214, v242, v[248:249]\n" \
     "v_mad_i64_i32 v[250:251], vcc, v210, v184, v[250:251]\n" \
     "v_mad_i64_i32 v[248:249], vcc, v210, v189, v[248:249]\n" \
-    "v_mad_i64_i32 v[250:251], vcc, v174, v189, v[250:251]\n" \
+    "v_mad_i64_i32 v[250:251], vcc, v173, v189, v[250:251]\n" \
     "v_mad_i64_i32 v[248:249], vcc, v215, v184, v[248:249]\n" \
     "v_mad_i64_i32 v[250:251], vcc, v211, v183, v[250:251]\n" \
     "v_mad_i64_i32 v[248:249], vcc, v211, v188, v[248:249]\n" \
-    "v_mad_i64_i32 v[250:251], vcc, v175, v188, v[250:251]\n" \
+    "v_mad_i64_i32 v[250:251], vcc, v174, v188, v[250:251]\n" \
     "v_mad_i64_i32 v[248:249], vcc, v216, v183, v[248:249]\n" \
     "v_mad_i64_i32 v[250:251], vcc, v212, v182, v[250:251]\n" \
     "v_mad_i64_i32 v[248:249], vcc, v212, v186, v[248:249]\n" \
-    "v_mad_i64_i32 v[250:251], vcc, v176, v186, v[250:251]\n" \
+    "v_mad_i64_i32 v[250:251], vcc, v175, v186, v[250:251]\n" \
     "v_mad_i64_i32 v[248:249], vcc, v217, v182, v[248:249]\n" \
-    "v_and_b32_e64 v177, %91, v250\n" \
-    "v_ashrrev_i64 v[250:251], 26, v[250:251]\n" \
-    "v_and_b32_e64 v182, %91, v248\n" \
-    "v_ashrrev_i64 v[248:249], 26, v[248:249]\n" \
-    "v_mad_i64_i32 v[250:251], vcc, v208, v236, v[250:251]\n" \
-    "v_mad_i64_i32 v[248:249], vcc, v208, v237, v[248:249]\n" \
-    "v_mad_i64_i32 v[250:251], vcc, v172, v237, v[250:251]\n" \
-    "v_mad_i64_i32 v[248:249], vcc, v213, v236, v[248:249]\n" \
+    "v_mad_i64_i32 v[250:251], vcc, v213, v177, v[250:251]\n" \
+    "v_mad_i64_i32 v[248:249], vcc, v213, v185, v[248:249]\n" \
+    "v_mad_i64_i32 v[250:251], vcc, v176, v185, v[250:251]\n" \
+    "v_mad_i64_i32 v[248:249], vcc, v218, v177, v[248:249]\n" \
+    "v_and_b32_e64 v254, %91, v250\n" \
+    "v_ashrrev_i64 v[250:251], 26, v[250:251]\n" \
+    "v_and_b32_e64 v252, %91, v248\n" \
+    "v_ashrrev_i64 v[248:249], 26, v[248:249]\n" \
     "v_mad_i64_i32 v[250:251], vcc, v209, v234, v[250:251]\n" \
     "v_mad_i64_i32 v[248:249], vcc, v209, v235, v[248:249]\n" \
-    "v_mad_i64_i32 v[250:251], vcc, v173, v235, v[250:251]\n" \
+    "v_mad_i64_i32 v[250:251], vcc, v172, v235, v[250:251]\n" \
     "v_mad_i64_i32 v[248:249], vcc, v214, v234, v[248:249]\n" \
     "v_mad_i64_i32 v[250:251], vcc, v210, v242, v[250:251]\n" \
     "v_mad_i64_i32 v[248:249], vcc, v210, v243, v[248:249]\n" \
-    "v_mad_i64_i32 v[250:251], vcc, v174, v243, v[250:251]\n" \
+    "v_mad_i64_i32 v[250:251], vcc, v173, v243, v[250:251]\n" \
     "v_mad_i64_i32 v[248:249], vcc, v215, v242, v[248:249]\n" \
     "v_mad_i64_i32 v[250:251], vcc, v211, v184, v[250:251]\n" \
     "v_mad_i64_i32 v[248:249], vcc, v211, v189, v[248:249]\n" \
-    "v_mad_i64_i32 v[250:251], vcc, v175, v189, v[250:251]\n" \
+    "v_mad_i64_i32 v[250:251], vcc, v174, v189, v[250:251]\n" \
     "v_mad_i64_i32 v[248:249], vcc, v216, v184, v[248:249]\n" \
     "v_mad_i64_i32 v[250:251], vcc, v212, v183, v[250:251]\n" \
     "v_mad_i64_i32 v[248:249], vcc, v212, v188, v[248:249]\n" \
-    "v_mad_i64_i32 v[250:251], vcc, v176, v188, v[250:251]\n" \
+    "v_mad_i64_i32 v[250:251], vcc, v175, v188, v[250:251]\n" \
     "v_mad_i64_i32 v[248:249], vcc, v217, v183, v[248:249]\n" \
-    "v_and_b32_e64 v183, %91, v250\n" \
-    "v_ashrrev_i64 v[250:251], 26, v[250:251]\n" \
-    "v_and_b32_e64 v185, %91, v248\n" \
-    "v_ashrrev_i64 v[248:249], 26, v[248:249]\n" \
-    "v_mad_i64_i32 v[250:251], vcc, v208, v238, v[250:251]\n" \
-    "v_mad_i64_i32 v[248:249], vcc, v208, v239, v[248:249]\n" \
-    "v_mad_i64_i32 v[250:251], vcc, v172, v239, v[250:251]\n" \
-    "v_mad_i64_i32 v[248:249], vcc, v213, v238, v[248:249]\n" \
+    "v_mad_i64_i32 v[250:251], vcc, v213, v182, v[250:251]\n" \
+    "v_mad_i64_i32 v[248:249], vcc, v213, v186, v[248:249]\n" \
+    "v_mad_i64_i32 v[250:251], vcc, v176, v186, v[250:251]\n" \
+    "v_mad_i64_i32 v[248:249], vcc, v218, v182, v[248:249]\n" \
+    "v_and_b32_e64 v177, %91, v250\n" \
+    "v_ashrrev_i64 v[250:251], 26, v[250:251]\n" \
+    "v_and_b32_e64 v182, %91, v248\n" \
+    "v_ashrrev_i64 v[248:249], 26, v[248:249]\n" \
     "v_mad_i64_i32 v[250:251], vcc, v209, v236, v[250:251]\n" \
     "v_mad_i64_i32 v[248:249], vcc, v209, v237, v[248:249]\n" \
-    "v_mad_i64_i32 v[250:251], vcc, v173, v237, v[250:251]\n" \
+    "v_mad_i64_i32 v[250:251], vcc, v172, v237, v[250:251]\n" \
     "v_mad_i64_i32 v[248:249], vcc, v214, v236, v[248:249]\n" \
     "v_mad_i64_i32 v[250:251], vcc, v210, v234, v[250:251]\n" \
     "v_mad_i64_i32 v[248:249], vcc, v210, v235, v[248:249]\n" \
-    "v_mad_i64_i32 v[250:251], vcc, v174, v235, v[250:251]\n" \
+    "v_mad_i64_i32 v[250:251], vcc, v173, v235, v[250:251]\n" \
     "v_mad_i64_i32 v[248:249], vcc, v215, v234, v[248:249]\n" \
     "v_mad_i64_i32 v[250:251], vcc, v211, v242, v[250:251]\n" \
     "v_mad_i64_i32 v[248:249], vcc, v211, v243, v[248:249]\n" \
-    "v_mad_i64_i32 v[250:251], vcc, v175, v243, v[250:251]\n" \
+    "v_mad_i64_i32 v[250:251], vcc, v174, v243, v[250:251]\n" \
     "v_mad_i64_i32 v[248:249], vcc, v216, v242, v[248:249]\n" \
     "v_mad_i64_i32 v[250:251], vcc, v212, v184, v[250:251]\n" \
     "v_mad_i64_i32 v[248:249], vcc, v212, v189, v[248:249]\n" \
-    "v_mad_i64_i32 v[250:251], vcc, v176, v189, v[250:251]\n" \
+    "v_mad_i64_i32 v[250:251], vcc, v175, v189, v[250:251]\n" \
     "v_mad_i64_i32 v[248:249], vcc, v217, v184, v[248:249]\n" \
-    "v_and_b32_e64 v184, %91, v250\n" \
-    "v_ashrrev_i64 v[250:251], 26, v[250:251]\n" \
-    "v_and_b32_e64 v186, %91, v248\n" \
-    "v_ashrrev_i64 v[248:249], 26, v[248:249]\n" \
-    "v_mad_i64_i32 v[250:251], vcc, v208, v240, v[250:251]\n" \
-    "v_mad_i64_i32 v[248:249], vcc, v208, v241, v[248:249]\n" \
-    "v_mad_i64_i32 v[250:251], vcc, v172, v241, v[250:251]\n" \
-    "v_mad_i64_i32 v[248:249], vcc, v213, v240, v[248:249]\n" \
+    "v_mad_i64_i32 v[250:251], vcc, v213, v183, v[250:251]\n" \
+    "v_mad_i64_i32 v[248:249], vcc, v213, v188, v[248:249]\n" \
+    "v_mad_i64_i32 v[250:251], vcc, v176, v188, v[250:251]\n" \
+    "v_mad_i64_i32 v[248:249], vcc, v218, v183, v[248:249]\n" \
+    "v_and_b32_e64 v183, %91, v250\n" \
+    "v_ashrrev_i64 v[250:251], 26, v[250:251]\n" \
+    "v_and_b32_e64 v185, %91, v248\n" \
+    "v_ashrrev_i64 v[248:249], 26, v[248:249]\n" \
     "v_mad_i64_i32 v[250:251], vcc, v209, v238, v[250:251]\n" \
     "v_mad_i64_i32 v[248:249], vcc, v209, v239, v[248:249]\n" \
-    "v_mad_i64_i32 v[250:251], vcc, v173, v239, v[250:251]\n" \
+    "v_mad_i64_i32 v[250:251], vcc, v172, v239, v[250:251]\n" \
     "v_mad_i64_i32 v[248:249], vcc, v214, v238, v[248:249]\n" \
     "v_mad_i64_i32 v[250:251], vcc, v210, v236, v[250:251]\n" \
     "v_mad_i64_i32 v[248:249], vcc, v210, v237, v[248:249]\n" \
-    "v_mad_i64_i32 v[250:251], vcc, v174, v237, v[250:251]\n" \
+    "v_mad_i64_i32 v[250:251], vcc, v173, v237, v[250:251]\n" \
     "v_mad_i64_i32 v[248:249], vcc, v215, v236, v[248:249]\n" \
     "v_mad_i64_i32 v[250:251], vcc, v211, v234, v[250:251]\n" \
     "v_mad_i64_i32 v[248:249], vcc, v211, v235, v[248:249]\n" \
-    "v_mad_i64_i32 v[250:251], vcc, v175, v235, v[250:251]\n" \
+    "v_mad_i64_i32 v[250:251], vcc, v174, v235, v[250:251]\n" \
     "v_mad_i64_i32 v[248:249], vcc, v216, v234, v[248:249]\n" \
     "v_mad_i64_i32 v[250:251], vcc, v212, v242, v[250:251]\n" \
     "v_mad_i64_i32 v[248:249], vcc, v212, v243, v[248:249]\n" \
+    "v_mad_i64_i32 v[250:251], vcc, v175, v243, v[250:251]\n" \
+    "v_mad_i64_i32 v[248:249], vcc, v217, v242, v[248:249]\n" \
+    "v_mad_i64_i32 v[250:251], vcc, v213, v184, v[250:251]\n" \
+    "v_mad_i64_i32 v[248:249], vcc, v213, v189, v[248:249]\n" \
+    "v_mad_i64_i32 v[250:251], vcc, v176, v189, v[250:251]\n" \
+    "v_mad_i64_i32 v[248:249], vcc, v218, v184, v[248:249]\n" \
+    "v_and_b32_e64 v184, %91, v250\n" \
+    "v_ashrrev_i64 v[250:251], 26, v[250:251]\n" \
+    "v_and_b32_e64 v186, %91, v248\n" \
+    "v_ashrrev_i64 v[248:249], 26, v[248:249]\n" \
+    "v_mad_i64_i32 v[250:251], vcc, v209, v240, v[250:251]\n" \
+    "v_mad_i64_i32 v[248:249], vcc, v209, v241, v[248:249]\n" \
+    "v_mad_i64_i32 v[250:251], vcc, v172, v241, v[250:251]\n" \
+    "v_mad_i64_i32 v[248:249], vcc, v214, v240, v[248:249]\n" \
+    "v_mad_i64_i32 v[250:251], vcc, v210, v238, v[250:251]\n" \
+    "v_mad_i64_i32 v[248:249], vcc, v210, v239, v[248:249]\n" \
+    "v_mad_i64_i32 v[250:251], vcc, v173, v239, v[250:251]\n" \
+    "v_mad_i64_i32 v[248:249], vcc, v215, v238, v[248:249]\n" \
+    "v_mad_i64_i32 v[250:251], vcc, v211, v236, v[250:251]\n" \
+    "v_mad_i64_i32 v[248:249], vcc, v211, v237, v[248:249]\n" \
+    "v_mad_i64_i32 v[250:251], vcc, v174, v237, v[250:251]\n" \
+    "v_mad_i64_i32 v[248:249], vcc, v216, v236, v[248:249]\n" \
+    "v_mad_i64_i32 v[250:251], vcc, v212, v234, v[250:251]\n" \
+    "v_mad_i64_i32 v[248:249], vcc, v212, v235, v[248:249]\n" \
+    "v_mad_i64_i32 v[250:251], vcc, v175, v235, v[250:251]\n" \
+    "v_mad_i64_i32 v[248:249], vcc, v217, v234, v[248:249]\n" \
+    "v_mad_i64_i32 v[250:251], vcc, v213, v242, v[250:251]\n" \
+    "v_mad_i64_i32 v[248:249], vcc, v213, v243, v[248:249]\n" \
     "v_mad_i64_i32 v[250:251], vcc, v176, v243, v[250:251]\n" \
-    "v_mad_i64_i32 v[248:249], vcc, v217, v242, v[248:249]\n" \
+    "v_mad_i64_i32 v[248:249], vcc, v218, v242, v[248:249]\n" \
     "v_and_b32_e64 v172, %91, v250\n" \
     "v_ashrrev_i64 v[250:251], 26, v[250:251]\n" \
     "v_and_b32_e64 v173, %91, v248\n" \
diff --git a/fourq_amd/csrc/recode.hip.h b/fourq_amd/csrc/recode.hip.h
--- a/fourq_amd/csrc/recode.hip.h
+++ b/fourq_amd/csrc/recode.hip.h
@@ -1,11 +1,21 @@
 #pragma once
+#if defined(__HIPCC__)
 #include "fp127.hip.h"
-
+#define FQ_HD __host__ __device__ __forceinline__
+#else
+#include <stdint.h>
 namespace fq {
+typedef uint32_t u32;
+typedef uint64_t u64;
+}
+#define FQ_HD inline
+#endif
+
+namespace fq {
 
 typedef unsigned __int128 u128;
 
-FQ_DEV u64 mul_shift256(const u64 a[4], const u64 m[4]) {
+FQ_HD u64 mul_shift256(const u64 a[4], const u64 m[4]) {
     u64 w0, w1, w2, w3, w4;
     u128 t;
     t = (u128)a[0] * m[0];                       w0 = (u64)t;
@@ -25,6 +35,7 @@
     return w4;
 }
 
+#if defined(__HIPCC__)
 FQ_DEV void decompose(const u64 m[4], u64 v[4]) {
     u64 t[4];
 #pragma unroll
@@ -45,67 +56,76 @@
 #pragma unroll
     for (int i = 0; i < 4; i++) v[i] = acp[i] ^ (mask & (ac[i] ^ acp[i]));
 }
+#endif
 
 struct EndoDigits {
     u64 sign;
     u64 d[3];
     u32 top;
 };
-FQ_DEV EndoDigits recode(const u64 vin[4]) {
+struct EndoPlanes {
+    u64 n;
+    u64 d[3];
+    u32 top;
+};
+FQ_HD EndoPlanes recode_planes(const u64 vin[4]) {
+    EndoPlanes r;
+    r.n = ~(vin[0] >> 1);
+    r.top = 0;
+#pragma unroll
+    for (int j = 0; j < 3; j++) {
+        const u64 t = vin[j + 1] + r.n;
+        r.d[j] = t ^ r.n;
+        r.top |= (u32)(t < r.n) << j;
+    }
+    return r;
+}
+FQ_HD EndoDigits recode(const u64 vin[4]) {
+    const EndoPlanes p = recode_planes(vin);
     EndoDigits r;
-    r.sign = vin[0] >> 1;
-    u64 v1 = vin[1], v2 = vin[2], v3 = vin[3];
-    u64 p1 = 0, p2 = 0, p3 = 0;
-    u64 s = r.sign;
-#pragma unroll 1
-    for (int i = 0; i < 64; i++) {
-        u64 nb1 = ~(s >> i) & 1;
-        u64 b;
-        b = v1 & 1; p1 |= b << i; v1 = (v1 >> 1) + (nb1 & b);
-        b = v2 & 1; p2 |= b << i; v2 = (v2 >> 1) + (nb1 & b);
-        b = v3 & 1; p3 |= b << i; v3 = (v3 >> 1) + (nb1 & b);
-    }
-    r.d[0] = p1; r.d[1] = p2; r.d[2] = p3;
-    r.top = (u32)(v1 + 2 * v2 + 4 * v3);
+    r.sign = ~p.n;
+    r.d[0] = p.d[0]; r.d[1] = p.d[1]; r.d[2] = p.d[2];
+    r.top = p.top;
     return r;
 }
 struct EndoNibbles {
     u32 w[8];
     u32 top;
 };
-FQ_DEV EndoNibbles recode_nibbles(const u64 vin[4]) {
+template <int RB, int PB> FQ_HD void exchange_address_bits(u32 x[8]) {
+    constexpr u32 D = 1u << PB;
+    constexpr u32 KEEP = PB == 0 ? 0x55555555u : PB == 1 ? 0x33333333u : PB == 2 ? 0x0f0f0f0fu : PB == 3 ? 0x00ff00ffu : 0x0000ffffu;
+#pragma unroll
+    for (int lo = 0; lo < 8; lo++) {
+        if (lo & (1 << RB)) continue;
+        const int hi = lo | (1 << RB);
+        const u32 a = x[lo], b = x[hi];
+        x[lo] = (a & KEEP) | ((b << D) & ~KEEP);
+        x[hi] = ((a >> D) & KEEP) | (b & ~KEEP);
+    }
+}
+FQ_HD EndoNibbles recode_nibbles(const u64 vin[4]) {
+    const EndoPlanes p = recode_planes(vin);
+    u32 x[8] = { (u32)p.d[0], (u32)(p.d[0] >> 32), (u32)p.d[1], (u32)(p.d[1] >> 32), (u32)p.d[2], (u32)(p.d[2] >> 32), (u32)p.n, (u32)(p.n >> 32) };
+    exchange_address_bits<1, 0>(x);
+    exchange_address_bits<1, 2>(x);
+    exchange_address_bits<1, 4>(x);
+    exchange_address_bits<2, 1>(x);
+    exchange_address_bits<2, 3>(x);
     EndoNibbles r;
-    u64 s = vin[0] >> 1;
-    u64 v1 = vin[1], v2 = vin[2], v3 = vin[3];
-#pragma unroll
-    for (int t = 0; t < 8; t++) r.w[t] = 0;
-#pragma unroll 1
-    for (int k = 0; k < 8; k++) {
-        u32 w = 0;
-#pragma unroll
-        for (int j = 0; j < 8; j++) {
-            const u32 nb1 = ~(u32)s & 1;
-            s >>= 1;
-            const u32 b1 = (u32)v1 & 1, b2 = (u32)v2 & 1, b3 = (u32)v3 & 1;
-            v1 = (v1 >> 1) + (nb1 & b1);
-            v2 = (v2 >> 1) + (nb1 & b2);
-            v3 = (v3 >> 1) + (nb1 & b3);
-            w = (w >> 4) | ((b1 | (b2 << 1) | (b3 << 2) | (nb1 << 3)) << 28);
-        }
-#pragma unroll
-        for (int t = 0; t < 7; t++) r.w[t] = r.w[t + 1];
-        r.w[7] = w;
-    }
-    r.top = (u32)(v1 + 2 * v2 + 4 * v3);
+#pragma unroll
+    for (int k = 0; k < 8; k++) r.w[k] = x[((k & 1) << 2) | (k & 2) | (k >> 2)];
+    r.top = p.top;
     return r;
 }
-FQ_DEV u32 endo_digit(const EndoDigits& e, int i) {
+FQ_HD u32 endo_digit(const EndoDigits& e, int i) {
     return (u32)((e.d[0] >> i) & 1) | ((u32)((e.d[1] >> i) & 1) << 1) | ((u32)((e.d[2] >> i) & 1) << 2);
 }
-FQ_DEV u32 endo_neg_mask(const EndoDigits& e, int i) {
+FQ_HD u32 endo_neg_mask(const EndoDigits& e, int i) {
     return (u32)((e.sign >> i) & 1) - 1u;
 }
 
+#if defined(__HIPCC__)
 struct WinScalar {
     u64 r[4];
 };
@@ -242,4 +262,6 @@
     for (int r = 0; r < S::W - 1; r++) if ((u >> r) & 1) set_bit(S::E * j + (r + 1) * S::D);
 }
 
-}
+#endif
+
+}
diff --git a/include/fourq_amd.h b/include/fourq_amd.h
--- a/include/fourq_amd.h
+++ b/include/fourq_amd.h
@@ -218,7 +218,8 @@
     FOURQ_SC_WINDOWED = 66,
     FOURQ_SC_REDUCE512 = 67,
     FOURQ_SC_MULSUB = 68,
-    FOURQ_SC_MUL = 69
+    FOURQ_SC_MUL = 69,
+    FOURQ_SC_RECODE_NIBBLES = 70
 };
 int fourq_prim_words(int op, size_t *in_words, size_t *out_words);
 int fourq_prim_batch(fourq_ctx *ctx, int op, const uint64_t *in, uint64_t *out, size_t n);
```

After: 223.2 million (median of 6 runs). +1.2%, better.
